# voidstrike/FPSG

Hardware: AMD Instinct MI355X
Metric: episodes/sec (+ Chamfer-kernel HBM GB/s in roofline.hbm), 2048-pt clouds, 224x224 images; episode = fwd + Chamfer + bwd, step = E episodes + all-reduce + Adam (higher is better)
Workload: dtype f32

## Files before the change

fpsg_amd/_hip.py:

```python
from __future__ import annotations

import ctypes
import os
import threading

import torch

_HERE = os.path.dirname(os.path.abspath(__file__))
LIB_PATH = os.environ.get("FPSG_HIP_LIB") or os.path.join(_HERE, "libfpsg_hip.so")

_c_f32p = ctypes.c_void_p
_c_i32p = ctypes.c_void_p
_c_int = ctypes.c_int
_c_stream = ctypes.c_void_p

SIGNATURES = {
    "fpsg_version": [],
    "fpsg_last_error": [],
    "fpsg_chamfer_fwd": [_c_f32p, _c_f32p, _c_int, _c_int, _c_int,
                         _c_f32p, _c_i32p, _c_f32p, _c_i32p, _c_stream],
    "fpsg_chamfer_bwd": [_c_f32p, _c_f32p, _c_i32p, _c_i32p, _c_f32p, _c_f32p,
                         _c_int, _c_int, _c_int, _c_f32p, _c_f32p, _c_stream],
    "fpsg_chamfer_losses": [_c_f32p, _c_f32p, _c_int, _c_int, _c_int, _c_int, ctypes.c_float, ctypes.c_float, _c_f32p,
                            _c_stream],
    "fpsg_chamfer_loss_grads": [_c_f32p, _c_f32p, _c_f32p, _c_int, _c_int, _c_int, _c_int, ctypes.c_float,
                                ctypes.c_float, _c_f32p, _c_f32p, _c_stream],
    "fpsg_chamfer_fwd_variant": [_c_f32p, _c_f32p, _c_int, _c_int, _c_int,
                                 _c_f32p, _c_i32p, _c_f32p, _c_i32p, _c_int, _c_stream],
    "fpsg_chamfer_workspace_bytes": [_c_int, _c_int, _c_int, _c_int],
    "fpsg_chamfer_fwd_tiled": [_c_f32p, _c_f32p, _c_int, _c_int, _c_int,
                               _c_f32p, _c_i32p, _c_f32p, _c_i32p, ctypes.c_void_p, ctypes.c_size_t, _c_int,
                               _c_stream],
    "fpsg_chamfer_fwd_tiled_losses": [_c_f32p, _c_f32p, _c_int, _c_int, _c_int,
                                      _c_f32p, _c_i32p, _c_f32p, _c_i32p, ctypes.c_void_p, ctypes.c_size_t, _c_int,
                                      _c_int, ctypes.c_float, ctypes.c_float, _c_f32p, _c_stream],
    "fpsg_chamfer_bwd_losses": [_c_f32p, _c_f32p, _c_i32p, _c_i32p, _c_f32p, _c_f32p, _c_f32p,
                                _c_int, _c_int, _c_int, _c_int, ctypes.c_float, ctypes.c_float, _c_f32p, _c_f32p,
                                _c_stream],
    "fpsg_chamfer_bwd_sorted": [_c_f32p, _c_f32p, _c_i32p, _c_i32p, _c_f32p, _c_f32p,
                                _c_int, _c_int, _c_int, _c_f32p, _c_f32p, _c_stream],
    "fpsg_chamfer_bwd_scan": [_c_f32p, _c_f32p, _c_i32p, _c_i32p, _c_f32p, _c_f32p,
                              _c_int, _c_int, _c_int, _c_f32p, _c_f32p, _c_stream],
    "fpsg_knn_workspace_floats": [_c_int, _c_int, _c_int],
    "fpsg_knn": [_c_f32p, _c_int, _c_int, _c_int, _c_int, _c_i32p, _c_f32p, _c_stream],
    "fpsg_knn_ex": [_c_f32p, _c_int, _c_int, _c_int, _c_int, _c_int, _c_i32p, _c_f32p, _c_int, _c_stream],
    "fpsg_edge_feature_fwd": [_c_f32p, _c_i32p, _c_int, _c_int, _c_int, _c_int, _c_f32p, _c_stream],
    "fpsg_edge_feature_bwd": [_c_f32p, _c_i32p, _c_int, _c_int, _c_int, _c_int, _c_f32p, _c_stream],
    "fpsg_edgeconv_blocks": [_c_int, _c_int, _c_int],
    "fpsg_edgeconv_reverse_graph_fits": [_c_int, _c_int],
    "fpsg_edgeconv_reverse_graph": [_c_i32p, _c_int, _c_int, _c_int, _c_i32p, _c_i32p, _c_stream],
    "fpsg_edgeconv_prep_blocks": [ctypes.c_long],
    "fpsg_edgeconv_stats_finalize": [_c_f32p, _c_int, _c_f32p, _c_f32p, _c_f32p, _c_f32p, ctypes.c_float, ctypes.c_float,
                                     ctypes.c_double, _c_int, _c_int, _c_f32p, _c_stream],
    "fpsg_edgeconv_stats_ws_floats": [_c_int, _c_int],
    "fpsg_edgeconv_stats_finalize_ws": [_c_f32p, _c_int, _c_f32p, _c_f32p, _c_f32p, _c_f32p, ctypes.c_float, ctypes.c_float,
                                        ctypes.c_double, _c_int, _c_int, _c_f32p, _c_f32p, _c_stream],
    "fpsg_edgeconv_bwd_finalize": [_c_f32p, _c_int, _c_f32p, ctypes.c_double, _c_int, _c_int, _c_f32p, _c_f32p, _c_f32p,
                                   _c_stream],
    "fpsg_edgeconv_act": [_c_f32p, _c_f32p, _c_f32p, ctypes.c_float, ctypes.c_long, _c_int, _c_f32p, _c_stream],
    "fpsg_edgeconv_bwd_prep": [_c_f32p, _c_f32p, _c_f32p, _c_f32p, ctypes.c_float, ctypes.c_long, _c_int, _c_f32p, _c_f32p,
                               _c_stream],
    "fpsg_edgeconv_fwd": [_c_f32p, _c_i32p, _c_f32p, _c_int, _c_int, _c_int, _c_int, _c_f32p, _c_f32p,
                          _c_f32p, _c_f32p, _c_stream],
    "fpsg_edgeconv_bwd": [_c_f32p, _c_f32p, _c_f32p, _c_f32p, _c_i32p, _c_i32p, _c_f32p, _c_int, _c_int,
                          _c_int, _c_int, _c_f32p, _c_stream],
    "fpsg_softmin": [_c_f32p, _c_f32p, _c_f32p, _c_int, _c_int, _c_int, ctypes.c_float, _c_f32p, _c_stream],
    "fpsg_sinkhorn_workspace_floats": [_c_int, _c_int, _c_int],
    "fpsg_sinkhorn_divergence": [_c_f32p, _c_f32p, _c_int, _c_int, _c_int, ctypes.c_void_p, _c_int, _c_f32p, _c_f32p,
                                 _c_stream],
    "fpsg_dec1_tiles": [_c_int],
    "fpsg_dec1_fwd": [_c_f32p, _c_f32p, _c_int, _c_int, _c_f32p, _c_f32p, _c_f32p, _c_f32p, _c_f32p, _c_int, _c_int,
                      _c_int, _c_int, _c_int, ctypes.c_float, _c_f32p, _c_f32p, _c_f32p, _c_f32p, _c_stream],
    "fpsg_dec1_bwd": [_c_f32p, _c_f32p, _c_f32p, _c_int, _c_int, _c_f32p, _c_f32p, _c_int, _c_int, _c_int, _c_int,
                      _c_int, _c_f32p, _c_f32p, _c_f32p, _c_f32p, _c_f32p, _c_stream],
    "fpsg_dec1_fwd_ld": [_c_f32p, _c_int, _c_f32p, _c_int, _c_int, _c_f32p, _c_int, _c_f32p, _c_f32p, _c_f32p, _c_f32p, _c_int,
                         _c_int, _c_int, _c_int, _c_int, ctypes.c_float, _c_f32p, _c_int, _c_f32p, _c_f32p, _c_f32p,
                         _c_stream],
    "fpsg_dec1_bwd_ld": [_c_f32p, _c_int, _c_f32p, _c_int, _c_f32p, _c_int, _c_int, _c_f32p, _c_int, _c_f32p, _c_int, _c_int,
                         _c_int, _c_int, _c_int, _c_int, _c_f32p, _c_f32p, _c_f32p, _c_f32p, _c_f32p, _c_stream],
    "fpsg_bn_act_rows_fwd": [_c_f32p, _c_int, ctypes.POINTER(ctypes.c_int), ctypes.POINTER(ctypes.c_int), _c_int,
                             _c_f32p, _c_f32p, _c_f32p, _c_int, ctypes.c_float, _c_int, ctypes.c_float, _c_f32p,
                             _c_f32p, _c_f32p, _c_stream],
    "fpsg_bn_act_rows_bwd": [_c_f32p, _c_int, ctypes.POINTER(ctypes.c_int), ctypes.POINTER(ctypes.c_int), _c_int,
                             _c_f32p, _c_f32p, _c_f32p, _c_int, _c_int, ctypes.c_float, _c_f32p, _c_f32p, _c_f32p,
                             _c_f32p, _c_stream],
    "fpsg_bn_workspace_floats": [_c_int, _c_int, _c_int],
    "fpsg_bn_act_fwd": [_c_f32p, _c_f32p, _c_f32p, _c_f32p, _c_f32p, _c_f32p, ctypes.c_float, _c_int, _c_int, _c_int, _c_int,
                        ctypes.c_float, _c_int, ctypes.c_float, _c_f32p, _c_f32p, _c_f32p, _c_f32p, _c_f32p,
                        _c_stream],
    "fpsg_bn_act_bwd": [_c_f32p, _c_f32p, _c_f32p, _c_f32p, _c_int, _c_int, _c_int, _c_int, _c_int,
                        ctypes.c_float, _c_f32p, _c_f32p, _c_f32p, _c_f32p, _c_f32p, _c_f32p, _c_stream],
    "fpsg_bn_act_bwd_coef": [_c_f32p, _c_f32p, _c_f32p, _c_f32p, _c_int, _c_int, _c_int, _c_int, _c_int, ctypes.c_float,
                             _c_f32p, _c_f32p, _c_f32p, _c_f32p, _c_stream],
    "fpsg_bn_act_bwd_parts": [_c_f32p, _c_f32p, _c_f32p, _c_f32p, _c_int, _c_int, _c_int, _c_int, _c_int,
                        ctypes.c_float, _c_f32p, _c_f32p, _c_f32p, _c_f32p, _c_f32p, _c_f32p, _c_f32p, _c_int, _c_stream],
    "fpsg_bn_pool_workspace_floats": [_c_int, _c_int, _c_int, _c_int],
    "fpsg_bn_act_pool_fwd": [_c_f32p, _c_f32p, _c_f32p, _c_f32p, _c_f32p, _c_f32p, ctypes.c_float, _c_int, _c_int, _c_int, _c_int,
                             _c_int, ctypes.c_float, _c_int, ctypes.c_float, _c_f32p, _c_f32p, _c_f32p, _c_f32p,
                             _c_f32p, _c_f32p, _c_int, _c_stream],
    "fpsg_bn_act_pool_bwd": [_c_f32p, _c_f32p, _c_f32p, _c_f32p, _c_int, _c_int, _c_int, _c_int, _c_int, _c_int,
                             ctypes.c_float, _c_f32p, _c_f32p, _c_f32p, _c_f32p, _c_f32p, _c_f32p, _c_stream],
    "fpsg_bn_max_workspace_floats": [_c_int, _c_int, _c_int],
    "fpsg_bn_max_dz_offset": [_c_int, _c_int, _c_int],
    "fpsg_bn_act_max_fwd": [_c_f32p, _c_f32p, _c_f32p, _c_f32p, _c_f32p, _c_f32p, ctypes.c_float, _c_int, _c_int, _c_int, _c_int,
                            ctypes.c_float, _c_int, ctypes.c_float, _c_f32p, _c_i32p, _c_f32p, _c_f32p, _c_f32p,
                            _c_f32p, _c_stream],
    "fpsg_bn_act_max_bwd": [_c_f32p, _c_f32p, _c_f32p, _c_i32p, _c_f32p, _c_int, _c_int, _c_int, _c_int, _c_int,
                            ctypes.c_float, _c_f32p, _c_f32p, _c_f32p, _c_f32p, _c_f32p, _c_f32p, _c_stream],
    "fpsg_max_bwd_prep": [_c_f32p, _c_f32p, _c_f32p, _c_f32p, _c_f32p, _c_f32p, _c_int, _c_int, _c_int, _c_int, _c_f32p, _c_f32p,
                          _c_f32p, _c_f32p, _c_stream],
    "fpsg_max_bwd_dw": [_c_f32p, _c_f32p, _c_f32p, _c_f32p, _c_f32p, _c_int, _c_int, _c_int, _c_f32p, _c_stream],
    "fpsg_max_bwd_gather": [_c_f32p, _c_f32p, _c_i32p, _c_int, _c_int, _c_int, _c_int, _c_f32p, _c_f32p, _c_stream],
    "fpsg_max_bwd_scatter": [_c_f32p, _c_f32p, _c_f32p, _c_f32p, _c_i32p, _c_f32p, _c_int, _c_int, _c_int, _c_int, _c_f32p,
                             _c_stream],
    "fpsg_max_bwd_scatter_workspace_floats": [_c_int, _c_int, _c_int],
    "fpsg_bn_act_max_bwd_coef": [_c_f32p, _c_f32p, _c_f32p, _c_i32p, _c_f32p, _c_int, _c_int, _c_int, _c_int, _c_int,
                                 ctypes.c_float, _c_f32p, _c_f32p, _c_f32p, _c_f32p, _c_stream],
    "fpsg_wino_input_transform": [_c_int, _c_f32p, _c_int, _c_int, _c_int, _c_int, _c_f32p, ctypes.c_long, _c_stream],
    "fpsg_wino_output_transform": [_c_int, _c_f32p, _c_int, _c_int, _c_int, _c_int, _c_f32p, ctypes.c_long, _c_stream],
    "fpsg_wino_stats_parts": [_c_int, _c_int, _c_int, _c_int],
    "fpsg_wino_output_transform_stats": [_c_int, _c_f32p, _c_int, _c_int, _c_int, _c_int, _c_f32p, _c_f32p, _c_f32p,
                                         ctypes.c_long, _c_stream],
    "fpsg_wino_grad_output_transform": [_c_int, _c_f32p, _c_int, _c_int, _c_int, _c_int, _c_f32p, ctypes.c_long, _c_stream],
    "fpsg_wino_grad_transforms": [_c_int, _c_f32p, _c_int, _c_int, _c_int, _c_int, _c_f32p, _c_f32p, ctypes.c_long, _c_stream],
    "fpsg_wino_filter_transform": [_c_int, _c_f32p, _c_int, _c_int, _c_int, _c_f32p, _c_stream],
    "fpsg_wino_output_transform_bwd_stats": [_c_int, _c_f32p, _c_int, _c_int, _c_int, _c_int, _c_f32p, _c_f32p, _c_f32p,
                                             _c_f32p, _c_f32p, ctypes.c_long, _c_stream],
    "fpsg_wino_filter_transform_batch": [ctypes.c_void_p, _c_int, ctypes.c_long, _c_stream],
    "fpsg_wino_filter_grad_transform": [_c_int, _c_f32p, _c_int, _c_int, _c_f32p, _c_stream],
    "fpsg_wino_conv_fused": [_c_f32p, _c_f32p, _c_int, _c_int, _c_int, _c_int, _c_int, _c_f32p, _c_stream],
    "fpsg_wino_input_transform_act": [_c_int, _c_f32p, _c_f32p, _c_f32p, _c_int, _c_int, _c_int, _c_int, _c_f32p, ctypes.c_long,
                                      _c_stream],
    "fpsg_wino_conv_fused_act": [_c_f32p, _c_f32p, _c_f32p, _c_f32p, _c_int, _c_int, _c_int, _c_int, _c_int, _c_f32p,
                                 _c_stream],
    "fpsg_wino_dw_fused_workspace_floats": [_c_int, _c_int, _c_int, _c_int],
    "fpsg_wino_dw_fused": [_c_f32p, _c_f32p, _c_f32p, _c_f32p, _c_int, _c_int, _c_int, _c_int, _c_int, _c_f32p, _c_f32p,
                           _c_stream],
    "fpsg_wino_conv_fused_parts": [_c_int, _c_int, _c_int, _c_int],
    "fpsg_wino_conv_fused_stats": [_c_f32p, _c_f32p, _c_f32p, _c_f32p, _c_int, _c_int, _c_int, _c_int, _c_int, _c_f32p,
                                   _c_f32p, _c_f32p, _c_stream],
    "fpsg_bn_stats": [_c_f32p, _c_f32p, _c_f32p, _c_f32p, _c_f32p, _c_f32p, ctypes.c_float, _c_int, _c_int, _c_int, _c_int,
                      ctypes.c_float, _c_f32p, _c_f32p, _c_f32p, _c_f32p, _c_f32p, _c_int, _c_stream],
    "fpsg_conv_first_dw_workspace_floats": [_c_int, _c_int, _c_int],
    "fpsg_conv_first_parts": [_c_int, _c_int, _c_int],
    "fpsg_conv_first_fwd": [_c_f32p, _c_f32p, _c_int, _c_int, _c_int, _c_int, _c_int, _c_f32p, _c_f32p, _c_f32p, _c_stream],
    "fpsg_conv_first_dw": [_c_f32p, _c_f32p, _c_int, _c_int, _c_int, _c_int, _c_int, _c_f32p, _c_f32p, _c_stream],
    "fpsg_conv_first_dw_fold": [_c_f32p, _c_f32p, _c_f32p, _c_f32p, _c_f32p, _c_f32p, _c_int, _c_int, _c_int, _c_int, _c_int,
                                _c_f32p, _c_f32p, _c_stream],
    "fpsg_adam_step": [_c_f32p, _c_f32p, _c_f32p, _c_f32p, ctypes.c_size_t, ctypes.c_float, ctypes.c_float,
                       ctypes.c_float, ctypes.c_float, _c_int, ctypes.c_float, _c_stream],
    "fpsg_flat_accumulate_segments": [_c_f32p, ctypes.c_void_p, ctypes.c_void_p, _c_int, ctypes.c_size_t, _c_int, _c_stream],
    "fpsg_flat_accumulate_tables": [_c_f32p, ctypes.c_void_p, ctypes.c_void_p, _c_int, _c_int, ctypes.c_size_t, _c_int,
                                    _c_stream],
    "fpsg_adam_step_segments": [_c_f32p, ctypes.c_void_p, ctypes.c_void_p, _c_int, _c_f32p, _c_f32p, ctypes.c_size_t,
                                ctypes.c_float, ctypes.c_float, ctypes.c_float, ctypes.c_float, _c_int, ctypes.c_float,
                                _c_stream],
    "fpsg_gemm_split_workspace_floats": [_c_int, _c_int, _c_int, _c_int, _c_int, _c_int],
    "fpsg_gemm_split": [_c_f32p, _c_f32p, _c_f32p, _c_int, _c_int, _c_int, _c_int, _c_int, _c_int, _c_int, ctypes.c_long,
                        ctypes.c_long, ctypes.c_long, _c_int, _c_int, _c_f32p, ctypes.c_size_t, _c_stream],
    "fpsg_gemm_split_packed_a_bytes": [_c_int, _c_int, _c_int, _c_int],
    "fpsg_gemm_split_pack_a": [_c_f32p, _c_int, _c_int, _c_int, _c_int, ctypes.c_long, _c_int, ctypes.c_void_p, _c_stream],
    "fpsg_gemm_split_nn_packed": [ctypes.c_void_p, _c_f32p, _c_f32p, _c_int, _c_int, _c_int, _c_int, _c_int, _c_int,
                                  ctypes.c_long, ctypes.c_long, _c_int, _c_stream],
    "fpsg_gemm_split_nn_persistent": [ctypes.c_void_p, _c_f32p, _c_f32p, _c_int, _c_int, _c_int, _c_int, _c_int, _c_int,
                                      ctypes.c_long, ctypes.c_long, _c_int, _c_stream],
    "fpsg_gemm_f32_nn": [_c_f32p, _c_f32p, _c_f32p, _c_int, _c_int, _c_int, _c_int, _c_int, _c_int, _c_int,
                         ctypes.c_long, ctypes.c_long, ctypes.c_long, _c_int, _c_stream],
    "fpsg_emd_workspace_floats": [_c_int, _c_int, _c_int],
    "fpsg_emd_approx": [_c_f32p, _c_f32p, _c_int, _c_int, _c_int, _c_f32p, _c_f32p, _c_f32p, _c_f32p,
                        _c_stream],
    "fpsg_emd_approx_variant": [_c_f32p, _c_f32p, _c_int, _c_int, _c_int, _c_f32p, _c_f32p, _c_f32p, _c_f32p, _c_int,
                                _c_stream],
    "fpsg_emd_exact_workspace_floats": [_c_int, _c_int],
    "fpsg_emd_exact": [_c_f32p, _c_f32p, _c_int, _c_int, ctypes.c_float, _c_int, _c_f32p, _c_f32p, _c_i32p, _c_i32p,
                       _c_f32p, _c_f32p, _c_f32p, _c_stream],
    "fpsg_chamfer_cross": [_c_f32p, _c_f32p, _c_int, _c_int, _c_int, _c_int, _c_f32p, _c_stream],
}
_RESTYPES = {"fpsg_last_error": ctypes.c_char_p, "fpsg_chamfer_workspace_bytes": ctypes.c_size_t,
             "fpsg_sinkhorn_workspace_floats": ctypes.c_size_t,
             "fpsg_knn_workspace_floats": ctypes.c_size_t,
             "fpsg_bn_workspace_floats": ctypes.c_size_t, "fpsg_bn_pool_workspace_floats": ctypes.c_size_t, "fpsg_bn_max_workspace_floats": ctypes.c_size_t, "fpsg_bn_max_dz_offset": ctypes.c_size_t, "fpsg_conv_first_dw_workspace_floats": ctypes.c_size_t, "fpsg_emd_workspace_floats": ctypes.c_size_t, "fpsg_emd_exact_workspace_floats": ctypes.c_size_t, "fpsg_max_bwd_scatter_workspace_floats": ctypes.c_size_t,
             "fpsg_wino_dw_fused_workspace_floats": ctypes.c_size_t, "fpsg_gemm_split_workspace_floats": ctypes.c_size_t, "fpsg_gemm_split_packed_a_bytes": ctypes.c_size_t, "fpsg_edgeconv_stats_ws_floats": ctypes.c_size_t}

_lib = None
_lock = threading.Lock()


class FpsgHipError(RuntimeError):
    pass


def load() -> ctypes.CDLL:
    global _lib
    if _lib is None:
        with _lock:
            if _lib is None:
                if not os.path.exists(LIB_PATH):
                    raise FpsgHipError(
                        f"{LIB_PATH} not found: build it with `make -C fpsg_amd/csrc` "
                        "(or `python -c 'import __graft_entry__ as g; g.build()'`). "
                        "fpsg_amd has no CPU or PyTorch fallback for its HIP ops.")
                lib = ctypes.CDLL(LIB_PATH)
                for name, argtypes in SIGNATURES.items():
                    fn = getattr(lib, name)
                    fn.argtypes = argtypes
                    fn.restype = _RESTYPES.get(name, ctypes.c_int)
                _lib = lib
    return _lib


def check(rc: int, what: str) -> None:
    if rc != 0:
        msg = load().fpsg_last_error()
        raise FpsgHipError(f"{what} failed (code {rc}): {msg.decode() if msg else ''}")


def dev_tensor(t: torch.Tensor, dtype: torch.dtype, name: str) -> torch.Tensor:
    if not isinstance(t, torch.Tensor):
        raise TypeError(f"{name}: expected a torch.Tensor, got {type(t)}")
    if t.device.type != "cuda":
        raise FpsgHipError(
            f"{name}: tensor is on '{t.device}'; fpsg_amd HIP ops run on a ROCm GPU only "
            "(no CPU fallback)")
    if t.dtype != dtype:
        raise TypeError(f"{name}: expected dtype {dtype}, got {t.dtype}")
    if not t.is_contiguous():
        raise ValueError(f"{name}: tensor must be contiguous")
    return t


def stream_of(t: torch.Tensor) -> int:
    return torch.cuda.current_stream(t.device).cuda_stream


def ptr(t: torch.Tensor) -> int:
    return t.data_ptr()
```

fpsg_amd/csrc/bnact.hip:

```cpp
#include <algorithm>
#include <atomic>
#include <cstdlib>

#include "fpsg_common.h"

namespace fpsg {
namespace {

constexpr int kBnThreads = 256;
constexpr int kBnSeg = 4096;
constexpr int kBnSlices = 64;
constexpr int kBnU = kBnSeg / 4 / kBnThreads;

enum BnAct { kActNone = 0, kActRelu = 1, kActLeaky = 2 };

template <int ACT>
__device__ __forceinline__ float act_fwd(float z, float slope) {
  if (ACT == kActRelu) return z > 0.0f ? z : 0.0f;
  if (ACT == kActLeaky) return z > 0.0f ? z : z * slope;
  return z;
}
template <int ACT>
__device__ __forceinline__ float act_grad(float z, float slope) {
  if (ACT == kActRelu) return z > 0.0f ? 1.0f : 0.0f;
  if (ACT == kActLeaky) return z > 0.0f ? 1.0f : slope;
  return 1.0f;
}

__device__ __forceinline__ void block_reduce2(float& a, float& b, float* red ) {
#pragma unroll
  for (int off = 32; off >= 1; off >>= 1) {
    a += __shfl_down(a, off, 64);
    b += __shfl_down(b, off, 64);
  }
  const int wave = threadIdx.x >> 6, lane = threadIdx.x & 63;
  if (lane == 0) { red[wave] = a; red[4 + wave] = b; }
  __syncthreads();
  if (threadIdx.x == 0) {
    a = (red[0] + red[1]) + (red[2] + red[3]);
    b = (red[4] + red[5]) + (red[6] + red[7]);
  }
}

constexpr int kBnFoldBanks = 16, kBnFoldChannels = 4096;
__device__ unsigned g_bn_fold_counters[kBnFoldBanks * kBnFoldChannels];
struct BnFoldArgs {
  const float* gamma; const float* beta;
  double count; float eps, momentum;
  float* chan; float* batch_mean; float* batch_var_unbiased; float* run_mean; float* run_var;
  unsigned* counters;
};
__device__ __forceinline__ void wave_sum2(double& a, double& b);
__device__ __forceinline__ void bn_fwd_finalize_channel(double s0, double s1, int c, int C, const float* gamma, const float* beta,
                                                        double count, float eps, float* chan, float* batch_mean,
                                                        float* batch_var_unbiased, float* run_mean, float* run_var, float momentum);

template <int MODE, int ACT, bool NT = false, bool FOLD = false>
__global__ __launch_bounds__(kBnThreads) void bn_reduce_kernel(
    const float* __restrict__ x, const float* __restrict__ dy, const float* __restrict__ chan ,
    const float* __restrict__ pb, int N, int C, int L, int S, float slope, float* __restrict__ part ,
    const BnFoldArgs f = BnFoldArgs{}) {
  __shared__ float red[8];
  const int c = blockIdx.y, s = blockIdx.x;
  const float b = pb ? pb[c] : 0.0f;
  const int segs = (L + kBnSeg - 1) / kBnSeg;
  const int items = N * segs;
  float sc = 0.0f, sh = 0.0f, mu = 0.0f, rs = 0.0f;
  if (MODE == 1) { sc = chan[c]; sh = chan[C + c]; mu = chan[2 * C + c]; rs = chan[3 * C + c]; }
  float a0 = 0.0f, a1 = 0.0f;
  const bool vec = (L & 3) == 0;
  for (int it = s; it < items; it += S) {
    const int n = it / segs, seg = it - n * segs;
    const size_t base = ((size_t)n * C + c) * L + (size_t)seg * kBnSeg;
    const int len = (L - seg * kBnSeg) < kBnSeg ? (L - seg * kBnSeg) : kBnSeg;
    if (vec) {
      const v4f* __restrict__ xp = reinterpret_cast<const v4f*>(x + base);
      const v4f* __restrict__ gp = reinterpret_cast<const v4f*>(MODE == 1 ? dy + base : x + base);
      const int nvec = len / 4;
      for (int e0 = threadIdx.x; e0 < nvec; e0 += kBnU * kBnThreads) {
        v4f xq[kBnU], gq[kBnU];
#pragma unroll
        for (int j = 0; j < kBnU; ++j) {
          const int e = e0 + j * kBnThreads;
          xq[j] = gq[j] = (v4f){0.0f, 0.0f, 0.0f, 0.0f};
          if (e < nvec) {
            xq[j] = ld_stream<NT>(xp + e);
            if (MODE == 1) gq[j] = ld_stream<NT>(gp + e);
          }
        }
#pragma unroll
        for (int j = 0; j < kBnU; ++j) {
          if (e0 + j * kBnThreads < nvec) {
            v4f xv = xq[j];
#pragma unroll
            for (int u = 0; u < 4; ++u) xv[u] += b;
            if (MODE == 0) {
#pragma unroll
              for (int u = 0; u < 4; ++u) { a0 += xv[u]; a1 = fma_rn(xv[u], xv[u], a1); }
            } else {
#pragma unroll
              for (int u = 0; u < 4; ++u) {
                const float dz = gq[j][u] * act_grad<ACT>(fma_rn(xv[u], sc, sh), slope);
                a0 += dz;
                a1 = fma_rn(dz, (xv[u] - mu) * rs, a1);
              }
            }
          }
        }
      }
    } else {
      for (int e = threadIdx.x; e < len; e += kBnThreads) {
        const float xv = x[base + e] + b;
        if (MODE == 0) {
          a0 += xv; a1 = fma_rn(xv, xv, a1);
        } else {
          const float dz = dy[base + e] * act_grad<ACT>(fma_rn(xv, sc, sh), slope);
          a0 += dz;
          a1 = fma_rn(dz, (xv - mu) * rs, a1);
        }
      }
    }
  }
  block_reduce2(a0, a1, red);
  if constexpr (FOLD) {
    __shared__ int last;
    if (threadIdx.x == 0) {
      __hip_atomic_store(&part[((size_t)c * S + s) * 2 + 0], a0, __ATOMIC_RELAXED, __HIP_MEMORY_SCOPE_AGENT);
      __hip_atomic_store(&part[((size_t)c * S + s) * 2 + 1], a1, __ATOMIC_RELAXED, __HIP_MEMORY_SCOPE_AGENT);
      asm volatile("s_waitcnt vmcnt(0)" ::: "memory");
      const unsigned t = __hip_atomic_fetch_add(&f.counters[c], 1u, __ATOMIC_RELAXED, __HIP_MEMORY_SCOPE_AGENT);
      last = t == (unsigned)S - 1u;
    }
    __syncthreads();
    if (!last || threadIdx.x >= 64) return;
    const int lane = threadIdx.x;
    double s0 = 0.0, s1 = 0.0;
    for (int sl = lane; sl < S; sl += 64) {
      s0 += __hip_atomic_load(&part[((size_t)c * S + sl) * 2], __ATOMIC_RELAXED, __HIP_MEMORY_SCOPE_AGENT);
      s1 += __hip_atomic_load(&part[((size_t)c * S + sl) * 2 + 1], __ATOMIC_RELAXED, __HIP_MEMORY_SCOPE_AGENT);
    }
    wave_sum2(s0, s1);
    if (lane != 0) return;
    bn_fwd_finalize_channel(s0, s1, c, C, f.gamma, f.beta, f.count, f.eps, f.chan, f.batch_mean, f.batch_var_unbiased,
                            f.run_mean, f.run_var, f.momentum);
    __hip_atomic_store(&f.counters[c], 0u, __ATOMIC_RELAXED, __HIP_MEMORY_SCOPE_AGENT);
    return;
  }
  if (threadIdx.x == 0) {
    part[((size_t)c * S + s) * 2 + 0] = a0;
    part[((size_t)c * S + s) * 2 + 1] = a1;
  }
}

__device__ __forceinline__ void wave_sum2(double& a, double& b) {
#pragma unroll
  for (int off = 32; off >= 1; off >>= 1) { a += __shfl_down(a, off, 64); b += __shfl_down(b, off, 64); }
}

__global__ __launch_bounds__(64) void bn_fwd_finalize_kernel(const float* __restrict__ part, const float* __restrict__ gamma,
                                       const float* __restrict__ beta, int C, int S, double count, float eps,
                                       float* __restrict__ chan, float* __restrict__ batch_mean,
                                       float* __restrict__ batch_var_unbiased, float* __restrict__ run_mean,
                                       float* __restrict__ run_var, float momentum) {
  const int c = blockIdx.x, lane = threadIdx.x;
  double s0 = 0.0, s1 = 0.0;
  for (int sl = lane; sl < S; sl += 64) { s0 += part[((size_t)c * S + sl) * 2]; s1 += part[((size_t)c * S + sl) * 2 + 1]; }
  wave_sum2(s0, s1);
  if (lane != 0) return;
  bn_fwd_finalize_channel(s0, s1, c, C, gamma, beta, count, eps, chan, batch_mean, batch_var_unbiased, run_mean, run_var, momentum);
}

__device__ __forceinline__ void bn_fwd_finalize_channel(double s0, double s1, int c, int C, const float* gamma, const float* beta,
                                                        double count, float eps, float* chan, float* batch_mean,
                                                        float* batch_var_unbiased, float* run_mean, float* run_var, float momentum) {
  const double mean = s0 / count;
  double var = s1 / count - mean * mean;
  var = var > 0.0 ? var : 0.0;
  const float rstd = (float)(1.0 / sqrt(var + (double)eps));
  const float g = gamma ? gamma[c] : 1.0f, b = beta ? beta[c] : 0.0f;
  const float scale = g * rstd;
  chan[c] = scale;
  chan[C + c] = b - (float)mean * scale;
  chan[2 * C + c] = (float)mean;
  chan[3 * C + c] = rstd;
  const float unbiased = (float)(count > 1.0 ? var * count / (count - 1.0) : var);
  if (batch_mean) batch_mean[c] = (float)mean;
  if (batch_var_unbiased) batch_var_unbiased[c] = unbiased;
  if (run_mean && momentum >= 0.0f) {
    run_mean[c] = fma_rn(momentum, (float)mean, (1.0f - momentum) * run_mean[c]);
    run_var[c] = fma_rn(momentum, unbiased, (1.0f - momentum) * run_var[c]);
  }
}

__global__ void bn_eval_chan_kernel(const float* __restrict__ rmean, const float* __restrict__ rvar,
                                    const float* __restrict__ gamma, const float* __restrict__ beta, int C,
                                    float eps, float* __restrict__ chan) {
  const int c = blockIdx.x * blockDim.x + threadIdx.x;
  if (c >= C) return;
  const float rstd = 1.0f / sqrtf(rvar[c] + eps);
  const float g = gamma ? gamma[c] : 1.0f, b = beta ? beta[c] : 0.0f;
  chan[c] = g * rstd;
  chan[C + c] = b - rmean[c] * g * rstd;
  chan[2 * C + c] = rmean[c];
  chan[3 * C + c] = rstd;
}

__global__ __launch_bounds__(64) void bn_bwd_finalize_kernel(const float* __restrict__ part, const float* __restrict__ chan, int C,
                                       int S, double count, int training, float* __restrict__ dgamma,
                                       float* __restrict__ dbeta, float* __restrict__ coef ) {
  const int c = blockIdx.x, lane = threadIdx.x;
  double s0 = 0.0, s1 = 0.0;
  for (int q = lane; q < S; q += 64) {
    s0 += part[((size_t)c * S + q) * 2];
    s1 += part[((size_t)c * S + q) * 2 + 1];
  }
  wave_sum2(s0, s1);
  if (lane != 0) return;
  dbeta[c] = (float)s0;
  dgamma[c] = (float)s1;
  const double scale = chan[c], mean = chan[2 * C + c], rstd = chan[3 * C + c];
  coef[c] = (float)scale;
  if (training) {
    const double k2 = -scale * s1 * rstd / count;
    coef[C + c] = (float)k2;
    coef[2 * C + c] = (float)(-scale * s0 / count - k2 * mean);
  } else {
    coef[C + c] = 0.0f;
    coef[2 * C + c] = 0.0f;
  }
}

template <int MODE, int ACT, bool NT = false>
__global__ __launch_bounds__(kBnThreads) void bn_apply_kernel(const float* __restrict__ x,
                                                              const float* __restrict__ dy,
                                                              const float* __restrict__ chan,
                                                              const float* __restrict__ coef,
                                                              const float* __restrict__ pb, int C, int L,
                                                              float slope, float* __restrict__ out,
                                                              float* __restrict__ dxpart ) {
  __shared__ float red[8];
  const int row = blockIdx.x;
  const int c = row % C;
  const int seg = blockIdx.y;
  const float b = pb ? pb[c] : 0.0f;
  float acc = 0.0f, unused = 0.0f;
  const size_t base = (size_t)row * L + (size_t)seg * kBnSeg;
  const int len = (L - seg * kBnSeg) < kBnSeg ? (L - seg * kBnSeg) : kBnSeg;
  const float sc = chan[c], sh = chan[C + c];
  float k1 = 0.0f, k2 = 0.0f, k3 = 0.0f;
  if (MODE == 1) { k1 = coef[c]; k2 = coef[C + c]; k3 = coef[2 * C + c]; }
  if ((L & 3) == 0) {
    const v4f* __restrict__ xp = reinterpret_cast<const v4f*>(x + base);
    const v4f* __restrict__ gp = reinterpret_cast<const v4f*>(MODE == 1 ? dy + base : x + base);
    v4f* __restrict__ op = reinterpret_cast<v4f*>(out + base);
    const int nvec = len / 4;
    for (int e0 = threadIdx.x; e0 < nvec; e0 += kBnU * kBnThreads) {
      v4f xq[kBnU], gq[kBnU];
#pragma unroll
      for (int j = 0; j < kBnU; ++j) {
        const int e = e0 + j * kBnThreads;
        xq[j] = gq[j] = (v4f){0.0f, 0.0f, 0.0f, 0.0f};
        if (e < nvec) {
          xq[j] = ld_stream<NT>(xp + e);
          if (MODE == 1) gq[j] = ld_stream<NT>(gp + e);
        }
      }
#pragma unroll
      for (int j = 0; j < kBnU; ++j) {
        const int e = e0 + j * kBnThreads;
        if (e < nvec) {
          v4f xv = xq[j];
#pragma unroll
          for (int u = 0; u < 4; ++u) xv[u] += b;
          v4f r;
          if (MODE == 0) {
#pragma unroll
            for (int u = 0; u < 4; ++u) r[u] = act_fwd<ACT>(fma_rn(xv[u], sc, sh), slope);
          } else {
#pragma unroll
            for (int u = 0; u < 4; ++u) {
              const float dz = gq[j][u] * act_grad<ACT>(fma_rn(xv[u], sc, sh), slope);
              r[u] = fma_rn(k1, dz, fma_rn(k2, xv[u], k3));
            }
            acc += (r[0] + r[1]) + (r[2] + r[3]);
          }
          st_stream<NT>(op + e, r);
        }
      }
    }
  } else {
    for (int e = threadIdx.x; e < len; e += kBnThreads) {
      const float xv = x[base + e] + b;
      if (MODE == 0) {
        out[base + e] = act_fwd<ACT>(fma_rn(xv, sc, sh), slope);
      } else {
        const float dz = dy[base + e] * act_grad<ACT>(fma_rn(xv, sc, sh), slope);
        const float r = fma_rn(k1, dz, fma_rn(k2, xv, k3));
        out[base + e] = r;
        acc += r;
      }
    }
  }
  if (MODE == 1 && dxpart) {
    block_reduce2(acc, unused, red);
    if (threadIdx.x == 0) dxpart[(size_t)row * gridDim.y + seg] = acc;
  }
}

__global__ __launch_bounds__(64) void bn_dxsum_kernel(const float* __restrict__ dxpart, int N, int C, int segs,
                                                      float* __restrict__ dpb) {
  const int c = blockIdx.x;
  const int items = N * segs;
  double a = 0.0;
  for (int it = threadIdx.x; it < items; it += 64) {
    const int n = it / segs, seg = it - n * segs;
    a += (double)dxpart[((size_t)n * C + c) * segs + seg];
  }
#pragma unroll
  for (int off = 32; off >= 1; off >>= 1) a += __shfl_down(a, off, 64);
  if (threadIdx.x == 0) dpb[c] = (float)a;
}

constexpr int kBnSmallMax = 16384;

constexpr int kBnMaxSegs = 4;
struct BnSegs {
  int ld;
  int off[kBnMaxSegs], len[kBnMaxSegs];
  int staged[kBnMaxSegs];
  int tpr_log2[kBnMaxSegs];
  int stat_stride;
};

template <int MODE, int ACT>
__global__ __launch_bounds__(kBnThreads) void bn_small_kernel(
    const float* __restrict__ x, const float* __restrict__ dy, const float* __restrict__ gamma,
    const float* __restrict__ beta, const float* __restrict__ pb, int N, int C, BnSegs segs, int training, float eps,
    float slope, float* __restrict__ out, float* __restrict__ chan, float* __restrict__ batch_mean,
    float* __restrict__ batch_var_unbiased, float* __restrict__ dgamma, float* __restrict__ dbeta,
    float* __restrict__ dpb, float* __restrict__ run_mean, float* __restrict__ run_var, float momentum) {
  const int sgi = blockIdx.y;
  const int L = segs.len[sgi], ld = segs.ld, staged = segs.staged[sgi], tpr_log2 = segs.tpr_log2[sgi];
  x += segs.off[sgi];
  out += segs.off[sgi];
  if (MODE == 1) dy += segs.off[sgi];
  chan += (size_t)sgi * 4 * C;
  if (batch_mean) batch_mean += (size_t)sgi * segs.stat_stride;
  if (batch_var_unbiased) batch_var_unbiased += (size_t)sgi * segs.stat_stride;
  if (MODE == 1) {
    dgamma += (size_t)sgi * C;
    dbeta += (size_t)sgi * C;
    if (dpb) dpb += (size_t)sgi * C;
  }
  extern __shared__ __attribute__((aligned(16))) float stage[];
  __shared__ float red[8];
  __shared__ float bc[4];
  const int c = blockIdx.x;
  const float b = pb ? pb[c] : 0.0f;
  const double count = (double)N * (double)L;
  const bool vec = (L & 3) == 0;
  const int L4 = L >> 2;
  v4f* __restrict__ sx = reinterpret_cast<v4f*>(stage);
  v4f* __restrict__ sd = reinterpret_cast<v4f*>(stage) + (size_t)N * L4;
  float sc = 0.0f, sh = 0.0f, mu = 0.0f, rs = 0.0f;
  if (MODE == 1 || !training) { sc = chan[c]; sh = chan[C + c]; mu = chan[2 * C + c]; rs = chan[3 * C + c]; }
  const bool two_sweeps = MODE == 1 || training;
  const bool keep = staged && vec && two_sweeps;
  const int tpr = 1 << tpr_log2, rpi = kBnThreads >> tpr_log2;
  const int e0 = threadIdx.x & (tpr - 1), n0 = threadIdx.x >> tpr_log2;
  if (two_sweeps) {
    float a0 = 0.0f, a1 = 0.0f;
    int n_first = n0;
    if (vec && L4 <= tpr) {
      const bool has = e0 < L4;
      for (; n_first + (kBnU - 1) * rpi < N; n_first += kBnU * rpi) {
        v4f xq[kBnU], gq[kBnU];
#pragma unroll
        for (int j = 0; j < kBnU; ++j) {
          xq[j] = gq[j] = (v4f){0.0f, 0.0f, 0.0f, 0.0f};
          if (has) {
            const size_t base = ((size_t)(n_first + j * rpi) * C + c) * ld;
            xq[j] = reinterpret_cast<const v4f*>(x + base)[e0];
            if (MODE == 1) gq[j] = reinterpret_cast<const v4f*>(dy + base)[e0];
          }
        }
        if (has) {
#pragma unroll
          for (int j = 0; j < kBnU; ++j) {
            const int n = n_first + j * rpi;
            v4f xv = xq[j];
#pragma unroll
            for (int u = 0; u < 4; ++u) xv[u] += b;
            if (MODE == 0) {
#pragma unroll
              for (int u = 0; u < 4; ++u) { a0 += xv[u]; a1 = fma_rn(xv[u], xv[u], a1); }
            } else {
              v4f dz;
#pragma unroll
              for (int u = 0; u < 4; ++u) {
                dz[u] = gq[j][u] * act_grad<ACT>(fma_rn(xv[u], sc, sh), slope);
                a0 += dz[u];
                a1 = fma_rn(dz[u], (xv[u] - mu) * rs, a1);
              }
              if (keep) sd[(size_t)n * L4 + e0] = dz;
            }
            if (keep) sx[(size_t)n * L4 + e0] = xv;
          }
        }
      }
    }
    for (int n = n_first; n < N; n += rpi) {
      const size_t base = ((size_t)n * C + c) * ld;
      if (vec) {
        const v4f* __restrict__ xp = reinterpret_cast<const v4f*>(x + base);
        const v4f* __restrict__ gp = reinterpret_cast<const v4f*>(MODE == 1 ? dy + base : x + base);
        for (int e = e0; e < L4; e += tpr) {
          v4f xv = xp[e];
#pragma unroll
          for (int u = 0; u < 4; ++u) xv[u] += b;
          if (MODE == 0) {
#pragma unroll
            for (int u = 0; u < 4; ++u) { a0 += xv[u]; a1 = fma_rn(xv[u], xv[u], a1); }
          } else {
            const v4f gv = gp[e];
            v4f dz;
#pragma unroll
            for (int u = 0; u < 4; ++u) {
              dz[u] = gv[u] * act_grad<ACT>(fma_rn(xv[u], sc, sh), slope);
              a0 += dz[u];
              a1 = fma_rn(dz[u], (xv[u] - mu) * rs, a1);
            }
            if (keep) sd[(size_t)n * L4 + e] = dz;
          }
          if (keep) sx[(size_t)n * L4 + e] = xv;
        }
      } else {
        for (int e = e0; e < L; e += tpr) {
          const float xv = x[base + e] + b;
          if (MODE == 0) {
            a0 += xv; a1 = fma_rn(xv, xv, a1);
          } else {
            const float dz = dy[base + e] * act_grad<ACT>(fma_rn(xv, sc, sh), slope);
            a0 += dz; a1 = fma_rn(dz, (xv - mu) * rs, a1);
          }
        }
      }
    }
    block_reduce2(a0, a1, red);
    if (threadIdx.x == 0) {
      if (MODE == 0) {
        const double mean = a0 / count;
        double var = a1 / count - mean * mean;
        var = var > 0.0 ? var : 0.0;
        const float rstd = (float)(1.0 / sqrt(var + (double)eps));
        const float g = gamma ? gamma[c] : 1.0f, bb = beta ? beta[c] : 0.0f;
        bc[0] = g * rstd; bc[1] = bb - (float)mean * g * rstd; bc[2] = (float)mean; bc[3] = rstd;
        chan[c] = bc[0]; chan[C + c] = bc[1]; chan[2 * C + c] = bc[2]; chan[3 * C + c] = bc[3];
        const float unbiased = (float)(count > 1.0 ? var * count / (count - 1.0) : var);
        if (batch_mean) batch_mean[c] = (float)mean;
        if (batch_var_unbiased) batch_var_unbiased[c] = unbiased;
        if (run_mean && momentum >= 0.0f) {
          run_mean[c] = fma_rn(momentum, (float)mean, (1.0f - momentum) * run_mean[c]);
          run_var[c] = fma_rn(momentum, unbiased, (1.0f - momentum) * run_var[c]);
        }
      } else {
        dbeta[c] = a0; dgamma[c] = a1;
        const double k2 = training ? -(double)sc * a1 * rs / count : 0.0;
        bc[0] = sc; bc[1] = (float)k2;
        bc[2] = training ? (float)(-(double)sc * a0 / count - k2 * mu) : 0.0f;
      }
    }
    __syncthreads();
    if (MODE == 0) { sc = bc[0]; sh = bc[1]; }
  } else {
    if (threadIdx.x == 0) { bc[0] = sc; bc[1] = 0.0f; bc[2] = 0.0f; }
    __syncthreads();
  }
  const float k1 = bc[0], k2 = bc[1], k3 = bc[2];
  float acc = 0.0f, unused = 0.0f;
  for (int n = n0; n < N; n += rpi) {
    const size_t base = ((size_t)n * C + c) * ld;
    if (vec) {
      const v4f* __restrict__ xp = reinterpret_cast<const v4f*>(x + base);
      const v4f* __restrict__ gp = reinterpret_cast<const v4f*>(MODE == 1 ? dy + base : x + base);
      v4f* __restrict__ op = reinterpret_cast<v4f*>(out + base);
      for (int e = e0; e < L4; e += tpr) {
        v4f xv;
        if (keep) {
          xv = sx[(size_t)n * L4 + e];
        } else {
          xv = xp[e];
#pragma unroll
          for (int u = 0; u < 4; ++u) xv[u] += b;
        }
        v4f r;
        if (MODE == 0) {
#pragma unroll
          for (int u = 0; u < 4; ++u) r[u] = act_fwd<ACT>(fma_rn(xv[u], sc, sh), slope);
        } else {
          v4f dz;
          if (keep) {
            dz = sd[(size_t)n * L4 + e];
          } else {
            const v4f gv = gp[e];
#pragma unroll
            for (int u = 0; u < 4; ++u) dz[u] = gv[u] * act_grad<ACT>(fma_rn(xv[u], sc, sh), slope);
          }
#pragma unroll
          for (int u = 0; u < 4; ++u) r[u] = fma_rn(k1, dz[u], fma_rn(k2, xv[u], k3));
          acc += (r[0] + r[1]) + (r[2] + r[3]);
        }
        op[e] = r;
      }
    } else {
      for (int e = e0; e < L; e += tpr) {
        const float xv = x[base + e] + b;
        if (MODE == 0) {
          out[base + e] = act_fwd<ACT>(fma_rn(xv, sc, sh), slope);
        } else {
          const float dz = dy[base + e] * act_grad<ACT>(fma_rn(xv, sc, sh), slope);
          const float r = fma_rn(k1, dz, fma_rn(k2, xv, k3));
          out[base + e] = r;
          acc += r;
        }
      }
    }
  }
  if (MODE == 1 && dpb) {
    __syncthreads();
    block_reduce2(acc, unused, red);
    if (threadIdx.x == 0) dpb[c] = acc;
  }
}

inline void small_segment(BnSegs& g, int i, int N, int off, int L, int training, bool backward) {
  g.off[i] = off;
  g.len[i] = L;
  const size_t need = (size_t)N * L * sizeof(float) * (backward ? 2 : 1);
  g.staged[i] = ((L & 3) == 0 && need <= 64 * 1024 && (backward || training)) ? 1 : 0;
  const int row_items = (L & 3) == 0 ? L / 4 : L;
  int t = 0;
  while ((1 << t) < row_items && (1 << t) < kBnThreads) ++t;
  g.tpr_log2[i] = t;
}

template <int MODE>
void launch_small_segs(int act, const float* x, const float* dy, const float* gamma, const float* beta, const float* pb,
                       int N, int C, const BnSegs& g, int nseg, int training, float eps, float slope, float* out,
                       float* chan, float* bm, float* bv, float* dgamma, float* dbeta, float* dpb, float* rmean,
                       float* rvar, float momentum, hipStream_t s) {
  dim3 grid(C, nseg);
  size_t lds = 0;
  for (int i = 0; i < nseg; ++i)
    if (g.staged[i]) lds = std::max(lds, (size_t)N * g.len[i] * sizeof(float) * (MODE == 1 ? 2 : 1));
#define FPSG_SMALL(A) hipLaunchKernelGGL((bn_small_kernel<MODE, A>), grid, dim3(kBnThreads), lds, s, x, dy, gamma, beta, \
                                         pb, N, C, g, training, eps, slope, out, chan, bm, bv, dgamma, dbeta, dpb, rmean, \
                                         rvar, momentum)
  if (act == kActRelu) FPSG_SMALL(kActRelu);
  else if (act == kActLeaky) FPSG_SMALL(kActLeaky);
  else FPSG_SMALL(kActNone);
#undef FPSG_SMALL
}

template <int MODE>
void launch_small(int act, const float* x, const float* dy, const float* gamma, const float* beta, const float* pb,
                  int N, int C, int L, int training, float eps, float slope, float* out, float* chan, float* bm,
                  float* bv, float* dgamma, float* dbeta, float* dpb, float* rmean, float* rvar, float momentum,
                  hipStream_t s) {
  BnSegs g{};
  g.ld = L;
  small_segment(g, 0, N, 0, L, training, MODE == 1);
  launch_small_segs<MODE>(act, x, dy, gamma, beta, pb, N, C, g, 1, training, eps, slope, out, chan, bm, bv, dgamma,
                          dbeta, dpb, rmean, rvar, momentum, s);
}

int slices_for(int N, int L) {
  const int items = N * ((L + kBnSeg - 1) / kBnSeg);
  return items < kBnSlices ? items : kBnSlices;
}

template <int MODE>
void launch_reduce(int act, const float* x, const float* dy, const float* chan, const float* pb, int N, int C, int L,
                   int S, float slope, float* part, hipStream_t s) {
  dim3 grid(S, C);
#define FPSG_RED(A, T) hipLaunchKernelGGL((bn_reduce_kernel<MODE, A, T>), grid, dim3(kBnThreads), 0, s, x, dy, chan, pb, N, C, L, S, slope, part)
  if (beyond_cache((size_t)N * C * L * sizeof(float))) {
    if (act == kActRelu) FPSG_RED(kActRelu, true); else if (act == kActLeaky) FPSG_RED(kActLeaky, true); else FPSG_RED(kActNone, true);
  } else {
    if (act == kActRelu) FPSG_RED(kActRelu, false); else if (act == kActLeaky) FPSG_RED(kActLeaky, false); else FPSG_RED(kActNone, false);
  }
#undef FPSG_RED
}

template <int MODE>
void launch_apply(int act, const float* x, const float* dy, const float* chan, const float* coef, const float* pb,
                  int N, int C, int L, float slope, float* out, float* dxpart, hipStream_t s) {
  dim3 grid((unsigned)((size_t)N * C), (L + kBnSeg - 1) / kBnSeg);
#define FPSG_APP(A, T) hipLaunchKernelGGL((bn_apply_kernel<MODE, A, T>), grid, dim3(kBnThreads), 0, s, x, dy, chan, coef, pb, C, L, slope, out, dxpart)
  if (beyond_cache((size_t)N * C * L * sizeof(float))) {
    if (act == kActRelu) FPSG_APP(kActRelu, true); else if (act == kActLeaky) FPSG_APP(kActLeaky, true); else FPSG_APP(kActNone, true);
  } else {
    if (act == kActRelu) FPSG_APP(kActRelu, false); else if (act == kActLeaky) FPSG_APP(kActLeaky, false); else FPSG_APP(kActNone, false);
  }
#undef FPSG_APP
}

template <int VW> struct PoolVec;
template <> struct PoolVec<2> { typedef v4f in_t; typedef v2f out_t; };
template <> struct PoolVec<1> { typedef v2f in_t; typedef float out_t; };

template <int ACT>
__device__ __forceinline__ int window_argmax(const float (&z)[4], float slope, float& ymax) {
  float m = -INFINITY;
  int sel = 0;
#pragma unroll
  for (int k = 0; k < 4; ++k) {
    const float y = act_fwd<ACT>(z[k], slope);
    if (y > m || y != y) { m = y; sel = k; }
  }
  ymax = m;
  return sel;
}

template <int MODE, int ACT, int VW, bool NT>
__device__ __forceinline__ void pool_item(const float* __restrict__ xpl, const float* __restrict__ gpl,
// ... 308 lines not shown
      coef[2 * C + c] = 0.0f;
    }
  }
}

template <bool NT>
__global__ __launch_bounds__(kBnThreads) void bn_max_apply_kernel(const float* __restrict__ x,
                                                                  const float* __restrict__ pb,
                                                                  const float* __restrict__ dz,
                                                                  const int* __restrict__ idx,
                                                                  const float* __restrict__ coef, int C, int L,
                                                                  float* __restrict__ dx, float* __restrict__ dxpart) {
  __shared__ float red[8];
  const int row = blockIdx.x, c = row % C, seg = blockIdx.y;
  const size_t base = (size_t)row * L + (size_t)seg * kBnSeg;
  const int len = (L - seg * kBnSeg) < kBnSeg ? (L - seg * kBnSeg) : kBnSeg;
  const float b = pb ? pb[c] : 0.0f;
  const float k1 = coef[c], k2 = coef[C + c], k3 = coef[2 * C + c];
  const float d = dz[row];
  const int sel = idx[row] - seg * kBnSeg;
  float acc = 0.0f, unused = 0.0f;
  if ((L & 3) == 0) {
    const v4f* __restrict__ xp = reinterpret_cast<const v4f*>(x + base);
    v4f* __restrict__ op = reinterpret_cast<v4f*>(dx + base);
    const int nvec = len / 4;
    for (int e0 = threadIdx.x; e0 < nvec; e0 += kBnU * kBnThreads) {
      v4f xq[kBnU];
#pragma unroll
      for (int j = 0; j < kBnU; ++j) {
        const int e = e0 + j * kBnThreads;
        xq[j] = e < nvec ? ld_stream<NT>(xp + e) : (v4f){0.0f, 0.0f, 0.0f, 0.0f};
      }
#pragma unroll
      for (int j = 0; j < kBnU; ++j) {
        const int e = e0 + j * kBnThreads;
        if (e < nvec) {
          v4f r;
#pragma unroll
          for (int u = 0; u < 4; ++u) r[u] = fma_rn(k1, (4 * e + u == sel) ? d : 0.0f, fma_rn(k2, xq[j][u] + b, k3));
          acc += (r[0] + r[1]) + (r[2] + r[3]);
          st_stream<NT>(op + e, r);
        }
      }
    }
  } else {
    for (int e = threadIdx.x; e < len; e += kBnThreads) {
      const float r = fma_rn(k1, (e == sel) ? d : 0.0f, fma_rn(k2, x[base + e] + b, k3));
      acc += r;
      dx[base + e] = r;
    }
  }
  if (dxpart) {
    block_reduce2(acc, unused, red);
    if (threadIdx.x == 0) dxpart[(size_t)row * gridDim.y + seg] = acc;
  }
}

int check_dims(const char* fn, int N, int C, int L, int act) {
  FPSG_REQUIRE(N > 0 && C > 0 && L > 0, FPSG_E_SHAPE, "%s: N,C,L must be positive (got %d,%d,%d)", fn, N, C, L);
  FPSG_REQUIRE(act >= 0 && act <= 2, FPSG_E_SHAPE, "%s: act must be 0 (none), 1 (relu) or 2 (leaky)", fn);
  FPSG_REQUIRE(C <= 65535 && (L + kBnSeg - 1) / kBnSeg <= 65535 && (long)N * C < (1L << 31), FPSG_E_LIMIT,
               "%s: C=%d, L=%d or N*C=%ld beyond the grid limits", fn, C, L, (long)N * C);
  return 0;
}

}
}

extern "C" size_t fpsg_bn_workspace_floats(int N, int C, int L) {
  if (N <= 0 || C <= 0 || L <= 0) return 0;
  const size_t segs = ((size_t)L + fpsg::kBnSeg - 1) / fpsg::kBnSeg;
  return (size_t)C * fpsg::kBnSlices * 2 + (size_t)N * C * segs;
}

extern "C" int fpsg_bn_act_fwd(const float* x, const float* pre_bias, const float* gamma, const float* beta,
                               float* running_mean, float* running_var, float momentum, int N, int C, int L,
                               int training, float eps, int act, float slope, float* y, float* chan,
                               float* batch_mean, float* batch_var_unbiased, float* ws, fpsg_stream_t stream) {
  using namespace fpsg;
  int rc = check_dims("fpsg_bn_act_fwd", N, C, L, act);
  if (rc) return rc;
  FPSG_REQUIRE_PTR(x); FPSG_REQUIRE_PTR(y); FPSG_REQUIRE_PTR(chan);
  FPSG_REQUIRE(((reinterpret_cast<uintptr_t>(x) | reinterpret_cast<uintptr_t>(y)) & 15) == 0, FPSG_E_ALIGN,
               "fpsg_bn_act_fwd: x and y must be 16-byte aligned");
  hipStream_t s = static_cast<hipStream_t>(stream);
  const bool chan_given = training == 2;
  if (chan_given) training = 0;
  if (!training && !chan_given) { FPSG_REQUIRE_PTR(running_mean); FPSG_REQUIRE_PTR(running_var); }
  if ((long)N * L <= kBnSmallMax) {
    if (!training && !chan_given) {
      hipLaunchKernelGGL(bn_eval_chan_kernel, dim3((C + 255) / 256), dim3(256), 0, s, running_mean, running_var,
                         gamma, beta, C, eps, chan);
      if ((rc = launch_status("fpsg_bn_act_fwd(eval)"))) return rc;
    }
    launch_small<0>(act, x, nullptr, gamma, beta, pre_bias, N, C, L, training, eps, slope, y, chan, batch_mean,
                    batch_var_unbiased, nullptr, nullptr, nullptr, running_mean, running_var, momentum, s);
    return launch_status("fpsg_bn_act_fwd(small)");
  }
  if (training) {
    FPSG_REQUIRE_PTR(ws);
    const int S = slices_for(N, L);
    const char* fold = getenv("FPSG_BN_FINALIZE_FOLD");
    if (fold && fold[0] == '1' && C <= kBnFoldChannels) {
      static std::atomic<unsigned> next_bank{0};
      unsigned* counters = nullptr;
      FPSG_REQUIRE(hipGetSymbolAddress(reinterpret_cast<void**>(&counters), HIP_SYMBOL(g_bn_fold_counters)) == hipSuccess &&
                       counters, FPSG_E_LIMIT, "fpsg_bn_act_fwd: the fold counters are not addressable");
      BnFoldArgs f{gamma, beta, (double)N * (double)L, eps, momentum, chan, batch_mean, batch_var_unbiased, running_mean,
                   running_var, counters + (size_t)(next_bank.fetch_add(1) % kBnFoldBanks) * kBnFoldChannels};
      const dim3 grid(S, C);
      if (beyond_cache((size_t)N * C * L * sizeof(float)))
        hipLaunchKernelGGL((bn_reduce_kernel<0, kActNone, true, true>), grid, dim3(kBnThreads), 0, s, x, nullptr, nullptr, pre_bias, N, C, L, S, 0.0f, ws, f);
      else
        hipLaunchKernelGGL((bn_reduce_kernel<0, kActNone, false, true>), grid, dim3(kBnThreads), 0, s, x, nullptr, nullptr, pre_bias, N, C, L, S, 0.0f, ws, f);
      if ((rc = launch_status("fpsg_bn_act_fwd(stats + finalize)"))) return rc;
    } else {
      launch_reduce<0>(kActNone, x, nullptr, nullptr, pre_bias, N, C, L, S, 0.0f, ws, s);
      if ((rc = launch_status("fpsg_bn_act_fwd(stats)"))) return rc;
      hipLaunchKernelGGL(bn_fwd_finalize_kernel, dim3(C), dim3(64), 0, s, ws, gamma, beta, C, S,
                         (double)N * (double)L, eps, chan, batch_mean, batch_var_unbiased, running_mean, running_var,
                         momentum);
      if ((rc = launch_status("fpsg_bn_act_fwd(finalize)"))) return rc;
    }
  } else if (!chan_given) {
    hipLaunchKernelGGL(bn_eval_chan_kernel, dim3((C + 255) / 256), dim3(256), 0, s, running_mean, running_var,
                       gamma, beta, C, eps, chan);
    if ((rc = launch_status("fpsg_bn_act_fwd(eval)"))) return rc;
  }
  launch_apply<0>(act, x, nullptr, chan, nullptr, pre_bias, N, C, L, slope, y, nullptr, s);
  return launch_status("fpsg_bn_act_fwd(apply)");
}

namespace fpsg {
namespace {
int rows_segments(const char* fn, int ld, const int* seg_off, const int* seg_len, int nseg, int C, int act, bool backward,
                  BnSegs& g) {
  FPSG_REQUIRE(C > 0 && C <= 65535 * 64 && ld > 0, FPSG_E_SHAPE, "%s: C, ld must be positive (got %d, %d)", fn, C, ld);
  FPSG_REQUIRE(act >= kActNone && act <= kActLeaky, FPSG_E_SHAPE, "%s: unknown activation %d", fn, act);
  FPSG_REQUIRE(nseg >= 1 && nseg <= kBnMaxSegs, FPSG_E_LIMIT, "%s: %d segments (1..%d)", fn, nseg, kBnMaxSegs);
  FPSG_REQUIRE_PTR(seg_off); FPSG_REQUIRE_PTR(seg_len);
  FPSG_REQUIRE((ld & 3) == 0, FPSG_E_ALIGN, "%s: ld = %d must be a multiple of 4", fn, ld);
  g = BnSegs{};
  g.ld = ld;
  for (int i = 0; i < nseg; ++i) {
    FPSG_REQUIRE(seg_len[i] > 0 && seg_len[i] <= kBnSmallMax && seg_off[i] >= 0 && seg_off[i] + seg_len[i] <= ld,
                 FPSG_E_SHAPE, "%s: segment %d = [%d, +%d) does not fit a row of %d (a segment holds at most %d)", fn, i,
                 seg_off[i], seg_len[i], ld, kBnSmallMax);
    FPSG_REQUIRE((seg_off[i] & 3) == 0, FPSG_E_ALIGN, "%s: segment offset %d must be a multiple of 4", fn, seg_off[i]);
    for (int j = 0; j < i; ++j)
      FPSG_REQUIRE(seg_off[i] >= seg_off[j] + seg_len[j] || seg_off[j] >= seg_off[i] + seg_len[i], FPSG_E_SHAPE,
                   "%s: segments %d and %d overlap", fn, j, i);
    small_segment(g, i, 1, seg_off[i], seg_len[i], 1, backward);
  }
  return 0;
}
}
}

extern "C" int fpsg_bn_act_rows_fwd(const float* x, int ld, const int* seg_off, const int* seg_len, int nseg,
                                    const float* pre_bias, const float* gamma, const float* beta, int C, float eps,
                                    int act, float slope, float* y, float* chan, float* stats,
                                    fpsg_stream_t stream) {
  using namespace fpsg;
  BnSegs g;
  int rc = rows_segments("fpsg_bn_act_rows_fwd", ld, seg_off, seg_len, nseg, C, act, false, g);
  if (rc) return rc;
  FPSG_REQUIRE_PTR(x); FPSG_REQUIRE_PTR(y); FPSG_REQUIRE_PTR(chan);
  FPSG_REQUIRE(((reinterpret_cast<uintptr_t>(x) | reinterpret_cast<uintptr_t>(y)) & 15) == 0, FPSG_E_ALIGN,
               "fpsg_bn_act_rows_fwd: x and y must be 16-byte aligned");
  g.stat_stride = 2 * C;
  launch_small_segs<0>(act, x, nullptr, gamma, beta, pre_bias, 1, C, g, nseg, 1, eps, slope, y, chan, stats,
                       stats ? stats + C : nullptr, nullptr, nullptr, nullptr, nullptr, nullptr, -1.0f,
                       static_cast<hipStream_t>(stream));
  return launch_status("fpsg_bn_act_rows_fwd");
}

extern "C" int fpsg_bn_act_rows_bwd(const float* x, int ld, const int* seg_off, const int* seg_len, int nseg,
                                    const float* pre_bias, const float* dy, const float* chan, int C, int act,
                                    float slope, float* dx, float* dgamma, float* dbeta, float* dpre_bias,
                                    fpsg_stream_t stream) {
  using namespace fpsg;
  BnSegs g;
  int rc = rows_segments("fpsg_bn_act_rows_bwd", ld, seg_off, seg_len, nseg, C, act, true, g);
  if (rc) return rc;
  FPSG_REQUIRE_PTR(x); FPSG_REQUIRE_PTR(dy); FPSG_REQUIRE_PTR(chan); FPSG_REQUIRE_PTR(dx);
  FPSG_REQUIRE_PTR(dgamma); FPSG_REQUIRE_PTR(dbeta);
  FPSG_REQUIRE(((reinterpret_cast<uintptr_t>(x) | reinterpret_cast<uintptr_t>(dy) | reinterpret_cast<uintptr_t>(dx)) & 15) == 0,
               FPSG_E_ALIGN, "fpsg_bn_act_rows_bwd: x, dy and dx must be 16-byte aligned");
  launch_small_segs<1>(act, x, dy, nullptr, nullptr, pre_bias, 1, C, g, nseg, 1, 0.0f, slope, dx,
                       const_cast<float*>(chan), nullptr, nullptr, dgamma, dbeta, dpre_bias, nullptr, nullptr, -1.0f,
                       static_cast<hipStream_t>(stream));
  return launch_status("fpsg_bn_act_rows_bwd");
}

extern "C" int fpsg_bn_stats(const float* x, const float* pre_bias, const float* gamma, const float* beta,
                             float* running_mean, float* running_var, float momentum, int N, int C, int L,
                             int training, float eps, float* chan, float* batch_mean, float* batch_var_unbiased,
                             float* ws, const float* parts, int n_parts, fpsg_stream_t stream) {
  using namespace fpsg;
  int rc = check_dims("fpsg_bn_stats", N, C, L, kActNone);
  if (rc) return rc;
  FPSG_REQUIRE_PTR(x); FPSG_REQUIRE_PTR(chan);
  FPSG_REQUIRE((reinterpret_cast<uintptr_t>(x) & 15) == 0, FPSG_E_ALIGN, "fpsg_bn_stats: x must be 16-byte aligned");
  hipStream_t s = static_cast<hipStream_t>(stream);
  if (training) {
    int S = n_parts;
    if (parts) {
      FPSG_REQUIRE(n_parts > 0, FPSG_E_SHAPE, "fpsg_bn_stats: n_parts must be positive with parts (got %d)", n_parts);
    } else {
      FPSG_REQUIRE_PTR(ws);
      S = slices_for(N, L);
      launch_reduce<0>(kActNone, x, nullptr, nullptr, pre_bias, N, C, L, S, 0.0f, ws, s);
      if ((rc = launch_status("fpsg_bn_stats(stats)"))) return rc;
    }
    hipLaunchKernelGGL(bn_fwd_finalize_kernel, dim3(C), dim3(64), 0, s, parts ? parts : ws, gamma, beta, C, S,
                       (double)N * (double)L, eps, chan, batch_mean, batch_var_unbiased, running_mean, running_var,
                       momentum);
    return launch_status("fpsg_bn_stats(finalize)");
  }
  FPSG_REQUIRE_PTR(running_mean); FPSG_REQUIRE_PTR(running_var);
  hipLaunchKernelGGL(bn_eval_chan_kernel, dim3((C + 255) / 256), dim3(256), 0, s, running_mean, running_var,
                     gamma, beta, C, eps, chan);
  return launch_status("fpsg_bn_stats(eval)");
}

extern "C" int fpsg_bn_act_bwd(const float* x, const float* pre_bias, const float* dy, const float* chan, int N,
                               int C, int L, int training, int act, float slope, float* dx, float* dgamma,
                               float* dbeta, float* dpre_bias, float* coef, float* ws, fpsg_stream_t stream) {
  using namespace fpsg;
  int rc = check_dims("fpsg_bn_act_bwd", N, C, L, act);
  if (rc) return rc;
  FPSG_REQUIRE_PTR(x); FPSG_REQUIRE_PTR(dy); FPSG_REQUIRE_PTR(chan); FPSG_REQUIRE_PTR(dx);
  FPSG_REQUIRE_PTR(dgamma); FPSG_REQUIRE_PTR(dbeta); FPSG_REQUIRE_PTR(coef); FPSG_REQUIRE_PTR(ws);
  FPSG_REQUIRE(((reinterpret_cast<uintptr_t>(x) | reinterpret_cast<uintptr_t>(dy) | reinterpret_cast<uintptr_t>(dx)) & 15) == 0,
               FPSG_E_ALIGN, "fpsg_bn_act_bwd: x, dy and dx must be 16-byte aligned");
  hipStream_t s = static_cast<hipStream_t>(stream);
  if ((long)N * L <= kBnSmallMax) {
    launch_small<1>(act, x, dy, nullptr, nullptr, pre_bias, N, C, L, training, 0.0f, slope, dx,
                    const_cast<float*>(chan), nullptr, nullptr, dgamma, dbeta, dpre_bias, nullptr, nullptr, -1.0f, s);
    return launch_status("fpsg_bn_act_bwd(small)");
  }
  const int S = slices_for(N, L);
  launch_reduce<1>(act, x, dy, chan, pre_bias, N, C, L, S, slope, ws, s);
  if ((rc = launch_status("fpsg_bn_act_bwd(reduce)"))) return rc;
  hipLaunchKernelGGL(bn_bwd_finalize_kernel, dim3(C), dim3(64), 0, s, ws, chan, C, S,
                     (double)N * (double)L, training, dgamma, dbeta, coef);
  if ((rc = launch_status("fpsg_bn_act_bwd(finalize)"))) return rc;
  float* dxpart = dpre_bias ? ws + (size_t)C * kBnSlices * 2 : nullptr;
  launch_apply<1>(act, x, dy, chan, coef, pre_bias, N, C, L, slope, dx, dxpart, s);
  if ((rc = launch_status("fpsg_bn_act_bwd(apply)"))) return rc;
  if (dpre_bias) {
    hipLaunchKernelGGL(bn_dxsum_kernel, dim3(C), dim3(64), 0, s, dxpart, N, C, (L + kBnSeg - 1) / kBnSeg, dpre_bias);
    return launch_status("fpsg_bn_act_bwd(dpre_bias)");
  }
  return 0;
}

extern "C" int fpsg_bn_act_bwd_coef(const float* x, const float* pre_bias, const float* dy, const float* chan, int N,
                                    int C, int L, int training, int act, float slope, float* dgamma, float* dbeta,
                                    float* coef, float* ws, fpsg_stream_t stream) {
  using namespace fpsg;
  int rc = check_dims("fpsg_bn_act_bwd_coef", N, C, L, act);
  if (rc) return rc;
  FPSG_REQUIRE_PTR(x); FPSG_REQUIRE_PTR(dy); FPSG_REQUIRE_PTR(chan);
  FPSG_REQUIRE_PTR(dgamma); FPSG_REQUIRE_PTR(dbeta); FPSG_REQUIRE_PTR(coef); FPSG_REQUIRE_PTR(ws);
  FPSG_REQUIRE(((reinterpret_cast<uintptr_t>(x) | reinterpret_cast<uintptr_t>(dy)) & 15) == 0, FPSG_E_ALIGN,
               "fpsg_bn_act_bwd_coef: x and dy must be 16-byte aligned");
  FPSG_REQUIRE((long)N * L > kBnSmallMax, FPSG_E_LIMIT, "fpsg_bn_act_bwd_coef: N*L = %ld is a small tensor (<= %d): use fpsg_bn_act_bwd",
               (long)N * L, kBnSmallMax);
  hipStream_t s = static_cast<hipStream_t>(stream);
  const int S = slices_for(N, L);
  launch_reduce<1>(act, x, dy, chan, pre_bias, N, C, L, S, slope, ws, s);
  if ((rc = launch_status("fpsg_bn_act_bwd_coef(reduce)"))) return rc;
  hipLaunchKernelGGL(bn_bwd_finalize_kernel, dim3(C), dim3(64), 0, s, ws, chan, C, S,
                     (double)N * (double)L, training, dgamma, dbeta, coef);
  return launch_status("fpsg_bn_act_bwd_coef(finalize)");
}

extern "C" int fpsg_bn_act_bwd_parts(const float* x, const float* pre_bias, const float* dy, const float* chan, int N,
                                     int C, int L, int training, int act, float slope, float* dx, float* dgamma,
                                     float* dbeta, float* dpre_bias, float* coef, float* ws, const float* parts,
                                     int n_parts, fpsg_stream_t stream) {
  using namespace fpsg;
  int rc = check_dims("fpsg_bn_act_bwd_parts", N, C, L, act);
  if (rc) return rc;
  FPSG_REQUIRE_PTR(x); FPSG_REQUIRE_PTR(dy); FPSG_REQUIRE_PTR(chan); FPSG_REQUIRE_PTR(dx); FPSG_REQUIRE_PTR(parts);
  FPSG_REQUIRE_PTR(dgamma); FPSG_REQUIRE_PTR(dbeta); FPSG_REQUIRE_PTR(coef);
  FPSG_REQUIRE(n_parts > 0, FPSG_E_SHAPE, "fpsg_bn_act_bwd_parts: n_parts must be positive (got %d)", n_parts);
  FPSG_REQUIRE(dpre_bias == nullptr || ws != nullptr, FPSG_E_NULL, "fpsg_bn_act_bwd_parts: dpre_bias needs the workspace");
  FPSG_REQUIRE(((reinterpret_cast<uintptr_t>(x) | reinterpret_cast<uintptr_t>(dy) | reinterpret_cast<uintptr_t>(dx)) & 15) == 0,
               FPSG_E_ALIGN, "fpsg_bn_act_bwd_parts: x, dy and dx must be 16-byte aligned");
  hipStream_t s = static_cast<hipStream_t>(stream);
  hipLaunchKernelGGL(bn_bwd_finalize_kernel, dim3(C), dim3(64), 0, s, parts, chan, C, n_parts,
                     (double)N * (double)L, training, dgamma, dbeta, coef);
  if ((rc = launch_status("fpsg_bn_act_bwd_parts(finalize)"))) return rc;
  float* dxpart = dpre_bias ? ws + (size_t)C * kBnSlices * 2 : nullptr;
  launch_apply<1>(act, x, dy, chan, coef, pre_bias, N, C, L, slope, dx, dxpart, s);
  if ((rc = launch_status("fpsg_bn_act_bwd_parts(apply)"))) return rc;
  if (dpre_bias) {
    hipLaunchKernelGGL(bn_dxsum_kernel, dim3(C), dim3(64), 0, s, dxpart, N, C, (L + kBnSeg - 1) / kBnSeg, dpre_bias);
    return launch_status("fpsg_bn_act_bwd_parts(dpre_bias)");
  }
  return 0;
}

extern "C" size_t fpsg_bn_pool_workspace_floats(int N, int C, int H, int W) {
  if (N <= 0 || C <= 0 || H <= 1 || W <= 1) return 0;
  const int RP = fpsg::pool_rows_per_item(W);
  const size_t items = (size_t)(H / 2 + RP - 1) / RP;
  return (size_t)C * fpsg::kBnSlices * 2 + (size_t)N * C * items;
}

extern "C" int fpsg_bn_act_pool_fwd(const float* x, const float* pre_bias, const float* gamma, const float* beta,
                                    float* running_mean, float* running_var, float momentum, int N, int C, int H, int W,
                                    int training, float eps, int act, float slope, float* y_pooled, float* chan,
                                    float* batch_mean, float* batch_var_unbiased, float* ws, const float* parts,
                                    int n_parts, fpsg_stream_t stream) {
  using namespace fpsg;
  int rc = check_pool_dims("fpsg_bn_act_pool_fwd", N, C, H, W, act);
  if (rc) return rc;
  FPSG_REQUIRE_PTR(x); FPSG_REQUIRE_PTR(y_pooled); FPSG_REQUIRE_PTR(chan);
  FPSG_REQUIRE(((reinterpret_cast<uintptr_t>(x) | reinterpret_cast<uintptr_t>(y_pooled)) & 15) == 0, FPSG_E_ALIGN,
               "fpsg_bn_act_pool_fwd: x and y_pooled must be 16-byte aligned");
  hipStream_t s = static_cast<hipStream_t>(stream);
  const int L = H * W;
  const bool chan_given = training == 2;
  if (chan_given) training = 0;
  if (training) {
    int S = n_parts;
    if (parts) {
      FPSG_REQUIRE(n_parts > 0, FPSG_E_SHAPE, "fpsg_bn_act_pool_fwd: n_parts must be positive with parts (got %d)", n_parts);
    } else {
      FPSG_REQUIRE_PTR(ws);
      S = slices_for(N, L);
      launch_reduce<0>(kActNone, x, nullptr, nullptr, pre_bias, N, C, L, S, 0.0f, ws, s);
      if ((rc = launch_status("fpsg_bn_act_pool_fwd(stats)"))) return rc;
    }
    hipLaunchKernelGGL(bn_fwd_finalize_kernel, dim3(C), dim3(64), 0, s, parts ? parts : ws, gamma, beta, C, S,
                       (double)N * (double)L, eps, chan, batch_mean, batch_var_unbiased, running_mean, running_var,
                       momentum);
    if ((rc = launch_status("fpsg_bn_act_pool_fwd(finalize)"))) return rc;
  } else if (!chan_given) {
    FPSG_REQUIRE_PTR(running_mean); FPSG_REQUIRE_PTR(running_var);
    hipLaunchKernelGGL(bn_eval_chan_kernel, dim3((C + 255) / 256), dim3(256), 0, s, running_mean, running_var,
                       gamma, beta, C, eps, chan);
    if ((rc = launch_status("fpsg_bn_act_pool_fwd(eval)"))) return rc;
  }
  launch_pool_apply<0>(act, x, nullptr, chan, nullptr, pre_bias, N, C, H, W, slope, y_pooled, nullptr, s);
  return launch_status("fpsg_bn_act_pool_fwd(apply)");
}

extern "C" int fpsg_bn_act_pool_bwd(const float* x, const float* pre_bias, const float* dy_pooled, const float* chan,
                                    int N, int C, int H, int W, int training, int act, float slope, float* dx,
                                    float* dgamma, float* dbeta, float* dpre_bias, float* coef, float* ws,
                                    fpsg_stream_t stream) {
  using namespace fpsg;
  int rc = check_pool_dims("fpsg_bn_act_pool_bwd", N, C, H, W, act);
  if (rc) return rc;
  FPSG_REQUIRE_PTR(x); FPSG_REQUIRE_PTR(dy_pooled); FPSG_REQUIRE_PTR(chan); FPSG_REQUIRE_PTR(dx);
  FPSG_REQUIRE_PTR(dgamma); FPSG_REQUIRE_PTR(dbeta); FPSG_REQUIRE_PTR(coef); FPSG_REQUIRE_PTR(ws);
  FPSG_REQUIRE(((reinterpret_cast<uintptr_t>(x) | reinterpret_cast<uintptr_t>(dy_pooled) | reinterpret_cast<uintptr_t>(dx)) & 15) == 0,
               FPSG_E_ALIGN, "fpsg_bn_act_pool_bwd: x, dy_pooled and dx must be 16-byte aligned");
  hipStream_t s = static_cast<hipStream_t>(stream);
  const int RP = pool_rows_per_item(W);
  const int per_plane = (H / 2 + RP - 1) / RP;
  const long items = (long)N * per_plane;
  const int S = items < kBnSlices ? (int)items : kBnSlices;
  launch_pool_reduce(act, x, dy_pooled, chan, pre_bias, N, C, H, W, S, slope, ws, s);
  if ((rc = launch_status("fpsg_bn_act_pool_bwd(reduce)"))) return rc;
  hipLaunchKernelGGL(bn_bwd_finalize_kernel, dim3(C), dim3(64), 0, s, ws, chan, C, S,
                     (double)N * (double)H * (double)W, training, dgamma, dbeta, coef);
  if ((rc = launch_status("fpsg_bn_act_pool_bwd(finalize)"))) return rc;
  float* dxpart = dpre_bias ? ws + (size_t)C * kBnSlices * 2 : nullptr;
  launch_pool_apply<2>(act, x, dy_pooled, chan, coef, pre_bias, N, C, H, W, slope, dx, dxpart, s);
  if ((rc = launch_status("fpsg_bn_act_pool_bwd(apply)"))) return rc;
  if (dpre_bias) {
    hipLaunchKernelGGL(bn_dxsum_kernel, dim3(C), dim3(64), 0, s, dxpart, N, C, per_plane, dpre_bias);
    return launch_status("fpsg_bn_act_pool_bwd(dpre_bias)");
  }
  return 0;
}

extern "C" size_t fpsg_bn_max_workspace_floats(int N, int C, int L) {
  if (N <= 0 || C <= 0 || L <= 0) return 0;
  const size_t segs = ((size_t)L + fpsg::kBnSeg - 1) / fpsg::kBnSeg;
  return (size_t)C * fpsg::kBnSlices * 2 + (size_t)N * C * segs * 4 + (size_t)N * C;
}

extern "C" size_t fpsg_bn_max_dz_offset(int N, int C, int L) {
  if (N <= 0 || C <= 0 || L <= 0) return 0;
  const size_t segs = ((size_t)L + fpsg::kBnSeg - 1) / fpsg::kBnSeg;
  return (size_t)C * fpsg::kBnSlices * 2 + (size_t)N * C * segs * 4;
}

extern "C" int fpsg_bn_act_max_fwd(const float* x, const float* pre_bias, const float* gamma, const float* beta,
                                   float* running_mean, float* running_var, float momentum, int N, int C, int L,
                                   int training, float eps, int act, float slope, float* out, int32_t* idx,
                                   float* chan, float* batch_mean, float* batch_var_unbiased, float* ws,
                                   fpsg_stream_t stream) {
  using namespace fpsg;
  int rc = check_dims("fpsg_bn_act_max_fwd", N, C, L, act);
  if (rc) return rc;
  FPSG_REQUIRE_PTR(x); FPSG_REQUIRE_PTR(out); FPSG_REQUIRE_PTR(idx); FPSG_REQUIRE_PTR(chan); FPSG_REQUIRE_PTR(ws);
  hipStream_t s = static_cast<hipStream_t>(stream);
  const int segs = (L + kBnSeg - 1) / kBnSeg;
  const int items_max = N * segs;
  const int S = items_max >= 4 * kBnSlices ? kBnSlices : (items_max + 3) / 4;
  RowExt* ext = reinterpret_cast<RowExt*>(ws + (size_t)C * kBnSlices * 2);
  dim3 grid(C, S);
  const bool chan_given = training == 2;
  if (chan_given) training = 0;
  if (training) {
    if (beyond_cache((size_t)N * C * L * sizeof(float))) hipLaunchKernelGGL((bn_reduce_ext_kernel<1, true>), grid, dim3(kBnThreads), 0, s, x, pre_bias, N, C, L, S, ws, ext);
    else hipLaunchKernelGGL(bn_reduce_ext_kernel<1>, grid, dim3(kBnThreads), 0, s, x, pre_bias, N, C, L, S, ws, ext);
    if ((rc = launch_status("fpsg_bn_act_max_fwd(stats)"))) return rc;
    hipLaunchKernelGGL(bn_fwd_finalize_kernel, dim3(C), dim3(64), 0, s, ws, gamma, beta, C, S,
                       (double)N * (double)L, eps, chan, batch_mean, batch_var_unbiased, running_mean, running_var,
                       momentum);
    if ((rc = launch_status("fpsg_bn_act_max_fwd(finalize)"))) return rc;
  } else {
    if (!chan_given) { FPSG_REQUIRE_PTR(running_mean); FPSG_REQUIRE_PTR(running_var); }
    hipLaunchKernelGGL(bn_reduce_ext_kernel<0>, grid, dim3(kBnThreads), 0, s, x, pre_bias, N, C, L, S, ws, ext);
    if ((rc = launch_status("fpsg_bn_act_max_fwd(extremes)"))) return rc;
    if (!chan_given) {
      hipLaunchKernelGGL(bn_eval_chan_kernel, dim3((C + 255) / 256), dim3(256), 0, s, running_mean, running_var,
                         gamma, beta, C, eps, chan);
      if ((rc = launch_status("fpsg_bn_act_max_fwd(eval)"))) return rc;
    }
  }
  const int rows = N * C;
  dim3 og((rows + 255) / 256);
  if (act == kActRelu) hipLaunchKernelGGL(bn_max_out_kernel<kActRelu>, og, dim3(256), 0, s, ext, chan, rows, C, segs, slope, out, idx);
  else if (act == kActLeaky) hipLaunchKernelGGL(bn_max_out_kernel<kActLeaky>, og, dim3(256), 0, s, ext, chan, rows, C, segs, slope, out, idx);
  else hipLaunchKernelGGL(bn_max_out_kernel<kActNone>, og, dim3(256), 0, s, ext, chan, rows, C, segs, slope, out, idx);
  return launch_status("fpsg_bn_act_max_fwd(out)");
}

extern "C" int fpsg_bn_act_max_bwd_coef(const float* x, const float* pre_bias, const float* gout, const int32_t* idx,
                                        const float* chan, int N, int C, int L, int training, int act, float slope,
                                        float* dgamma, float* dbeta, float* coef, float* ws, fpsg_stream_t stream) {
  using namespace fpsg;
  int rc = check_dims("fpsg_bn_act_max_bwd_coef", N, C, L, act);
  if (rc) return rc;
  FPSG_REQUIRE_PTR(x); FPSG_REQUIRE_PTR(gout); FPSG_REQUIRE_PTR(idx); FPSG_REQUIRE_PTR(chan);
  FPSG_REQUIRE_PTR(dgamma); FPSG_REQUIRE_PTR(dbeta); FPSG_REQUIRE_PTR(coef); FPSG_REQUIRE_PTR(ws);
  hipStream_t s = static_cast<hipStream_t>(stream);
  const int segs = (L + kBnSeg - 1) / kBnSeg;
  float* dz = ws + (size_t)C * kBnSlices * 2 + (size_t)N * C * segs * 4;
#define FPSG_MAXB(A) hipLaunchKernelGGL(bn_max_bwd_coef_kernel<A>, dim3(C), dim3(64), 0, s, x, pre_bias, gout, idx, chan, \
                                        N, C, L, training, slope, dz, dgamma, dbeta, coef)
  if (act == kActRelu) FPSG_MAXB(kActRelu); else if (act == kActLeaky) FPSG_MAXB(kActLeaky); else FPSG_MAXB(kActNone);
#undef FPSG_MAXB
  return launch_status("fpsg_bn_act_max_bwd_coef");
}

extern "C" int fpsg_bn_act_max_bwd(const float* x, const float* pre_bias, const float* gout, const int32_t* idx,
                                   const float* chan, int N, int C, int L, int training, int act, float slope,
                                   float* dx, float* dgamma, float* dbeta, float* dpre_bias, float* coef, float* ws,
                                   fpsg_stream_t stream) {
  using namespace fpsg;
  int rc = check_dims("fpsg_bn_act_max_bwd", N, C, L, act);
  if (rc) return rc;
  FPSG_REQUIRE_PTR(x); FPSG_REQUIRE_PTR(gout); FPSG_REQUIRE_PTR(idx); FPSG_REQUIRE_PTR(chan); FPSG_REQUIRE_PTR(dx);
  FPSG_REQUIRE_PTR(dgamma); FPSG_REQUIRE_PTR(dbeta); FPSG_REQUIRE_PTR(coef); FPSG_REQUIRE_PTR(ws);
  FPSG_REQUIRE(((reinterpret_cast<uintptr_t>(x) | reinterpret_cast<uintptr_t>(dx)) & 15) == 0, FPSG_E_ALIGN,
               "fpsg_bn_act_max_bwd: x and dx must be 16-byte aligned");
  hipStream_t s = static_cast<hipStream_t>(stream);
  const int segs = (L + kBnSeg - 1) / kBnSeg;
  float* dxpart = ws + (size_t)C * kBnSlices * 2;
  float* dz = dxpart + (size_t)N * C * segs * 4;
#define FPSG_MAXB(A) hipLaunchKernelGGL(bn_max_bwd_coef_kernel<A>, dim3(C), dim3(64), 0, s, x, pre_bias, gout, idx, chan, \
                                        N, C, L, training, slope, dz, dgamma, dbeta, coef)
  if (act == kActRelu) FPSG_MAXB(kActRelu); else if (act == kActLeaky) FPSG_MAXB(kActLeaky); else FPSG_MAXB(kActNone);
#undef FPSG_MAXB
  if ((rc = launch_status("fpsg_bn_act_max_bwd(coef)"))) return rc;
  dim3 grid((unsigned)((size_t)N * C), segs);
  hipLaunchKernelGGL(beyond_cache((size_t)N * C * L * sizeof(float)) ? bn_max_apply_kernel<true> : bn_max_apply_kernel<false>, grid, dim3(kBnThreads), 0, s, x, pre_bias, dz, idx, coef, C, L, dx,
                     dpre_bias ? dxpart : nullptr);
  if ((rc = launch_status("fpsg_bn_act_max_bwd(apply)"))) return rc;
  if (dpre_bias) {
    hipLaunchKernelGGL(bn_dxsum_kernel, dim3(C), dim3(64), 0, s, dxpart, N, C, segs, dpre_bias);
    return launch_status("fpsg_bn_act_max_bwd(dpre_bias)");
  }
  return 0;
}
```

fpsg_amd/csrc/winograd.hip:

```cpp
#include "fpsg_common.h"

namespace fpsg {
namespace {

constexpr size_t kStreamBytes = (size_t)300 << 20;
template <bool NT>
__device__ __forceinline__ void stream_store(float* p, float v) {
  if constexpr (NT) __builtin_nontemporal_store(v, p);
  else *p = v;
}
template <bool NT>
__device__ __forceinline__ float stream_load(const float* p) {
  if constexpr (NT) return __builtin_nontemporal_load(p);
  else return *p;
}

constexpr int kWinoThreads = 256;

template <int M> struct Wino;

template <> struct Wino<2> {
  static constexpr int A = 4;
  static __device__ __forceinline__ void in(const float (&d)[4], float (&t)[4]) {
    t[0] = d[0] - d[2]; t[1] = d[1] + d[2]; t[2] = d[2] - d[1]; t[3] = d[1] - d[3];
  }
  static __device__ __forceinline__ void out(const float (&m)[4], float (&s)[2]) {
    s[0] = (m[0] + m[1]) + m[2]; s[1] = (m[1] - m[2]) - m[3];
  }
  static __device__ __forceinline__ void flt(const float (&g)[3], float (&u)[4]) {
    u[0] = g[0]; u[1] = 0.5f * ((g[0] + g[1]) + g[2]); u[2] = 0.5f * ((g[0] - g[1]) + g[2]); u[3] = g[2];
  }
  static __device__ __forceinline__ void gout(const float (&y)[2], float (&r)[4]) {
    r[0] = y[0]; r[1] = y[0] + y[1]; r[2] = y[0] - y[1]; r[3] = -y[1];
  }
  static __device__ __forceinline__ void fgrad(const float (&u)[4], float (&a)[3]) {
    a[0] = u[0] + 0.5f * (u[1] + u[2]); a[1] = 0.5f * (u[1] - u[2]); a[2] = 0.5f * (u[1] + u[2]) + u[3];
  }
};

template <> struct Wino<4> {
  static constexpr int A = 6;
  static __device__ __forceinline__ void in(const float (&d)[6], float (&t)[6]) {
    const float p = fma_rn(-4.0f, d[2], d[4]), q = fma_rn(-4.0f, d[1], d[3]);
    const float r = d[4] - d[2], s = d[3] - d[1];
    t[0] = fma_rn(4.0f, d[0], fma_rn(-5.0f, d[2], d[4]));
    t[1] = p + q;
    t[2] = p - q;
    t[3] = fma_rn(2.0f, s, r);
    t[4] = fma_rn(-2.0f, s, r);
    t[5] = fma_rn(4.0f, d[1], fma_rn(-5.0f, d[3], d[5]));
  }
  static __device__ __forceinline__ void out(const float (&m)[6], float (&s)[4]) {
    const float p12 = m[1] + m[2], m12 = m[1] - m[2], p34 = m[3] + m[4], m34 = m[3] - m[4];
    s[0] = (m[0] + p12) + p34;
    s[1] = fma_rn(2.0f, m34, m12);
    s[2] = fma_rn(4.0f, p34, p12);
    s[3] = fma_rn(8.0f, m34, m12) + m[5];
  }
  static __device__ __forceinline__ void flt(const float (&g)[3], float (&u)[6]) {
    const float e = g[0] + g[2];
    u[0] = 0.25f * g[0];
    u[1] = (-1.0f / 6.0f) * (e + g[1]);
    u[2] = (-1.0f / 6.0f) * (e - g[1]);
    const float f = fma_rn(1.0f / 24.0f, g[0], (1.0f / 6.0f) * g[2]);
    u[3] = fma_rn(1.0f / 12.0f, g[1], f);
    u[4] = fma_rn(-1.0f / 12.0f, g[1], f);
    u[5] = g[2];
  }
  static __device__ __forceinline__ void gout(const float (&y)[4], float (&r)[6]) {
    const float e = y[0] + y[2], o = y[1] + y[3];
    r[0] = y[0];
    r[1] = e + o;
    r[2] = e - o;
    const float e4 = fma_rn(4.0f, y[2], y[0]), o4 = fma_rn(8.0f, y[3], 2.0f * y[1]);
    r[3] = e4 + o4;
    r[4] = e4 - o4;
    r[5] = y[3];
  }
  static __device__ __forceinline__ void fgrad(const float (&u)[6], float (&a)[3]) {
    const float p12 = u[1] + u[2], m12 = u[1] - u[2], p34 = u[3] + u[4], m34 = u[3] - u[4];
    a[0] = fma_rn(0.25f, u[0], fma_rn(-1.0f / 6.0f, p12, (1.0f / 24.0f) * p34));
    a[1] = fma_rn(-1.0f / 6.0f, m12, (1.0f / 12.0f) * m34);
    a[2] = fma_rn(-1.0f / 6.0f, p12, fma_rn(1.0f / 6.0f, p34, u[5]));
  }
};

struct TileIndex { long n; int th, tw; };
__device__ __forceinline__ TileIndex tile_of(long p, int Th, int Tw) {
  TileIndex t;
  t.tw = (int)(p % Tw);
  const long q = p / Tw;
  t.th = (int)(q % Th);
  t.n = q / Th;
  return t;
}

template <int M, bool ACT, bool NT = false, bool RAG = false, bool GO = false>
__global__ __launch_bounds__(kWinoThreads) void wino_input_kernel(const float* __restrict__ x, int C, int H, int W,
                                                                   int Th, int Tw, long P, long Ps, float* __restrict__ V,
                                                                   const float* __restrict__ chan,
                                                                   const float* __restrict__ pre_bias,
                                                                   float* __restrict__ dM = nullptr) {
  constexpr int A = Wino<M>::A;
  typedef float vin __attribute__((ext_vector_type(M)));
  const long p_raw = (long)blockIdx.x * kWinoThreads + threadIdx.x;
  const bool live = p_raw < P;
  const long p = live ? p_raw : P - 1;
  const int c = blockIdx.y;
  const TileIndex ti = tile_of(p, Th, Tw);
  const float* xp = x + ((size_t)ti.n * C + c) * H * W;
  const int r0 = M * ti.th - 1, c0 = M * ti.tw;
  const int lane = threadIdx.x & (kWave - 1);
  const bool has_left = ti.tw > 0, has_right = ti.tw < Tw - 1;
  const bool left_lane = has_left && lane > 0;
  const bool right_lane = has_right && lane < kWave - 1;
  float sc = 1.0f, sh = 0.0f, pb = 0.0f;
  if (ACT) { sc = chan[c]; sh = chan[C + c]; pb = pre_bias ? pre_bias[c] : 0.0f; }
  auto act = [&](float v) { return ACT ? __builtin_fmaxf(fma_rn(v + pb, sc, sh), 0.0f) : v; };
  vin mid[A];
  bool rin[A];
  const float* rp[A];
  const bool hi_in = !RAG || c0 + 2 < W;
#pragma unroll
  for (int i = 0; i < A; ++i) {
    const int r = r0 + i;
    rin[i] = r >= 0 && r < H;
    rp[i] = xp + (size_t)(rin[i] ? r : (r < 0 ? 0 : H - 1)) * W + c0;
    if constexpr (RAG) {
      typedef float v2 __attribute__((ext_vector_type(2)));
      const v2 lo = *reinterpret_cast<const v2*>(rp[i]);
      v2 hi = {0.0f, 0.0f};
      if (hi_in) hi = *reinterpret_cast<const v2*>(rp[i] + 2);
      mid[i][0] = lo[0]; mid[i][1] = lo[1]; mid[i][M - 2] = hi[0]; mid[i][M - 1] = hi[1];
    } else {
      mid[i] = *reinterpret_cast<const vin*>(rp[i]);
    }
  }
  float el[A], er[A];
#pragma unroll
  for (int i = 0; i < A; ++i) el[i] = er[i] = 0.0f;
  if (has_left && !left_lane) {
#pragma unroll
    for (int i = 0; i < A; ++i) el[i] = rp[i][-1];
  }
  if (has_right && !right_lane) {
#pragma unroll
    for (int i = 0; i < A; ++i) er[i] = rp[i][M];
  }
  float d[A][A];
#pragma unroll
  for (int i = 0; i < A; ++i) {
#pragma unroll
    for (int j = 0; j < M; ++j) mid[i][j] = (rin[i] && (!RAG || j < 2 || hi_in)) ? act(mid[i][j]) : 0.0f;
    float lft = __shfl_up(mid[i][M - 1], 1, kWave);
    float rgt = __shfl_down(mid[i][0], 1, kWave);
    if (!left_lane) lft = (has_left && rin[i]) ? act(el[i]) : 0.0f;
    if (!right_lane) rgt = (has_right && rin[i]) ? act(er[i]) : 0.0f;
    d[i][0] = lft;
#pragma unroll
    for (int j = 0; j < M; ++j) d[i][1 + j] = mid[i][j];
    d[i][A - 1] = rgt;
  }
  float t[A][A];
#pragma unroll
  for (int j = 0; j < A; ++j) {
    float col[A];
#pragma unroll
    for (int i = 0; i < A; ++i) col[i] = d[i][j];
    Wino<M>::in(col, t[j]);
  }
  const size_t plane = (size_t)C * Ps;
  if (!live) {
    if (p_raw < Ps) {
#pragma unroll
      for (int q = 0; q < A * A; ++q) {
        stream_store<NT>(V + (size_t)c * Ps + p_raw + (size_t)q * plane, 0.0f);
        if constexpr (GO) stream_store<NT>(dM + (size_t)c * Ps + p_raw + (size_t)q * plane, 0.0f);
      }
    }
    return;
  }
  float* vp = V + (size_t)c * Ps + p;
#pragma unroll
  for (int i = 0; i < A; ++i) {
    float row[A], v[A];
#pragma unroll
    for (int j = 0; j < A; ++j) row[j] = t[j][i];
    Wino<M>::in(row, v);
#pragma unroll
    for (int j = 0; j < A; ++j) stream_store<NT>(vp + (size_t)(A * i + j) * plane, v[j]);
  }
  if constexpr (GO) {
    static_assert(!ACT, "an output gradient is not activated");
    float r[M][A];
#pragma unroll
    for (int j = 0; j < M; ++j) {
      float col[M];
#pragma unroll
      for (int i = 0; i < M; ++i) col[i] = mid[1 + i][j];
      Wino<M>::gout(col, r[j]);
    }
    float* mp = dM + (size_t)c * Ps + p;
#pragma unroll
    for (int i = 0; i < A; ++i) {
      float row[M], o[A];
#pragma unroll
      for (int j = 0; j < M; ++j) row[j] = r[j][i];
      Wino<M>::gout(row, o);
#pragma unroll
      for (int j = 0; j < A; ++j) stream_store<NT>(mp + (size_t)(A * i + j) * plane, o[j]);
    }
  }
}

template <int M, bool STATS, bool BWD = false, bool NT = false, bool RAG = false>
__global__ __launch_bounds__(kWinoThreads) void wino_output_kernel(const float* __restrict__ Mt, int K, int H, int W,
                                                                    int Th, int Tw, long P, long Ps, float* __restrict__ y,
                                                                    const float* __restrict__ bias,
                                                                    float* __restrict__ parts,
                                                                    const float* __restrict__ xpre = nullptr,
                                                                    const float* __restrict__ chan = nullptr) {
  constexpr int A = Wino<M>::A;
  typedef float vout __attribute__((ext_vector_type(M)));
  __shared__ float red[2 * (kWinoThreads / kWave)];
  const long p_raw = (long)blockIdx.x * kWinoThreads + threadIdx.x;
  const bool live = p_raw < P;
  if (!STATS && !live) return;
  const long p = live ? p_raw : P - 1;
  const int k = blockIdx.y;
  const TileIndex ti = tile_of(p, Th, Tw);
  const size_t plane = (size_t)K * Ps;
  const float* mp = Mt + (size_t)k * Ps + p;
  float s[A][M];
#pragma unroll
  for (int j = 0; j < A; ++j) {
    float m[A];
#pragma unroll
    for (int i = 0; i < A; ++i) m[i] = stream_load<NT>(mp + (size_t)(A * i + j) * plane);
    Wino<M>::out(m, s[j]);
  }
  const size_t yoff = (((size_t)ti.n * K + k) * H + M * ti.th) * W + M * ti.tw;
  float* yp = y + yoff;
  const float b = (STATS && bias) ? bias[k] : 0.0f;
  float sc = 0.0f, sh = 0.0f, mu = 0.0f, rs = 0.0f;
  vout xrow[M];
  const bool hi_in = !RAG || M * ti.tw + 2 < W;
  bool row_in[M];
#pragma unroll
  for (int i = 0; i < M; ++i) row_in[i] = !RAG || M * ti.th + i < H;
  if constexpr (BWD) {
    sc = chan[k]; sh = chan[K + k]; mu = chan[2 * K + k]; rs = chan[3 * K + k];
#pragma unroll
    for (int i = 0; i < M; ++i) {
      if constexpr (RAG) {
        typedef float v2 __attribute__((ext_vector_type(2)));
        v2 lo = {0.0f, 0.0f}, hi = {0.0f, 0.0f};
        if (row_in[i]) {
          lo = *reinterpret_cast<const v2*>(xpre + yoff + (size_t)i * W);
          if (hi_in) hi = *reinterpret_cast<const v2*>(xpre + yoff + (size_t)i * W + 2);
        }
        xrow[i][0] = lo[0]; xrow[i][1] = lo[1]; xrow[i][M - 2] = hi[0]; xrow[i][M - 1] = hi[1];
      } else {
        xrow[i] = *reinterpret_cast<const vout*>(xpre + yoff + (size_t)i * W);
      }
    }
  }
  float a0 = 0.0f, a1 = 0.0f;
#pragma unroll
  for (int i = 0; i < M; ++i) {
    float row[A], o[M];
#pragma unroll
    for (int j = 0; j < A; ++j) row[j] = s[j][i];
    Wino<M>::out(row, o);
    vout ov;
#pragma unroll
    for (int j = 0; j < M; ++j) ov[j] = o[j];
    if constexpr (RAG) {
      typedef float v2 __attribute__((ext_vector_type(2)));
      if (live && row_in[i]) {
        *reinterpret_cast<v2*>(yp + (size_t)i * W) = (v2){o[0], o[1]};
        if (hi_in) *reinterpret_cast<v2*>(yp + (size_t)i * W + 2) = (v2){o[M - 2], o[M - 1]};
      }
    } else {
      if (live) *reinterpret_cast<vout*>(yp + (size_t)i * W) = ov;
    }
    if constexpr (BWD) {
#pragma unroll
      for (int j = 0; j < M; ++j) {
        const bool in = live && row_in[i] && (j < 2 || hi_in);
        const float xv = xrow[i][j] + b;
        const float dz = (in && fma_rn(xv, sc, sh) > 0.0f) ? o[j] : 0.0f;
        a0 += dz;
        a1 = fma_rn(dz, (xv - mu) * rs, a1);
      }
    } else if (STATS) {
#pragma unroll
      for (int j = 0; j < M; ++j) {
        const bool in = live && row_in[i] && (j < 2 || hi_in);
        const float v = in ? o[j] + b : 0.0f;
        a0 += v;
        a1 = fma_rn(v, v, a1);
      }
    }
  }
  if (STATS) {
    a0 = wave_sum(a0);
    a1 = wave_sum(a1);
    const int wave = threadIdx.x / kWave;
    if ((threadIdx.x & (kWave - 1)) == 0) { red[2 * wave] = a0; red[2 * wave + 1] = a1; }
    __syncthreads();
    if (threadIdx.x == 0) {
      float t0 = red[0], t1 = red[1];
#pragma unroll
      for (int w = 1; w < kWinoThreads / kWave; ++w) { t0 += red[2 * w]; t1 += red[2 * w + 1]; }
      float* out = parts + ((size_t)k * gridDim.x + blockIdx.x) * 2;
      out[0] = t0;
      out[1] = t1;
    }
  }
}

template <int M, bool NT = false, bool RAG = false>
__global__ __launch_bounds__(kWinoThreads) void wino_grad_output_kernel(const float* __restrict__ dy, int K, int H,
                                                                         int W, int Th, int Tw, long P, long Ps,
                                                                         float* __restrict__ dM) {
  constexpr int A = Wino<M>::A;
  typedef float vin __attribute__((ext_vector_type(M)));
  const long p = (long)blockIdx.x * kWinoThreads + threadIdx.x;
  const int k = blockIdx.y;
  if (p >= P) {
    if (p < Ps) {
#pragma unroll
      for (int q = 0; q < A * A; ++q) stream_store<NT>(dM + (size_t)k * Ps + p + (size_t)q * (size_t)K * Ps, 0.0f);
    }
    return;
  }
  const TileIndex ti = tile_of(p, Th, Tw);
  const float* yp = dy + (((size_t)ti.n * K + k) * H + M * ti.th) * W + M * ti.tw;
  float yv[M][M];
#pragma unroll
  for (int i = 0; i < M; ++i) {
    if constexpr (RAG) {
      typedef float v2 __attribute__((ext_vector_type(2)));
      v2 lo = {0.0f, 0.0f}, hi = {0.0f, 0.0f};
      if (M * ti.th + i < H) {
        lo = *reinterpret_cast<const v2*>(yp + (size_t)i * W);
        if (M * ti.tw + 2 < W) hi = *reinterpret_cast<const v2*>(yp + (size_t)i * W + 2);
      }
      yv[i][0] = lo[0]; yv[i][1] = lo[1]; yv[i][M - 2] = hi[0]; yv[i][M - 1] = hi[1];
    } else {
      const vin v = *reinterpret_cast<const vin*>(yp + (size_t)i * W);
#pragma unroll
      for (int j = 0; j < M; ++j) yv[i][j] = v[j];
    }
  }
  float r[M][A];
#pragma unroll
  for (int j = 0; j < M; ++j) {
    float col[M];
#pragma unroll
    for (int i = 0; i < M; ++i) col[i] = yv[i][j];
    Wino<M>::gout(col, r[j]);
  }
  const size_t plane = (size_t)K * Ps;
  float* mp = dM + (size_t)k * Ps + p;
#pragma unroll
  for (int i = 0; i < A; ++i) {
    float row[M], o[A];
#pragma unroll
    for (int j = 0; j < M; ++j) row[j] = r[j][i];
    Wino<M>::gout(row, o);
#pragma unroll
    for (int j = 0; j < A; ++j) stream_store<NT>(mp + (size_t)(A * i + j) * plane, o[j]);
  }
}

template <int M>
__device__ __forceinline__ void wino_filter_one(const float* __restrict__ w, int K, int C, int flip, float* __restrict__ U,
                                                long e) {
  constexpr int A = Wino<M>::A;
  const int k = flip ? (int)(e % K) : (int)(e / C), c = flip ? (int)(e / K) : (int)(e % C);
  const float* g = w + ((size_t)k * C + c) * 9;
  float t[3][A];
#pragma unroll
  for (int j = 0; j < 3; ++j) {
    float col[3];
#pragma unroll
    for (int i = 0; i < 3; ++i) col[i] = flip ? g[(2 - i) * 3 + (2 - j)] : g[i * 3 + j];
    Wino<M>::flt(col, t[j]);
  }
  const size_t plane = (size_t)K * C;
  float* up = U + (flip ? (size_t)c * K + k : (size_t)k * C + c);
#pragma unroll
  for (int i = 0; i < A; ++i) {
    float row[3], o[A];
#pragma unroll
    for (int j = 0; j < 3; ++j) row[j] = t[j][i];
    Wino<M>::flt(row, o);
#pragma unroll
    for (int j = 0; j < A; ++j) up[(size_t)(A * i + j) * plane] = o[j];
  }
}

template <int M>
__global__ void wino_filter_kernel(const float* __restrict__ w, int K, int C, int flip, float* __restrict__ U) {
  const long e = (long)blockIdx.x * blockDim.x + threadIdx.x;
  if (e >= (long)K * C) return;
  wino_filter_one<M>(w, K, C, flip, U, e);
}

constexpr int kFilterJobFields = 6;
__global__ __launch_bounds__(256) void wino_filter_batch_kernel(const long long* __restrict__ jobs, int n_jobs) {
  int j = 0;
  while (j + 1 < n_jobs && (long long)blockIdx.x >= jobs[(j + 1) * kFilterJobFields + 5]) ++j;
  const long long* job = jobs + (size_t)j * kFilterJobFields;
  const float* w = reinterpret_cast<const float*>(job[0]);
  float* U = reinterpret_cast<float*>(job[1]);
  const int K = (int)job[2], C = (int)job[3], mf = (int)job[4];
  const long e = ((long)blockIdx.x - (long)job[5]) * 256 + threadIdx.x;
  if (e >= (long)K * C) return;
  if ((mf >> 1) == 2) wino_filter_one<2>(w, K, C, mf & 1, U, e);
  else wino_filter_one<4>(w, K, C, mf & 1, U, e);
}

template <int M>
__global__ void wino_filter_grad_kernel(const float* __restrict__ dU, int K, int C, float* __restrict__ dw) {
  constexpr int A = Wino<M>::A;
  const long e = (long)blockIdx.x * blockDim.x + threadIdx.x;
  if (e >= (long)K * C) return;
  const size_t plane = (size_t)K * C;
  float a[A][3];
#pragma unroll
  for (int j = 0; j < A; ++j) {
    float col[A];
#pragma unroll
    for (int i = 0; i < A; ++i) col[i] = dU[(size_t)(A * i + j) * plane + e];
    Wino<M>::fgrad(col, a[j]);
  }
  float* g = dw + (size_t)e * 9;
#pragma unroll
  for (int i = 0; i < 3; ++i) {
    float row[A], o[3];
#pragma unroll
    for (int j = 0; j < A; ++j) row[j] = a[j][i];
    Wino<M>::fgrad(row, o);
#pragma unroll
    for (int j = 0; j < 3; ++j) g[i * 3 + j] = o[j];
  }
}

inline int tiles_of(int H, int m) { return (H + m - 1) / m; }
inline bool ragged(int m, int H, int W) { return m == 4 && ((H | W) & 3) != 0; }

int check_image(const char* fn, int m, int N, int C, int H, int W) {
  FPSG_REQUIRE(m == 2 || m == 4, FPSG_E_SHAPE, "%s: m must be 2 or 4 (got %d)", fn, m);
  FPSG_REQUIRE(N > 0 && C > 0 && H > 0 && W > 0 && H % 2 == 0 && W % 2 == 0, FPSG_E_SHAPE,
               "%s: N,C positive and H,W positive and even (got %d,%d,%d,%d)", fn, N, C, H, W);
  const long P = (long)N * ((H + m - 1) / m) * ((W + m - 1) / m);
  FPSG_REQUIRE(C <= 65535 && (P + kWinoThreads - 1) / kWinoThreads < (1L << 31), FPSG_E_LIMIT,
               "%s: C=%d or tile count %ld beyond the grid limits", fn, C, P);
  return 0;
}

}
}

#define FPSG_WINO_IMAGE_LAUNCH(KERNEL, CH, ...)                                                              \
  const long P = (long)N * tiles_of(H, m) * tiles_of(W, m);                                                                \
  dim3 grid((unsigned)((P + kWinoThreads - 1) / kWinoThreads), CH);                                          \
  if (m == 2) hipLaunchKernelGGL((KERNEL<2>), grid, dim3(kWinoThreads), 0, static_cast<hipStream_t>(stream), __VA_ARGS__); \
  else hipLaunchKernelGGL((KERNEL<4>), grid, dim3(kWinoThreads), 0, static_cast<hipStream_t>(stream), __VA_ARGS__)

extern "C" int fpsg_wino_input_transform(int m, const float* x, int N, int C, int H, int W, float* V, long ldp,
    fpsg_stream_t stream) {
  using namespace fpsg;
  int rc = check_image("fpsg_wino_input_transform", m, N, C, H, W);
  if (rc) return rc;
  FPSG_REQUIRE_PTR(x); FPSG_REQUIRE_PTR(V);
  FPSG_REQUIRE((reinterpret_cast<uintptr_t>(x) & 15) == 0, FPSG_E_ALIGN, "fpsg_wino_input_transform: x must be 16-byte aligned");
  const long P = (long)N * tiles_of(H, m) * tiles_of(W, m);
  const long Ps = ldp ? ldp : P;
  FPSG_REQUIRE(Ps >= P, FPSG_E_SHAPE, "fpsg_wino_input_transform: row stride %ld must be 0 or at least the %ld tiles", ldp, P);
  dim3 grid((unsigned)((Ps + kWinoThreads - 1) / kWinoThreads), C);
  if (m == 2) hipLaunchKernelGGL((wino_input_kernel<2, false>), grid, dim3(kWinoThreads), 0, static_cast<hipStream_t>(stream), x, C, H, W, tiles_of(H, m), tiles_of(W, m), P, Ps, V, nullptr, nullptr);
  else if (ragged(m, H, W)) hipLaunchKernelGGL((wino_input_kernel<4, false, false, true>), grid, dim3(kWinoThreads), 0, static_cast<hipStream_t>(stream), x, C, H, W, tiles_of(H, m), tiles_of(W, m), P, Ps, V, nullptr, nullptr);
  else if ((size_t)36 * C * Ps * sizeof(float) > kStreamBytes) hipLaunchKernelGGL((wino_input_kernel<4, false, true>), grid, dim3(kWinoThreads), 0, static_cast<hipStream_t>(stream), x, C, H, W, tiles_of(H, m), tiles_of(W, m), P, Ps, V, nullptr, nullptr);
  else hipLaunchKernelGGL((wino_input_kernel<4, false>), grid, dim3(kWinoThreads), 0, static_cast<hipStream_t>(stream), x, C, H, W, tiles_of(H, m), tiles_of(W, m), P, Ps, V, nullptr, nullptr);
  return launch_status("fpsg_wino_input_transform");
}

extern "C" int fpsg_wino_input_transform_act(int m, const float* x, const float* chan, const float* pre_bias, int N,
                                             int C, int H, int W, float* V, long ldp,
    fpsg_stream_t stream) {
  using namespace fpsg;
  int rc = check_image("fpsg_wino_input_transform_act", m, N, C, H, W);
  if (rc) return rc;
  FPSG_REQUIRE_PTR(x); FPSG_REQUIRE_PTR(V); FPSG_REQUIRE_PTR(chan);
  FPSG_REQUIRE(!misaligned4(pre_bias), FPSG_E_ALIGN, "fpsg_wino_input_transform_act: pre_bias not 4-byte aligned");
  FPSG_REQUIRE((reinterpret_cast<uintptr_t>(x) & 15) == 0, FPSG_E_ALIGN, "fpsg_wino_input_transform_act: x must be 16-byte aligned");
  const long P = (long)N * tiles_of(H, m) * tiles_of(W, m);
  const long Ps = ldp ? ldp : P;
  FPSG_REQUIRE(Ps >= P, FPSG_E_SHAPE, "fpsg_wino_input_transform_act: row stride %ld must be 0 or at least the %ld tiles", ldp, P);
  dim3 grid((unsigned)((Ps + kWinoThreads - 1) / kWinoThreads), C);
  if (m == 2) hipLaunchKernelGGL((wino_input_kernel<2, true>), grid, dim3(kWinoThreads), 0, static_cast<hipStream_t>(stream), x, C, H, W, tiles_of(H, m), tiles_of(W, m), P, Ps, V, chan, pre_bias);
  else if (ragged(m, H, W)) hipLaunchKernelGGL((wino_input_kernel<4, true, false, true>), grid, dim3(kWinoThreads), 0, static_cast<hipStream_t>(stream), x, C, H, W, tiles_of(H, m), tiles_of(W, m), P, Ps, V, chan, pre_bias);
  else if ((size_t)36 * C * Ps * sizeof(float) > kStreamBytes) hipLaunchKernelGGL((wino_input_kernel<4, true, true>), grid, dim3(kWinoThreads), 0, static_cast<hipStream_t>(stream), x, C, H, W, tiles_of(H, m), tiles_of(W, m), P, Ps, V, chan, pre_bias);
  else hipLaunchKernelGGL((wino_input_kernel<4, true>), grid, dim3(kWinoThreads), 0, static_cast<hipStream_t>(stream), x, C, H, W, tiles_of(H, m), tiles_of(W, m), P, Ps, V, chan, pre_bias);
  return launch_status("fpsg_wino_input_transform_act");
}

extern "C" int fpsg_wino_output_transform(int m, const float* M, int N, int K, int H, int W, float* y, long ldp,
    fpsg_stream_t stream) {
  using namespace fpsg;
  int rc = check_image("fpsg_wino_output_transform", m, N, K, H, W);
  if (rc) return rc;
  FPSG_REQUIRE_PTR(M); FPSG_REQUIRE_PTR(y);
  FPSG_REQUIRE((reinterpret_cast<uintptr_t>(y) & 15) == 0, FPSG_E_ALIGN, "fpsg_wino_output_transform: y must be 16-byte aligned");
  const long P = (long)N * tiles_of(H, m) * tiles_of(W, m);
  const long Ps = ldp ? ldp : P;
  FPSG_REQUIRE(Ps >= P, FPSG_E_SHAPE, "fpsg_wino_output_transform: row stride %ld must be 0 or at least the %ld tiles", ldp, P);
  dim3 grid((unsigned)((P + kWinoThreads - 1) / kWinoThreads), K);
  hipStream_t hs = static_cast<hipStream_t>(stream);
  if (m == 2) hipLaunchKernelGGL((wino_output_kernel<2, false>), grid, dim3(kWinoThreads), 0, hs, M, K, H, W, tiles_of(H, m), tiles_of(W, m), P, Ps, y, nullptr, nullptr);
  else if (ragged(m, H, W)) hipLaunchKernelGGL((wino_output_kernel<4, false, false, false, true>), grid, dim3(kWinoThreads), 0, hs, M, K, H, W, tiles_of(H, m), tiles_of(W, m), P, Ps, y, nullptr, nullptr);
  else if ((size_t)36 * K * Ps * sizeof(float) > kStreamBytes) hipLaunchKernelGGL((wino_output_kernel<4, false, false, true>), grid, dim3(kWinoThreads), 0, hs, M, K, H, W, tiles_of(H, m), tiles_of(W, m), P, Ps, y, nullptr, nullptr);
  else hipLaunchKernelGGL((wino_output_kernel<4, false>), grid, dim3(kWinoThreads), 0, hs, M, K, H, W, tiles_of(H, m), tiles_of(W, m), P, Ps, y, nullptr, nullptr);
  return launch_status("fpsg_wino_output_transform");
}

extern "C" int fpsg_wino_stats_parts(int m, int N, int H, int W) {
  if ((m != 2 && m != 4) || N <= 0 || H <= 0 || W <= 0 || H % 2 || W % 2) return 0;
  const long P = (long)N * fpsg::tiles_of(H, m) * fpsg::tiles_of(W, m);
  return (int)((P + fpsg::kWinoThreads - 1) / fpsg::kWinoThreads);
}

extern "C" int fpsg_wino_output_transform_stats(int m, const float* M, int N, int K, int H, int W, float* y,
                                                const float* bias, float* parts, long ldp,
    fpsg_stream_t stream) {
  using namespace fpsg;
  int rc = check_image("fpsg_wino_output_transform_stats", m, N, K, H, W);
  if (rc) return rc;
  FPSG_REQUIRE_PTR(M); FPSG_REQUIRE_PTR(y); FPSG_REQUIRE_PTR(parts);
  FPSG_REQUIRE((reinterpret_cast<uintptr_t>(y) & 15) == 0, FPSG_E_ALIGN, "fpsg_wino_output_transform_stats: y must be 16-byte aligned");
  FPSG_REQUIRE(!misaligned4(bias) && !misaligned4(parts), FPSG_E_ALIGN, "fpsg_wino_output_transform_stats: bias / parts not 4-byte aligned");
  const long P = (long)N * tiles_of(H, m) * tiles_of(W, m);
  const long Ps = ldp ? ldp : P;
  FPSG_REQUIRE(Ps >= P, FPSG_E_SHAPE, "fpsg_wino_output_transform_stats: row stride %ld must be 0 or at least the %ld tiles", ldp, P);
  dim3 grid((unsigned)((P + kWinoThreads - 1) / kWinoThreads), K);
  hipStream_t hs = static_cast<hipStream_t>(stream);
  if (m == 2) hipLaunchKernelGGL((wino_output_kernel<2, true>), grid, dim3(kWinoThreads), 0, hs, M, K, H, W, tiles_of(H, m), tiles_of(W, m), P, Ps, y, bias, parts);
  else if (ragged(m, H, W)) hipLaunchKernelGGL((wino_output_kernel<4, true, false, false, true>), grid, dim3(kWinoThreads), 0, hs, M, K, H, W, tiles_of(H, m), tiles_of(W, m), P, Ps, y, bias, parts);
  else if ((size_t)36 * K * Ps * sizeof(float) > kStreamBytes) hipLaunchKernelGGL((wino_output_kernel<4, true, false, true>), grid, dim3(kWinoThreads), 0, hs, M, K, H, W, tiles_of(H, m), tiles_of(W, m), P, Ps, y, bias, parts);
  else hipLaunchKernelGGL((wino_output_kernel<4, true>), grid, dim3(kWinoThreads), 0, hs, M, K, H, W, tiles_of(H, m), tiles_of(W, m), P, Ps, y, bias, parts);
  return launch_status("fpsg_wino_output_transform_stats");
}

extern "C" int fpsg_wino_output_transform_bwd_stats(int m, const float* M, int N, int K, int H, int W, float* y,
                                                    const float* xpre, const float* pre_bias, const float* chan,
                                                    float* parts, long ldp,
    fpsg_stream_t stream) {
  using namespace fpsg;
  int rc = check_image("fpsg_wino_output_transform_bwd_stats", m, N, K, H, W);
  if (rc) return rc;
  FPSG_REQUIRE_PTR(M); FPSG_REQUIRE_PTR(y); FPSG_REQUIRE_PTR(parts); FPSG_REQUIRE_PTR(xpre); FPSG_REQUIRE_PTR(chan);
  FPSG_REQUIRE(((reinterpret_cast<uintptr_t>(y) | reinterpret_cast<uintptr_t>(xpre)) & 15) == 0, FPSG_E_ALIGN,
               "fpsg_wino_output_transform_bwd_stats: y and xpre must be 16-byte aligned");
  FPSG_REQUIRE(!misaligned4(pre_bias) && !misaligned4(parts) && !misaligned4(chan), FPSG_E_ALIGN,
               "fpsg_wino_output_transform_bwd_stats: pre_bias / chan / parts not 4-byte aligned");
  const long P = (long)N * tiles_of(H, m) * tiles_of(W, m);
  const long Ps = ldp ? ldp : P;
  FPSG_REQUIRE(Ps >= P, FPSG_E_SHAPE, "fpsg_wino_output_transform_bwd_stats: row stride %ld must be 0 or at least the %ld tiles", ldp, P);
  dim3 grid((unsigned)((P + kWinoThreads - 1) / kWinoThreads), K);
  hipStream_t hs = static_cast<hipStream_t>(stream);
  if (m == 2) hipLaunchKernelGGL((wino_output_kernel<2, true, true>), grid, dim3(kWinoThreads), 0, hs, M, K, H, W, tiles_of(H, m), tiles_of(W, m), P, Ps, y, pre_bias, parts, xpre, chan);
  else if (ragged(m, H, W)) hipLaunchKernelGGL((wino_output_kernel<4, true, true, false, true>), grid, dim3(kWinoThreads), 0, hs, M, K, H, W, tiles_of(H, m), tiles_of(W, m), P, Ps, y, pre_bias, parts, xpre, chan);
  else if ((size_t)36 * K * Ps * sizeof(float) > kStreamBytes) hipLaunchKernelGGL((wino_output_kernel<4, true, true, true>), grid, dim3(kWinoThreads), 0, hs, M, K, H, W, tiles_of(H, m), tiles_of(W, m), P, Ps, y, pre_bias, parts, xpre, chan);
  else hipLaunchKernelGGL((wino_output_kernel<4, true, true>), grid, dim3(kWinoThreads), 0, hs, M, K, H, W, tiles_of(H, m), tiles_of(W, m), P, Ps, y, pre_bias, parts, xpre, chan);
  return launch_status("fpsg_wino_output_transform_bwd_stats");
}

extern "C" int fpsg_wino_grad_output_transform(int m, const float* dy, int N, int K, int H, int W, float* dM, long ldp,
    fpsg_stream_t stream) {
  using namespace fpsg;
  int rc = check_image("fpsg_wino_grad_output_transform", m, N, K, H, W);
  if (rc) return rc;
  FPSG_REQUIRE_PTR(dy); FPSG_REQUIRE_PTR(dM);
  FPSG_REQUIRE((reinterpret_cast<uintptr_t>(dy) & 15) == 0, FPSG_E_ALIGN, "fpsg_wino_grad_output_transform: dy must be 16-byte aligned");
  const long P = (long)N * tiles_of(H, m) * tiles_of(W, m);
  const long Ps = ldp ? ldp : P;
  FPSG_REQUIRE(Ps >= P, FPSG_E_SHAPE, "fpsg_wino_grad_output_transform: row stride %ld must be 0 or at least the %ld tiles", ldp, P);
  dim3 grid((unsigned)((Ps + kWinoThreads - 1) / kWinoThreads), K);
  hipStream_t hs = static_cast<hipStream_t>(stream);
  if (m == 2) hipLaunchKernelGGL((wino_grad_output_kernel<2>), grid, dim3(kWinoThreads), 0, hs, dy, K, H, W, tiles_of(H, m), tiles_of(W, m), P, Ps, dM);
  else if (ragged(m, H, W)) hipLaunchKernelGGL((wino_grad_output_kernel<4, false, true>), grid, dim3(kWinoThreads), 0, hs, dy, K, H, W, tiles_of(H, m), tiles_of(W, m), P, Ps, dM);
  else if ((size_t)36 * K * Ps * sizeof(float) > kStreamBytes) hipLaunchKernelGGL((wino_grad_output_kernel<4, true>), grid, dim3(kWinoThreads), 0, hs, dy, K, H, W, tiles_of(H, m), tiles_of(W, m), P, Ps, dM);
  else hipLaunchKernelGGL((wino_grad_output_kernel<4>), grid, dim3(kWinoThreads), 0, hs, dy, K, H, W, tiles_of(H, m), tiles_of(W, m), P, Ps, dM);
  return launch_status("fpsg_wino_grad_output_transform");
}

extern "C" int fpsg_wino_grad_transforms(int m, const float* dy, int N, int K, int H, int W, float* V, float* dM, long ldp,
    fpsg_stream_t stream) {
  using namespace fpsg;
  int rc = check_image("fpsg_wino_grad_transforms", m, N, K, H, W);
  if (rc) return rc;
  FPSG_REQUIRE_PTR(dy); FPSG_REQUIRE_PTR(V); FPSG_REQUIRE_PTR(dM);
  FPSG_REQUIRE((reinterpret_cast<uintptr_t>(dy) & 15) == 0, FPSG_E_ALIGN, "fpsg_wino_grad_transforms: dy must be 16-byte aligned");
  const long P = (long)N * tiles_of(H, m) * tiles_of(W, m);
  const long Ps = ldp ? ldp : P;
  FPSG_REQUIRE(Ps >= P, FPSG_E_SHAPE, "fpsg_wino_grad_transforms: row stride %ld must be 0 or at least the %ld tiles", ldp, P);
  dim3 grid((unsigned)((Ps + kWinoThreads - 1) / kWinoThreads), K);
  hipStream_t hs = static_cast<hipStream_t>(stream);
  if (m == 2) hipLaunchKernelGGL((wino_input_kernel<2, false, false, false, true>), grid, dim3(kWinoThreads), 0, hs, dy, K, H, W, tiles_of(H, m), tiles_of(W, m), P, Ps, V, nullptr, nullptr, dM);
  else if (ragged(m, H, W)) hipLaunchKernelGGL((wino_input_kernel<4, false, false, true, true>), grid, dim3(kWinoThreads), 0, hs, dy, K, H, W, tiles_of(H, m), tiles_of(W, m), P, Ps, V, nullptr, nullptr, dM);
  else if ((size_t)36 * K * Ps * sizeof(float) > kStreamBytes) hipLaunchKernelGGL((wino_input_kernel<4, false, true, false, true>), grid, dim3(kWinoThreads), 0, hs, dy, K, H, W, tiles_of(H, m), tiles_of(W, m), P, Ps, V, nullptr, nullptr, dM);
  else hipLaunchKernelGGL((wino_input_kernel<4, false, false, false, true>), grid, dim3(kWinoThreads), 0, hs, dy, K, H, W, tiles_of(H, m), tiles_of(W, m), P, Ps, V, nullptr, nullptr, dM);
  return launch_status("fpsg_wino_grad_transforms");
}

extern "C" int fpsg_wino_filter_transform(int m, const float* w, int K, int C, int flip_transpose, float* U,
                                          fpsg_stream_t stream) {
  using namespace fpsg;
  FPSG_REQUIRE(m == 2 || m == 4, FPSG_E_SHAPE, "fpsg_wino_filter_transform: m must be 2 or 4 (got %d)", m);
  FPSG_REQUIRE(K > 0 && C > 0, FPSG_E_SHAPE, "fpsg_wino_filter_transform: K,C must be positive (got %d,%d)", K, C);
  FPSG_REQUIRE_PTR(w); FPSG_REQUIRE_PTR(U);
  const long n = (long)K * C;
  dim3 grid((unsigned)((n + 255) / 256));
  if (m == 2) hipLaunchKernelGGL(wino_filter_kernel<2>, grid, dim3(256), 0, static_cast<hipStream_t>(stream), w, K, C, flip_transpose, U);
  else hipLaunchKernelGGL(wino_filter_kernel<4>, grid, dim3(256), 0, static_cast<hipStream_t>(stream), w, K, C, flip_transpose, U);
  return launch_status("fpsg_wino_filter_transform");
}

extern "C" int fpsg_wino_filter_transform_batch(const int64_t* jobs, int n_jobs, long total_blocks, fpsg_stream_t stream) {
  using namespace fpsg;
  FPSG_REQUIRE(n_jobs > 0 && total_blocks > 0 && total_blocks < (1L << 31), FPSG_E_SHAPE,
               "fpsg_wino_filter_transform_batch: n_jobs and total_blocks must be positive (got %d, %ld)", n_jobs, total_blocks);
  FPSG_REQUIRE_PTR(jobs);
  hipLaunchKernelGGL(wino_filter_batch_kernel, dim3((unsigned)total_blocks), dim3(256), 0, static_cast<hipStream_t>(stream),
                     reinterpret_cast<const long long*>(jobs), n_jobs);
  return launch_status("fpsg_wino_filter_transform_batch");
}

extern "C" int fpsg_wino_filter_grad_transform(int m, const float* dU, int K, int C, float* dw, fpsg_stream_t stream) {
  using namespace fpsg;
  FPSG_REQUIRE(m == 2 || m == 4, FPSG_E_SHAPE, "fpsg_wino_filter_grad_transform: m must be 2 or 4 (got %d)", m);
  FPSG_REQUIRE(K > 0 && C > 0, FPSG_E_SHAPE, "fpsg_wino_filter_grad_transform: K,C must be positive (got %d,%d)", K, C);
  FPSG_REQUIRE_PTR(dU); FPSG_REQUIRE_PTR(dw);
  const long n = (long)K * C;
  dim3 grid((unsigned)((n + 255) / 256));
  if (m == 2) hipLaunchKernelGGL(wino_filter_grad_kernel<2>, grid, dim3(256), 0, static_cast<hipStream_t>(stream), dU, K, C, dw);
  else hipLaunchKernelGGL(wino_filter_grad_kernel<4>, grid, dim3(256), 0, static_cast<hipStream_t>(stream), dU, K, C, dw);
  return launch_status("fpsg_wino_filter_grad_transform");
}
```

fpsg_amd/image_net.py:

```python
from __future__ import annotations

import os

import torch
import torch.nn as nn

from . import winograd
from .fused_bn import (_conv_without_bias, bn_act, bn_act_of, bn_act_pool_of, conv_bn_act, conv_bn_act_pool,
                       foldable_into, fusable_conv, wants_conv_stats)

_VGG16_PLAN = (64, 64, "P", 128, 128, "P", 256, 256, 256, "P", 512, 512, 512, "P", 512, 512,
               512, "P")


def vgg16_bn_trunk() -> nn.Sequential:
    layers = []
    c_in = 3
    for item in _VGG16_PLAN:
        if item == "P":
            layers.append(nn.MaxPool2d(kernel_size=2, stride=2))
            continue
        conv = nn.Conv2d(c_in, item, kernel_size=3, padding=1)
        nn.init.kaiming_normal_(conv.weight, mode="fan_out", nonlinearity="relu")
        nn.init.zeros_(conv.bias)
        layers += [conv, nn.BatchNorm2d(item), nn.ReLU(inplace=True)]
        c_in = item
    return nn.Sequential(*layers)


class ImageEncoderWarpper(nn.Module):

    def __init__(self, core: str = "vgg_16", finetune_layer: int = 0, weights: str | None = None):
        super().__init__()
        if core != "vgg_16":
            raise NotImplementedError(f"Unsupported Image Encoder Core Compoenent: {core}")
        self.finetune_layer = finetune_layer
        self.img_feature_extractor = vgg16_bn_trunk()
        self.img_feature_pool = nn.AdaptiveAvgPool2d(output_size=(1, 1))
        if weights:
            self.load_trunk(weights)

    def load_trunk(self, path: str) -> None:
        if not os.path.exists(path):
            raise FileNotFoundError(path)
        sd = torch.load(path, map_location="cpu", weights_only=True)
        if any(k.startswith("features.") for k in sd):
            sd = {k[len("features."):]: v for k, v in sd.items() if k.startswith("features.")}
        elif any(k.startswith("img_feature_extractor.") for k in sd):
            sd = {k[len("img_feature_extractor."):]: v for k, v in sd.items()
                  if k.startswith("img_feature_extractor.")}
        self.img_feature_extractor.load_state_dict(sd)

    def forward(self, x: torch.Tensor) -> torch.Tensor:
        layers = list(self.img_feature_extractor)
        i = 0
        pending = None
        while i < len(layers):
            layer = layers[i]
            triple = (isinstance(layer, nn.Conv2d) and i + 2 < len(layers) and isinstance(layers[i + 1], nn.BatchNorm2d)
                      and isinstance(layers[i + 2], nn.ReLU))
            if triple and (pending is not None or fusable_conv(layer, layers[i + 1], x)):
                bn = layers[i + 1]
                want = wants_conv_stats(layer, bn, x)
                parts = None
                nxt3 = layers[i + 3] if i + 5 < len(layers) else None
                if (pending is None and i == 0 and isinstance(nxt3, nn.Conv2d) and isinstance(layers[i + 4], nn.BatchNorm2d)
                        and isinstance(layers[i + 5], nn.ReLU) and fusable_conv(nxt3, layers[i + 4], x)
                        and winograd.stem_applies(x, layer, bn, nxt3)):
                    i += 3
                    layer, bn = nxt3, layers[i + 1]
                    want = bn.training and winograd.stats_enabled()
                    y = winograd.stem_conv_bn_relu_conv(x, layers[0], layers[1], layer, want_parts=want)
                elif pending is not None:
                    py, pconv, pbn, pparts = pending
                    y = winograd.bn_relu_conv3x3(py, pconv.bias, pbn, layer.weight, parts=pparts,
                                                 stats_bias=layer.bias, want_parts=want)
                    pending = None
                else:
                    y = _conv_without_bias(layer, x, want)
                if want:
                    y, parts = y
                nxt = layers[i + 3] if i + 3 < len(layers) else None
                next_is_triple = (isinstance(nxt, nn.Conv2d) and i + 5 < len(layers)
                                  and isinstance(layers[i + 4], nn.BatchNorm2d) and isinstance(layers[i + 5], nn.ReLU))
                if isinstance(nxt, nn.MaxPool2d):
                    x = bn_act_pool_of(y, layer, bn, nxt, "relu", parts)
                    i += 4
                elif next_is_triple and fusable_conv(nxt, layers[i + 4], y) and foldable_into(y, bn, nxt):
                    pending = (y, layer, bn, parts)
                    x = y
                    i += 3
                else:
                    x = bn_act_of(y, layer, bn, "relu")
                    i += 3
            elif triple:
                if i + 3 < len(layers) and isinstance(layers[i + 3], nn.MaxPool2d):
                    x = conv_bn_act_pool(layer, layers[i + 1], layers[i + 3], x, "relu")
                    i += 4
                else:
                    x = conv_bn_act(layer, layers[i + 1], x, "relu")
                    i += 3
            elif isinstance(layer, nn.BatchNorm2d) and i + 1 < len(layers) and isinstance(layers[i + 1], nn.ReLU):
                x = bn_act(layer, x, "relu")
                i += 2
            else:
                x = layer(x)
                i += 1
        return self.img_feature_pool(x).flatten(1)

    def _set_finetune(self, new_layer: int | None = None) -> None:
        if new_layer is not None:
            self.finetune_layer = new_layer
        budget = self.finetune_layer
        for layer in reversed(self.img_feature_extractor):
            if isinstance(layer, nn.Conv2d):
                layer.requires_grad_(budget > 0)
                budget -= 1 if budget > 0 else 0
```

fpsg_amd/winograd.py:

```python
from __future__ import annotations

import os

import torch

from . import _hip, gemm_split
from .bn_counters import count_batch

MIN_CHANNELS_M4 = 64
MIN_CHANNELS_M2 = 128
MIN_WIDE_CHANNELS_M2 = 256


def enabled() -> bool:
    return os.environ.get("FPSG_WINOGRAD", "1") != "0"


def _eligible_layer(conv: torch.nn.Conv2d, H: int, W: int) -> bool:
    def is_(v, want):
        return v == want or v == (want, want)
    return (enabled() and is_(conv.kernel_size, 3) and is_(conv.stride, 1) and is_(conv.padding, 1) and is_(conv.dilation, 1)
            and conv.groups == 1 and conv.padding_mode == "zeros" and H % 2 == 0 and W % 2 == 0
            and _wide_enough(conv.in_channels, conv.out_channels, tile_size(H, W)))

# ... 38 lines not shown
            and c_out % 16 == 0 and H % 4 == 0 and W % 16 == 0 and N * max(c_in, c_out) * H * W * 4 < (1 << 31)
            and N * (H // 4) * (W // 4) >= MIN_DW_TILES)


def _fused_dw(x, chan, pre_bias, gy):
    N, C, H, W = x.shape
    K = gy.shape[1]
    lib = _hip.load()
    dU = torch.empty((36, K, C), dtype=torch.float32, device=x.device)
    ws = torch.empty((lib.fpsg_wino_dw_fused_workspace_floats(N, K, H, W),), dtype=torch.float32, device=x.device)
    opt = lambda t: _hip.ptr(t) if t is not None else None
    _call("fpsg_wino_dw_fused", _hip.ptr(x), opt(chan), opt(pre_bias), _hip.ptr(gy), N, C, K, H, W, _hip.ptr(dU),
          _hip.ptr(ws), _hip.stream_of(x))
    return dU


def _wide_enough(c_in: int, c_out: int, m: int) -> bool:
    lo, hi = min(c_in, c_out), max(c_in, c_out)
    return lo >= MIN_CHANNELS_M4 if m == 4 else (lo >= MIN_CHANNELS_M2 and hi >= MIN_WIDE_CHANNELS_M2)


def _call(name, *args):
    _hip.check(getattr(_hip.load(), name)(*args), name)


def _bmm(A, B):
    if gemm_split.enabled() and min(A.shape[1], A.shape[2]) >= 128 and A.is_cuda:
        return gemm_split.bmm_split(A.contiguous(), B.contiguous(), False)
    return torch.bmm(A, B)


def _bmm_nt(A, B):
    if gemm_split.enabled() and min(A.shape[1], B.shape[1]) >= 128 and A.is_cuda:
        return gemm_split.bmm_split(A.contiguous(), B.contiguous(), True)
    return torch.bmm(A, B.transpose(1, 2))


_frozen_cache = None


class _FilterBank:

    MAX_ENTRIES = 96

    def __init__(self):
        self.entries = {}
        self.table = None
        self.valid = False

    def register(self, key, w, U):
        if len(self.entries) < self.MAX_ENTRIES:
            self.entries[key] = [w, U, w.shape[0], w.shape[1], True, False]
            self.table = None

    def lookup(self, key, w, capturing):
        ent = self.entries.get(key) if self.valid else None
        if ent is None or ent[2] != w.shape[0] or ent[3] != w.shape[1] or ent[1].device != w.device:
            return None
        ent[4] = True
        ent[5] = ent[5] or capturing
        return ent[1]

    def has_pinned(self) -> bool:
        return any(e[5] for e in self.entries.values())

    def refresh(self):
        self.valid = False
        stale = [k for k, e in self.entries.items() if not (e[4] or e[5])]
        for k in stale:
            del self.entries[k]
        if stale:
            self.table = None
        if not self.entries:
            return
        if self.table is None:
            per_dev = {}
            for (ptr, m, flip), (w, U, K, C, _, _) in self.entries.items():
                rows, first = per_dev.setdefault(U.device, [[], 0])
                rows.append([ptr, U.data_ptr(), K, C, 2 * m + (1 if flip else 0), first])
                per_dev[U.device][1] = first + (K * C + 255) // 256
            self.table = [(dev, torch.tensor(rows, dtype=torch.int64).to(dev), blocks)
                          for dev, (rows, blocks) in per_dev.items()]
        for e in self.entries.values():
            e[4] = False
        for dev, table, blocks in self.table:
            with torch.cuda.device(dev):
                _call("fpsg_wino_filter_transform_batch", _hip.ptr(table), table.shape[0], blocks,
                      torch.cuda.current_stream(dev).cuda_stream)
        self.valid = True


_bank = _FilterBank()


def check_bank_before_replay() -> None:
    if _bank.has_pinned() and not _bank.valid:
        raise RuntimeError("hipGraph replay outside a refreshed winograd.weights_frozen() block: the captured "
                           "episode reads transformed filters that were not recomputed for the current weights")


def filter_bank_enabled() -> bool:
    return os.environ.get("FPSG_FILTER_BANK", "1") != "0"


class _ReadOnlyView:

    def __init__(self, d):
        self._d = d

    def __contains__(self, k):
        return k in self._d

    def __getitem__(self, k):
        return self._d[k]

    def get(self, k, default=None):
        return self._d.get(k, default)

    def __setitem__(self, k, v):
        pass

    def __iter__(self):
        return iter(self._d)


_frozen_constant = False


class weights_frozen:

    def __init__(self, constant: bool = False):
        self._constant = bool(constant)

    def __enter__(self):
        global _frozen_cache, _frozen_constant
        self._outer = _frozen_cache
        self._outer_constant = _frozen_constant
        _frozen_constant = self._constant or (_frozen_constant and _frozen_cache is not None)
        _frozen_cache = {} if _frozen_cache is None else _frozen_cache
        if self._outer is None and (filter_bank_enabled() or _bank.has_pinned()) and torch.cuda.is_available() \
                and not torch.cuda.is_current_stream_capturing():
            _bank.refresh()
        return self

    def __exit__(self, *exc):
        global _frozen_cache, _frozen_constant
        _frozen_cache = self._outer
        _frozen_constant = self._outer_constant
        if self._outer is None:
            _bank.valid = False
        return False


def frozen_cache():
    if _frozen_cache is None:
        return None
    if torch.cuda.is_available() and torch.cuda.is_current_stream_capturing():
        return _ReadOnlyView(_frozen_cache) if _frozen_constant else None
    return _frozen_cache


def frozen_cache_ro():
    return _frozen_cache


def eval_chan(gamma, beta, running_mean, running_var, eps, C, dev):
    cache = _frozen_cache
    if cache is None or running_mean is None or running_var is None or os.environ.get("FPSG_EVAL_CHAN_CACHE", "1") == "0":
        return torch.empty((4, C), dtype=torch.float32, device=dev), 0
    key = ("bn_chan", running_mean.data_ptr(), running_var.data_ptr(), gamma.data_ptr() if gamma is not None else 0,
           beta.data_ptr() if beta is not None else 0, float(eps))
    chan = cache.get(key)
    if chan is not None:
        return chan, 2
    chan = torch.empty((4, C), dtype=torch.float32, device=dev)
    if dev.type != "cuda" or torch.cuda.is_current_stream_capturing():
        return chan, 0
    opt = lambda t: _hip.ptr(t) if t is not None else None
    with torch.cuda.device(dev):
        _call("fpsg_bn_stats", _hip.ptr(chan), None, opt(gamma), opt(beta), _hip.ptr(running_mean), _hip.ptr(running_var),
              0.0, 1, C, 1, 0, float(eps), _hip.ptr(chan), None, None, None, None, 0,
              torch.cuda.current_stream(dev).cuda_stream)
    cache[key] = chan
    return chan, 2


def _filter(m, w, flip):
    key = (w.data_ptr(), m, bool(flip))
    capturing = w.is_cuda and torch.cuda.is_current_stream_capturing()
    banked = _bank.lookup(key, w, capturing)
    if banked is not None:
        return banked
    cache = _frozen_cache
    if cache is not None and capturing:
        cache = _ReadOnlyView(cache) if _frozen_constant else None
    if cache is not None and key in cache:
        return cache[key]
    K, C = w.shape[0], w.shape[1]
    a2 = (m + 2) ** 2
    U = torch.empty((a2, C, K) if flip else (a2, K, C), dtype=torch.float32, device=w.device)
    _call("fpsg_wino_filter_transform", m, _hip.ptr(w), K, C, 1 if flip else 0, _hip.ptr(U), _hip.stream_of(w))
    if cache is not None and not capturing:
        cache[key] = U
        if filter_bank_enabled():
            _bank.register(key, w.detach(), U)
    return U


def row_stride(P: int) -> int:
    a = int(os.environ.get("FPSG_WINO_ROW_ALIGN", "32"))
    if a < 1 or a > 1024:
        raise ValueError(f"FPSG_WINO_ROW_ALIGN must be in 1 .. 1024 (got {a})")
    return (P + a - 1) // a * a


def _ldp(T, N, H, W, m):
    if not T.is_contiguous() or T.shape[2] < N * _tiles(H, W, m):
        raise ValueError(f"transform-domain tensor {tuple(T.shape)} must be contiguous with at least "
                         f"{N * _tiles(H, W, m)} columns")
    return T.shape[2]


def _input(m, x):
    N, C, H, W = x.shape
    Ps = row_stride(N * _tiles(H, W, m))
    V = torch.empty(((m + 2) ** 2, C, Ps), dtype=torch.float32, device=x.device)
    _call("fpsg_wino_input_transform", m, _hip.ptr(x), N, C, H, W, _hip.ptr(V), Ps, _hip.stream_of(x))
    return V


def stats_enabled() -> bool:
    return os.environ.get("FPSG_CONV_STATS", "1") != "0"


_BN_SMALL_MAX = 16384


def bwd_stats_enabled() -> bool:
    return os.environ.get("FPSG_CONV_BWD_STATS", "1") != "0"


def _output_bwd_stats(m, M, N, H, W, xpre, pre_bias, chan):
    K = M.shape[1]
    y = torch.empty((N, K, H, W), dtype=torch.float32, device=M.device)
    S = _hip.load().fpsg_wino_stats_parts(m, N, H, W)
    parts = torch.empty((K, S, 2), dtype=torch.float32, device=M.device)
    _call("fpsg_wino_output_transform_bwd_stats", m, _hip.ptr(M), N, K, H, W, _hip.ptr(y), _hip.ptr(xpre),
          _hip.ptr(pre_bias) if pre_bias is not None else None, _hip.ptr(chan), _hip.ptr(parts), _ldp(M, N, H, W, m),
          _hip.stream_of(M))
    return y, parts


def _output(m, M, N, H, W, stats_bias=None, want_parts=False):
    K = M.shape[1]
    y = torch.empty((N, K, H, W), dtype=torch.float32, device=M.device)
    if not want_parts:
        _call("fpsg_wino_output_transform", m, _hip.ptr(M), N, K, H, W, _hip.ptr(y), _ldp(M, N, H, W, m), _hip.stream_of(M))
        return y
    S = _hip.load().fpsg_wino_stats_parts(m, N, H, W)
    parts = torch.empty((K, S, 2), dtype=torch.float32, device=M.device)
    _call("fpsg_wino_output_transform_stats", m, _hip.ptr(M), N, K, H, W, _hip.ptr(y),
          _hip.ptr(stats_bias) if stats_bias is not None else None, _hip.ptr(parts), _ldp(M, N, H, W, m), _hip.stream_of(M))
    return y, parts


def _fused_stats(x, chan, pre_bias, U, stats_bias):
    N, C, H, W = x.shape
    K = U.shape[1]
    y = torch.empty((N, K, H, W), dtype=torch.float32, device=x.device)
    S = _hip.load().fpsg_wino_conv_fused_parts(N, K, H, W)
    parts = torch.empty((K, S, 2), dtype=torch.float32, device=x.device)
    opt = lambda t: _hip.ptr(t) if t is not None else None
    _call("fpsg_wino_conv_fused_stats", _hip.ptr(x), opt(chan), opt(pre_bias), _hip.ptr(U), N, C, K, H, W, _hip.ptr(y),
          opt(stats_bias), _hip.ptr(parts), _hip.stream_of(x))
    return y, parts


def _fused(x, U):
    N, C, H, W = x.shape
    K = U.shape[1]
    y = torch.empty((N, K, H, W), dtype=torch.float32, device=x.device)
    _call("fpsg_wino_conv_fused", _hip.ptr(x), _hip.ptr(U), N, C, K, H, W, _hip.ptr(y), _hip.stream_of(x))
    return y


def _grad_output(m, gy):
    N, K, H, W = gy.shape
    Ps = row_stride(N * _tiles(H, W, m))
    dM = torch.empty(((m + 2) ** 2, K, Ps), dtype=torch.float32, device=gy.device)
    _call("fpsg_wino_grad_output_transform", m, _hip.ptr(gy), N, K, H, W, _hip.ptr(dM), Ps, _hip.stream_of(gy))
    return dM


def grad_transforms_enabled() -> bool:
    return os.environ.get("FPSG_GRAD_TRANSFORMS", "1") != "0"


def _grad_transforms(m, gy):
    N, K, H, W = gy.shape
    Ps = row_stride(N * _tiles(H, W, m))
    V = torch.empty(((m + 2) ** 2, K, Ps), dtype=torch.float32, device=gy.device)
    dM = torch.empty_like(V)
    _call("fpsg_wino_grad_transforms", m, _hip.ptr(gy), N, K, H, W, _hip.ptr(V), _hip.ptr(dM), Ps, _hip.stream_of(gy))
    return V, dM


def _filter_grad(m, dU, like):
    gw = torch.empty_like(like)
    _call("fpsg_wino_filter_grad_transform", m, _hip.ptr(dU), like.shape[0], like.shape[1], _hip.ptr(gw),
          _hip.stream_of(dU))
    return gw


class _Conv3x3(torch.autograd.Function):

    @staticmethod
    def forward(ctx, x, w, m, stats_bias=None, want_parts=False):
        ctx.set_materialize_grads(False)
        x, w = x.contiguous(), w.contiguous()
        N, C, H, W = x.shape
        K = w.shape[0]
        parts = None
        with torch.cuda.device(x.device):
            if _can_fuse(m, C, K, N * H * W, H, W):
                if want_parts:
                    y, parts = _fused_stats(x, None, None, _filter(m, w, False), stats_bias)
                else:
                    y = _fused(x, _filter(m, w, False))
                keep, kept_is_v = x, False
            else:
                V = _input(m, x)
                Mt = _bmm(_filter(m, w, False), V)
                if want_parts:
                    y, parts = _output(m, Mt, N, H, W, stats_bias, True)
                else:
                    y = _output(m, Mt, N, H, W)
                keep, kept_is_v = V, True
        ctx.save_for_backward(keep if ctx.needs_input_grad[1] else None, w)
        ctx.dims = (N, C, H, W, m, kept_is_v)
        if not want_parts:
            return y
        if parts is not None:
            ctx.mark_non_differentiable(parts)
        return y, parts

    @staticmethod
    def backward(ctx, gy, _gparts=None):
        if gy is None:
            return None, None, None, None, None
        kept, w = ctx.saved_tensors
        N, C, H, W, m, kept_is_v = ctx.dims
        K = w.shape[0]
        gy = gy.contiguous()
        gx = gw = None
        with torch.cuda.device(gy.device):
            fuse_dx = _can_fuse(m, K, C, N * H * W, H, W)
            fuse_dw = not kept_is_v and _can_fuse_dw(m, C, K, N, H, W)
            Vg = dM = None
            if (ctx.needs_input_grad[0] and ctx.needs_input_grad[1] and not fuse_dx and not fuse_dw
                    and grad_transforms_enabled()):
                Vg, dM = _grad_transforms(m, gy)
            if ctx.needs_input_grad[0]:
                if fuse_dx:
                    gx = _fused(gy, _filter(m, w, True))
                else:
                    gx = _output(m, _bmm(_filter(m, w, True), Vg if Vg is not None else _input(m, gy)), N, H, W)
                    Vg = None
            if ctx.needs_input_grad[1]:
                if fuse_dw:
                    gw = _filter_grad(m, _fused_dw(kept, None, None, gy), w)
                else:
                    V = kept if kept_is_v else _input(m, kept)
                    gw = _filter_grad(m, _bmm_nt(dM if dM is not None else _grad_output(m, gy), V), w)
        return gx, gw, None, None, None


def _input_act(m, x, chan, pre_bias):
    N, C, H, W = x.shape
    Ps = row_stride(N * _tiles(H, W, m))
    V = torch.empty(((m + 2) ** 2, C, Ps), dtype=torch.float32, device=x.device)
    _call("fpsg_wino_input_transform_act", m, _hip.ptr(x), _hip.ptr(chan), _hip.ptr(pre_bias) if pre_bias is not None else None,
          N, C, H, W, _hip.ptr(V), Ps, _hip.stream_of(x))
    return V


def _fused_act(x, chan, pre_bias, U):
    N, C, H, W = x.shape
    K = U.shape[1]
    y = torch.empty((N, K, H, W), dtype=torch.float32, device=x.device)
    _call("fpsg_wino_conv_fused_act", _hip.ptr(x), _hip.ptr(chan), _hip.ptr(pre_bias) if pre_bias is not None else None,
          _hip.ptr(U), N, C, K, H, W, _hip.ptr(y), _hip.stream_of(x))
    return y


def fold_enabled() -> bool:
    return os.environ.get("FPSG_BN_FOLD", "1") != "0"


class _BNReluConv3x3(torch.autograd.Function):

    @staticmethod
    def forward(ctx, y, pre_bias, gamma, beta, running_mean, running_var, training, momentum, eps, w, m, parts=None,
                stats_bias=None, want_parts=False):
        ctx.set_materialize_grads(False)
        y, w = y.contiguous(), w.contiguous()
        N, C, H, W = y.shape
        K = w.shape[0]
        lib = _hip.load()
        dev = y.device
        chan, mode = (torch.empty((4, C), dtype=torch.float32, device=dev), 1) if training else \
            eval_chan(gamma, beta, running_mean, running_var, eps, C, dev)
        use_parts = parts is not None and training
        ws = None if (use_parts or mode == 2) else torch.empty((lib.fpsg_bn_workspace_floats(N, C, H * W),), dtype=torch.float32, device=dev)
        opt = lambda t: _hip.ptr(t) if t is not None else None
        out_parts = None
        with torch.cuda.device(dev):
            if mode != 2:
                _call("fpsg_bn_stats", _hip.ptr(y), opt(pre_bias), opt(gamma), opt(beta), opt(running_mean), opt(running_var),
                      float(momentum), N, C, H * W, 1 if training else 0, float(eps), _hip.ptr(chan), None, None,
                      opt(ws), _hip.ptr(parts) if use_parts else None, parts.shape[1] if use_parts else 0,
                      _hip.stream_of(y))
            if _can_fuse(m, C, K, N * H * W, H, W):
                if want_parts:
                    out, out_parts = _fused_stats(y, chan, pre_bias, _filter(m, w, False), stats_bias)
                else:
                    out = _fused_act(y, chan, pre_bias, _filter(m, w, False))
                V = None
            else:
                V = _input_act(m, y, chan, pre_bias)
                Mt = _bmm(_filter(m, w, False), V)
                if want_parts:
                    out, out_parts = _output(m, Mt, N, H, W, stats_bias, True)
                else:
                    out = _output(m, Mt, N, H, W)
        ctx.save_for_backward(y, chan, pre_bias, w, V if ctx.needs_input_grad[9] else None)
        ctx.cfg = (N, C, H, W, m, bool(training), gamma is not None, beta is not None)
        if not want_parts:
            return out
        if out_parts is not None:
            ctx.mark_non_differentiable(out_parts)
        return out, out_parts

    @staticmethod
    def backward(ctx, gout, _gparts=None):
        if gout is None:
            return (None,) * 14
        y, chan, pre_bias, w, V = ctx.saved_tensors
        N, C, H, W, m, training, has_g, has_b = ctx.cfg
        K = w.shape[0]
        lib = _hip.load()
        dev = y.device
        gout = gout.contiguous()
        gw = None
        with torch.cuda.device(dev):
            bwd_parts = None
            fuse_dx = _can_fuse(m, K, C, N * H * W, H, W)
            fuse_dw = V is None and _can_fuse_dw(m, C, K, N, H, W)
            Vg = dM = None
            if ctx.needs_input_grad[9] and not fuse_dx and not fuse_dw and grad_transforms_enabled():
                Vg, dM = _grad_transforms(m, gout)
            if fuse_dx:
                ga = _fused(gout, _filter(m, w, True))
            elif bwd_stats_enabled() and N * H * W > _BN_SMALL_MAX:
                ga, bwd_parts = _output_bwd_stats(m, _bmm(_filter(m, w, True), Vg if Vg is not None else _input(m, gout)),
                                                  N, H, W, y, pre_bias, chan)
            else:
                ga = _output(m, _bmm(_filter(m, w, True), Vg if Vg is not None else _input(m, gout)), N, H, W)
            Vg = None
            if ctx.needs_input_grad[9]:
                if fuse_dw:
                    gw = _filter_grad(m, _fused_dw(y, chan, pre_bias, gout), w)
                else:
                    if V is None:
                        V = _input_act(m, y, chan, pre_bias)
                    gw = _filter_grad(m, _bmm_nt(dM if dM is not None else _grad_output(m, gout), V), w)
            want_dpb = pre_bias is not None and ctx.needs_input_grad[1]
            dy = torch.empty_like(y)
            dgamma = torch.empty((C,), dtype=torch.float32, device=dev)
            dbeta = torch.empty((C,), dtype=torch.float32, device=dev)
            dpb = torch.empty((C,), dtype=torch.float32, device=dev) if want_dpb else None
            coef = torch.empty((3, C), dtype=torch.float32, device=dev)
            ws = torch.empty((lib.fpsg_bn_workspace_floats(N, C, H * W),), dtype=torch.float32, device=dev)
            if bwd_parts is not None:
                _call("fpsg_bn_act_bwd_parts", _hip.ptr(y), _hip.ptr(pre_bias) if pre_bias is not None else None,
                      _hip.ptr(ga), _hip.ptr(chan), N, C, H * W, 1 if training else 0, 1, 0.0, _hip.ptr(dy),
                      _hip.ptr(dgamma), _hip.ptr(dbeta), _hip.ptr(dpb) if want_dpb else None, _hip.ptr(coef),
                      _hip.ptr(ws), _hip.ptr(bwd_parts), bwd_parts.shape[1], _hip.stream_of(y))
            else:
                _call("fpsg_bn_act_bwd", _hip.ptr(y), _hip.ptr(pre_bias) if pre_bias is not None else None, _hip.ptr(ga),
                      _hip.ptr(chan), N, C, H * W, 1 if training else 0, 1, 0.0, _hip.ptr(dy), _hip.ptr(dgamma),
                      _hip.ptr(dbeta), _hip.ptr(dpb) if want_dpb else None, _hip.ptr(coef), _hip.ptr(ws), _hip.stream_of(y))
        return (dy, dpb, dgamma if has_g else None, dbeta if has_b else None, None, None, None, None, None, gw, None,
                None, None, None)


def stem_fold_enabled() -> bool:
    return os.environ.get("FPSG_STEM_FOLD", "1") != "0"


class _StemConvBNReluConv(torch.autograd.Function):

    @staticmethod
    def forward(ctx, x, w1, b1, gamma, beta, running_mean, running_var, momentum, eps, w2, m, stats_bias=None,
                want_parts=False):
        from . import conv_first
        ctx.set_materialize_grads(False)
        y1, parts1 = conv_first._forward(x, w1, b1, True)
        N, C, H, W = y1.shape
        K = w2.shape[0]
        lib = _hip.load()
        dev = y1.device
        chan = torch.empty((4, C), dtype=torch.float32, device=dev)
        opt = lambda t: _hip.ptr(t) if t is not None else None
        out_parts = None
        w2c = w2.contiguous()
        with torch.cuda.device(dev):
            _call("fpsg_bn_stats", _hip.ptr(y1), opt(b1), opt(gamma), opt(beta), opt(running_mean), opt(running_var),
                  float(momentum), N, C, H * W, 1, float(eps), _hip.ptr(chan), None, None, None, _hip.ptr(parts1),
                  parts1.shape[1], _hip.stream_of(y1))
            if _can_fuse(m, C, K, N * H * W, H, W):
                if want_parts:
                    out, out_parts = _fused_stats(y1, chan, b1, _filter(m, w2c, False), stats_bias)
                else:
                    out = _fused_act(y1, chan, b1, _filter(m, w2c, False))
                V = None
            else:
                V = _input_act(m, y1, chan, b1)
                Mt = _bmm(_filter(m, w2c, False), V)
                if want_parts:
                    out, out_parts = _output(m, Mt, N, H, W, stats_bias, True)
                else:
                    out = _output(m, Mt, N, H, W)
        ctx.save_for_backward(x, w1, y1, chan, b1, w2c, V if ctx.needs_input_grad[9] else None)
        ctx.cfg = (N, C, H, W, m, gamma is not None, beta is not None)
        if not want_parts:
            return out
        if out_parts is not None:
            ctx.mark_non_differentiable(out_parts)
        return out, out_parts

    @staticmethod
    def backward(ctx, gout, _gparts=None):
        if gout is None:
            return (None,) * 13
        x, w1, y1, chan, b1, w2, V = ctx.saved_tensors
        N, C, H, W, m, has_g, has_b = ctx.cfg
        K = w2.shape[0]
        lib = _hip.load()
        dev = y1.device
        gout = gout.contiguous()
        gw1 = gw2 = db1 = None
        with torch.cuda.device(dev):
            if _can_fuse(m, K, C, N * H * W, H, W):
                ga = _fused(gout, _filter(m, w2, True))
            else:
                ga = _output(m, _bmm(_filter(m, w2, True), _input(m, gout)), N, H, W)
            if ctx.needs_input_grad[9]:
                if V is None and _can_fuse_dw(m, C, K, N, H, W):
                    gw2 = _filter_grad(m, _fused_dw(y1, chan, b1, gout), w2)
                else:
                    if V is None:
                        V = _input_act(m, y1, chan, b1)
                    gw2 = _filter_grad(m, _bmm_nt(_grad_output(m, gout), V), w2)
            dgamma = torch.empty((C,), dtype=torch.float32, device=dev)
            dbeta = torch.empty((C,), dtype=torch.float32, device=dev)
            coef = torch.empty((3, C), dtype=torch.float32, device=dev)
            ws = torch.empty((lib.fpsg_bn_workspace_floats(N, C, H * W),), dtype=torch.float32, device=dev)
            _call("fpsg_bn_act_bwd_coef", _hip.ptr(y1), _hip.ptr(b1), _hip.ptr(ga), _hip.ptr(chan), N, C, H * W, 1, 1, 0.0,
                  _hip.ptr(dgamma), _hip.ptr(dbeta), _hip.ptr(coef), _hip.ptr(ws), _hip.stream_of(y1))
            if ctx.needs_input_grad[1]:
                gw1 = torch.empty_like(w1, memory_format=torch.contiguous_format)
                ws1 = torch.empty((lib.fpsg_conv_first_dw_workspace_floats(N, H, W),), dtype=torch.float32, device=dev)
                xc = x.contiguous()
                _call("fpsg_conv_first_dw_fold", _hip.ptr(xc), _hip.ptr(y1), _hip.ptr(ga), _hip.ptr(chan), _hip.ptr(coef),
                      _hip.ptr(b1), N, 3, 64, H, W, _hip.ptr(gw1), _hip.ptr(ws1), _hip.stream_of(y1))
            if ctx.needs_input_grad[2]:
                db1 = torch.zeros((C,), dtype=torch.float32, device=dev)
        return (None, gw1, db1, dgamma if has_g else None, dbeta if has_b else None, None, None, None, None, gw2, None,
                None, None)


def stem_applies(x, conv1, bn1, conv2) -> bool:
    from . import conv_first
    if not (stem_fold_enabled() and fold_enabled() and bn1.training and bn1.track_running_stats and stats_enabled()):
        return False
    if x.requires_grad or not conv_first.eligible(x, conv1) or os.environ.get("FPSG_CONV_FIRST_FWD", "1") == "0":
        return False
    if conv1.bias is None or conv2.bias is None or x.shape[0] * x.shape[2] * x.shape[3] <= _BN_SMALL_MAX:
        return False
    return (isinstance(conv2, torch.nn.Conv2d) and conv2.in_channels == 64
            and _eligible_layer(conv2, x.shape[2], x.shape[3]))


def stem_conv_bn_relu_conv(x, conv1, bn1, conv2, want_parts=False):
    count_batch(bn1)
    mom = 0.1 if bn1.momentum is None else float(bn1.momentum)
    m = tile_size(x.shape[2], x.shape[3])
    return _StemConvBNReluConv.apply(x.contiguous(), conv1.weight, conv1.bias, bn1.weight, bn1.bias, bn1.running_mean,
                                     bn1.running_var, mom, bn1.eps, conv2.weight, m, conv2.bias, bool(want_parts))


def bn_relu_conv3x3(y, pre_bias, bn, weight, m=None, parts=None, stats_bias=None, want_parts=False):
    if m is None:
        m = tile_size(y.shape[2], y.shape[3])
    training = bn.training
    if training:
        count_batch(bn)
    mom = (0.1 if bn.momentum is None else float(bn.momentum)) if training else -1.0
    return _BNReluConv3x3.apply(y, pre_bias, bn.weight, bn.bias, bn.running_mean, bn.running_var, bool(training), mom,
                                bn.eps, weight, m, parts, stats_bias, bool(want_parts))


def conv3x3(x: torch.Tensor, weight: torch.Tensor, m: int | None = None, stats_bias=None, want_parts: bool = False):
    if x.dim() != 4 or weight.dim() != 4 or tuple(weight.shape[2:]) != (3, 3) or weight.shape[1] != x.shape[1]:
        raise ValueError(f"conv3x3: x {tuple(x.shape)} / weight {tuple(weight.shape)}")
    if m is None:
        m = tile_size(x.shape[2], x.shape[3])
    if m not in (2, 4) or x.shape[2] % 2 or x.shape[3] % 2:
        raise ValueError(f"conv3x3: m={m} must be 2 or 4 and H, W even (got {tuple(x.shape[2:])})")
    if want_parts:
        return _Conv3x3.apply(x, weight, m, stats_bias, True)
    return _Conv3x3.apply(x, weight, m)
```

include/fpsg_hip.h:

```cpp
#ifndef FPSG_HIP_H
#define FPSG_HIP_H

#include <stddef.h>
#include <stdint.h>

#ifdef __cplusplus
extern "C" {
#endif

typedef void* fpsg_stream_t;

#define FPSG_ABI_VERSION 1

#define FPSG_E_NULL   (-1)
#define FPSG_E_SHAPE  (-2)
#define FPSG_E_ALIGN  (-3)
#define FPSG_E_LIMIT  (-4)

int         fpsg_version(void);
const char* fpsg_last_error(void);

int fpsg_chamfer_fwd(const float* xyz1, const float* xyz2, int B, int N, int M,
                     float* dist1, int32_t* idx1, float* dist2, int32_t* idx2,
                     fpsg_stream_t stream);

int fpsg_chamfer_fwd_variant(const float* xyz1, const float* xyz2, int B, int N, int M,
                             float* dist1, int32_t* idx1, float* dist2, int32_t* idx2,
                             int cfg, fpsg_stream_t stream);

size_t fpsg_chamfer_workspace_bytes(int B, int N, int M, int variant);
int fpsg_chamfer_fwd_tiled(const float* xyz1, const float* xyz2, int B, int N, int M,
                           float* dist1, int32_t* idx1, float* dist2, int32_t* idx2,
                           void* ws, size_t ws_bytes, int variant, fpsg_stream_t stream);
int fpsg_chamfer_fwd_tiled_losses(const float* xyz1, const float* xyz2, int B, int N, int M,
                                  float* dist1, int32_t* idx1, float* dist2, int32_t* idx2,
                                  void* ws, size_t ws_bytes, int variant, int n_first, float w_first,
                                  float w_rest, float* out3, fpsg_stream_t stream);

int fpsg_chamfer_bwd(const float* xyz1, const float* xyz2,
                     const int32_t* idx1, const int32_t* idx2,
                     const float* g1, const float* g2,
                     int B, int N, int M,
                     float* gxyz1, float* gxyz2, fpsg_stream_t stream);
int fpsg_chamfer_bwd_sorted(const float* xyz1, const float* xyz2,
                            const int32_t* idx1, const int32_t* idx2,
                            const float* g1, const float* g2,
                            int B, int N, int M,
                            float* gxyz1, float* gxyz2, fpsg_stream_t stream);
int fpsg_chamfer_bwd_scan(const float* xyz1, const float* xyz2,
                          const int32_t* idx1, const int32_t* idx2,
                          const float* g1, const float* g2,
                          int B, int N, int M,
                          float* gxyz1, float* gxyz2, fpsg_stream_t stream);

int fpsg_chamfer_losses(const float* dist1, const float* dist2, int B, int N, int M, int n_first,
                        float w_first, float w_rest, float* out3, fpsg_stream_t stream);
int fpsg_chamfer_loss_grads(const float* g_first, const float* g_rest, const float* g_total, int B, int N, int M,
                            int n_first, float w_first, float w_rest, float* g1, float* g2, fpsg_stream_t stream);
int fpsg_chamfer_bwd_losses(const float* xyz1, const float* xyz2, const int32_t* idx1, const int32_t* idx2,
                            const float* g_first, const float* g_rest, const float* g_total,
                            int B, int N, int M, int n_first, float w_first, float w_rest,
                            float* gxyz1, float* gxyz2, fpsg_stream_t stream);

#define FPSG_KNN_CHANNEL_MAJOR 0
#define FPSG_KNN_POINT_MAJOR   1
#define FPSG_KNN_FORCE_TILE    1
#define FPSG_KNN_FORCE_SLOW    2
size_t fpsg_knn_workspace_floats(int B, int C, int N);
int fpsg_knn(const float* x, int B, int C, int N, int k, int32_t* idx, float* ws,
             fpsg_stream_t stream);
int fpsg_knn_ex(const float* x, int layout, int B, int C, int N, int k, int32_t* idx, float* ws,
                int flags, fpsg_stream_t stream);

int fpsg_edge_feature_fwd(const float* x, const int32_t* idx, int B, int C, int N, int k,
                          float* out, fpsg_stream_t stream);

int fpsg_edge_feature_bwd(const float* gout, const int32_t* idx, int B, int C, int N, int k,
                          float* gx, fpsg_stream_t stream);

size_t fpsg_emd_workspace_floats(int B, int N, int M);
int fpsg_emd_approx(const float* xyz1, const float* xyz2, int B, int N, int M, float* cost,
                    float* gxyz1, float* gxyz2, float* ws, fpsg_stream_t stream);
int fpsg_emd_approx_variant(const float* xyz1, const float* xyz2, int B, int N, int M, float* cost,
                            float* gxyz1, float* gxyz2, float* ws, int variant, fpsg_stream_t stream);

#define FPSG_EMD_EXACT_MAX_N 2048
size_t fpsg_emd_exact_workspace_floats(int B, int N);
int fpsg_emd_exact(const float* xyz1, const float* xyz2, int B, int N, float eps_final, int max_rounds,
                   float* cost, float* gap, int* assign, int* status,
                   float* gxyz1, float* gxyz2, float* ws, fpsg_stream_t stream);

#define FPSG_CHAMFER_CROSS_MAX_N 4096
int fpsg_chamfer_cross(const float* xyz1, const float* xyz2, int Na, int Nb, int N, int M, float* out,
                       fpsg_stream_t stream);

int fpsg_edgeconv_blocks(int B, int N, int Co);
int fpsg_edgeconv_fwd(const float* PQ, const int32_t* idx, const float* sgn, int B, int N, int k,
                      int Co, float* ysel, uint8_t* jsel, float* s1, float* part,
                      fpsg_stream_t stream);
int fpsg_edgeconv_bwd(const float* dzs, const uint8_t* jsel, const float* PQ, const float* s1,
                      const int32_t* rev, const int32_t* off, const float* coef, int B, int N, int k,
                      int Co, float* dPQ, fpsg_stream_t stream);

int fpsg_edgeconv_reverse_graph_fits(int N, int k);
int fpsg_edgeconv_reverse_graph(const int32_t* idx, int B, int N, int k, int32_t* rev, int32_t* off,
                                fpsg_stream_t stream);
int fpsg_edgeconv_prep_blocks(long rows);
int fpsg_edgeconv_stats_finalize(const float* part, int blocks, const float* gamma, const float* beta,
                                 float* running_mean, float* running_var, float momentum, float eps, double count, int Co,
                                 int training, float* chan, fpsg_stream_t stream);
size_t fpsg_edgeconv_stats_ws_floats(int blocks, int Co);
int fpsg_edgeconv_stats_finalize_ws(const float* part, int blocks, const float* gamma, const float* beta,
                                    float* running_mean, float* running_var, float momentum, float eps, double count,
                                    int Co, int training, float* chan, float* ws, fpsg_stream_t stream);
int fpsg_edgeconv_bwd_finalize(const float* part, int blocks, const float* chan, double count, int Co, int training,
                               float* dgamma, float* dbeta, float* coef, fpsg_stream_t stream);
int fpsg_edgeconv_act(const float* ysel, const float* scale, const float* shift, float slope, long rows, int Co,
                      float* out, fpsg_stream_t stream);
int fpsg_edgeconv_bwd_prep(const float* g, const float* ysel, const float* scale, const float* shift, float slope,
                           long rows, int Co, float* dzs, float* part, fpsg_stream_t stream);

int fpsg_softmin(const float* x, const float* y, const float* h, int B, int N, int M, float eps,
                 float* out, fpsg_stream_t stream);

size_t fpsg_sinkhorn_workspace_floats(int B, int N, int M);
int fpsg_sinkhorn_divergence(const float* x, const float* y, int B, int N, int M,
                             const float* eps_host, int n_eps, float* out, float* ws,
                             fpsg_stream_t stream);

int fpsg_dec1_tiles(int D);
int fpsg_dec1_fwd(const float* hlat, const float* w, int ldw, int wofs, const float* pts,
                  const float* gamma, const float* beta, const float* running_mean, const float* running_var,
                  int G, int D, int B, int P, int training, float eps, float* out, float* chan,
                  float* batch_mean, float* batch_var_unbiased, fpsg_stream_t stream);
int fpsg_dec1_bwd(const float* dout, const float* hlat, const float* w, int ldw, int wofs, const float* pts,
                  const float* chan, int G, int D, int B, int P, int training, float* dhlat, float* dw,
                  float* dpts_part, float* dgamma, float* dbeta, fpsg_stream_t stream);

int fpsg_dec1_fwd_ld(const float* hlat, int ld_hlat, const float* w, int ldw, int wofs, const float* pts, int ld_pts,
                     const float* gamma, const float* beta, const float* running_mean, const float* running_var,
                     int G, int D, int B, int P, int training, float eps, float* out, int ld_out, float* chan,
                     float* batch_mean, float* batch_var_unbiased, fpsg_stream_t stream);
int fpsg_dec1_bwd_ld(const float* dout, int ld_dout, const float* hlat, int ld_hlat, const float* w, int ldw, int wofs,
                     const float* pts, int ld_pts, const float* chan, int G, int D, int B, int P, int training,
                     int accumulate, float* dhlat, float* dw, float* dpts_part, float* dgamma, float* dbeta,
                     fpsg_stream_t stream);

size_t fpsg_bn_workspace_floats(int N, int C, int L);
int fpsg_bn_act_fwd(const float* x, const float* pre_bias, const float* gamma, const float* beta,
                    float* running_mean, float* running_var, float momentum, int N, int C, int L, int training,
                    float eps, int act, float slope, float* y, float* chan, float* batch_mean,
                    float* batch_var_unbiased, float* ws, fpsg_stream_t stream);
int fpsg_bn_stats(const float* x, const float* pre_bias, const float* gamma, const float* beta,
                  float* running_mean, float* running_var, float momentum, int N, int C, int L, int training,
                  float eps, float* chan, float* batch_mean, float* batch_var_unbiased, float* ws,
                  const float* parts, int n_parts, fpsg_stream_t stream);
int fpsg_bn_act_bwd(const float* x, const float* pre_bias, const float* dy, const float* chan, int N, int C,
                    int L, int training, int act, float slope, float* dx, float* dgamma, float* dbeta,
                    float* dpre_bias, float* coef, float* ws, fpsg_stream_t stream);
int fpsg_bn_act_bwd_coef(const float* x, const float* pre_bias, const float* dy, const float* chan, int N, int C,
                         int L, int training, int act, float slope, float* dgamma, float* dbeta, float* coef,
                         float* ws, fpsg_stream_t stream);
int fpsg_bn_act_rows_fwd(const float* x, int ld, const int* seg_off, const int* seg_len, int nseg,
                         const float* pre_bias, const float* gamma, const float* beta, int C, float eps, int act,
                         float slope, float* y, float* chan, float* stats, fpsg_stream_t stream);
int fpsg_bn_act_rows_bwd(const float* x, int ld, const int* seg_off, const int* seg_len, int nseg,
                         const float* pre_bias, const float* dy, const float* chan, int C, int act, float slope,
                         float* dx, float* dgamma, float* dbeta, float* dpre_bias, fpsg_stream_t stream);
int fpsg_bn_act_bwd_parts(const float* x, const float* pre_bias, const float* dy, const float* chan, int N,
                          int C, int L, int training, int act, float slope, float* dx, float* dgamma,
                          float* dbeta, float* dpre_bias, float* coef, float* ws, const float* parts,
                          int n_parts, fpsg_stream_t stream);

size_t fpsg_bn_pool_workspace_floats(int N, int C, int H, int W);
int fpsg_bn_act_pool_fwd(const float* x, const float* pre_bias, const float* gamma, const float* beta,
                         float* running_mean, float* running_var, float momentum, int N, int C, int H, int W,
                         int training, float eps, int act, float slope, float* y_pooled, float* chan,
                         float* batch_mean, float* batch_var_unbiased, float* ws, const float* parts, int n_parts,
                         fpsg_stream_t stream);
int fpsg_bn_act_pool_bwd(const float* x, const float* pre_bias, const float* dy_pooled, const float* chan,
                         int N, int C, int H, int W, int training, int act, float slope, float* dx,
                         float* dgamma, float* dbeta, float* dpre_bias, float* coef, float* ws,
                         fpsg_stream_t stream);

size_t fpsg_bn_max_workspace_floats(int N, int C, int L);
size_t fpsg_bn_max_dz_offset(int N, int C, int L);
int fpsg_bn_act_max_fwd(const float* x, const float* pre_bias, const float* gamma, const float* beta,
                        float* running_mean, float* running_var, float momentum, int N, int C, int L, int training,
                        float eps, int act, float slope, float* out, int32_t* idx, float* chan, float* batch_mean,
                        float* batch_var_unbiased, float* ws, fpsg_stream_t stream);
int fpsg_bn_act_max_bwd(const float* x, const float* pre_bias, const float* gout, const int32_t* idx,
                        const float* chan, int N, int C, int L, int training, int act, float slope, float* dx,
                        float* dgamma, float* dbeta, float* dpre_bias, float* coef, float* ws, fpsg_stream_t stream);
int fpsg_bn_act_max_bwd_coef(const float* x, const float* pre_bias, const float* gout, const int32_t* idx,
                             const float* chan, int N, int C, int L, int training, int act, float slope,
                             float* dgamma, float* dbeta, float* coef, float* ws, fpsg_stream_t stream);

int fpsg_max_bwd_gather(const float* a, const float* dz, const int32_t* idx, int B, int K, int C, int L, float* S,
                        float* spart , fpsg_stream_t stream);
int fpsg_max_bwd_prep(const float* W, const float* coef, const float* pre_bias, const float* mean, const float* dz,
                      const float* spart, int B, int K, int C, int L, float* Wk, float* u, float* dpre_bias, float* s,
                      fpsg_stream_t stream);
int fpsg_max_bwd_dw(const float* S, const float* WG, const float* coef, const float* pre_bias, const float* s, int B,
                    int K, int C, float* dw, fpsg_stream_t stream);
size_t fpsg_max_bwd_scatter_workspace_floats(int B, int C, int L);
int fpsg_max_bwd_scatter(float* da, const float* W, const float* k1, const float* dz, const int32_t* idx, const float* v,
                         int B, int K, int C, int L, float* ws, fpsg_stream_t stream);


int fpsg_wino_input_transform(int m, const float* x, int N, int C, int H, int W, float* V, long ldp,
                              fpsg_stream_t stream);
int fpsg_wino_output_transform(int m, const float* M, int N, int K, int H, int W, float* y, long ldp,
                               fpsg_stream_t stream);
int fpsg_wino_stats_parts(int m, int N, int H, int W);
int fpsg_wino_output_transform_stats(int m, const float* M, int N, int K, int H, int W, float* y, const float* bias,
                                     float* parts, long ldp, fpsg_stream_t stream);
int fpsg_wino_output_transform_bwd_stats(int m, const float* M, int N, int K, int H, int W, float* y,
                                         const float* xpre, const float* pre_bias, const float* chan,
                                         float* parts, long ldp, fpsg_stream_t stream);
int fpsg_wino_grad_output_transform(int m, const float* dy, int N, int K, int H, int W, float* dM, long ldp,
                                    fpsg_stream_t stream);
int fpsg_wino_grad_transforms(int m, const float* dy, int N, int K, int H, int W, float* V, float* dM, long ldp,
                              fpsg_stream_t stream);
int fpsg_wino_filter_transform(int m, const float* w, int K, int C, int flip_transpose, float* U,
                               fpsg_stream_t stream);
int fpsg_wino_filter_transform_batch(const int64_t* jobs, int n_jobs, long total_blocks, fpsg_stream_t stream);
int fpsg_wino_filter_grad_transform(int m, const float* dU, int K, int C, float* dw, fpsg_stream_t stream);

size_t fpsg_gemm_split_workspace_floats(int batch, int M, int N, int K, int transB, int variant);
int fpsg_gemm_split(const float* A, const float* B, float* C, int batch, int M, int N, int K, int lda, int ldb, int ldc,
                    long sA, long sB, long sC, int transB, int variant, float* ws, size_t ws_floats,
                    fpsg_stream_t stream);

size_t fpsg_gemm_split_packed_a_bytes(int batch, int M, int K, int variant);
int fpsg_gemm_split_pack_a(const float* A, int batch, int M, int K, int lda, long sA, int variant, void* Ap,
                           fpsg_stream_t stream);
int fpsg_gemm_split_nn_packed(const void* Ap, const float* B, float* C, int batch, int M, int N, int K, int ldb, int ldc,
                              long sB, long sC, int variant, fpsg_stream_t stream);

int fpsg_gemm_split_nn_persistent(const void* Ap, const float* B, float* C, int batch, int M, int N, int K, int ldb, int ldc,
                                  long sB, long sC, int variant, fpsg_stream_t stream);

int fpsg_gemm_f32_nn(const float* A, const float* B, float* C, int batch, int M, int N, int K, int lda, int ldb, int ldc,
                     long sA, long sB, long sC, int variant, fpsg_stream_t stream);

int fpsg_wino_conv_fused(const float* x, const float* U, int N, int C, int K, int H, int W, float* y,
                         fpsg_stream_t stream);

int fpsg_wino_conv_fused_parts(int N, int K, int H, int W);
int fpsg_wino_conv_fused_stats(const float* x, const float* chan, const float* pre_bias, const float* U, int N, int C,
                               int K, int H, int W, float* y, const float* out_bias, float* parts, fpsg_stream_t stream);

size_t fpsg_wino_dw_fused_workspace_floats(int N, int K, int H, int W);
int fpsg_wino_dw_fused(const float* x, const float* chan, const float* pre_bias, const float* dy, int N, int C, int K,
                       int H, int W, float* dU, float* ws, fpsg_stream_t stream);

int fpsg_wino_input_transform_act(int m, const float* x, const float* chan, const float* pre_bias, int N, int C,
                                  int H, int W, float* V, long ldp, fpsg_stream_t stream);
int fpsg_wino_conv_fused_act(const float* x, const float* chan, const float* pre_bias, const float* U, int N, int C,
                             int K, int H, int W, float* y, fpsg_stream_t stream);

size_t fpsg_conv_first_dw_workspace_floats(int N, int H, int W);
int fpsg_conv_first_dw(const float* x, const float* dy, int N, int C, int K, int H, int W, float* dw, float* ws,
                       fpsg_stream_t stream);
int fpsg_conv_first_dw_fold(const float* x, const float* y, const float* ga, const float* chan, const float* coef,
                            const float* pre_bias, int N, int C, int K, int H, int W, float* dw, float* ws,
                            fpsg_stream_t stream);
int fpsg_conv_first_parts(int N, int H, int W);
int fpsg_conv_first_fwd(const float* x, const float* w, int N, int C, int K, int H, int W, float* y, const float* bias,
                        float* parts, fpsg_stream_t stream);

int fpsg_adam_step(float* param, const float* grad, float* exp_avg, float* exp_avg_sq, size_t n, float lr,
                   float beta1, float beta2, float eps, int step, float grad_scale, fpsg_stream_t stream);
int fpsg_adam_step_segments(float* param, const float* const* grad_ptrs, const long long* seg_off, int nseg,
                            float* exp_avg, float* exp_avg_sq, size_t n, float lr, float beta1, float beta2,
                            float eps, int step, float grad_scale, fpsg_stream_t stream);
int fpsg_flat_accumulate_segments(float* flat, const float* const* grad_ptrs, const long long* seg_off, int nseg,
                                  size_t n, int accumulate, fpsg_stream_t stream);
int fpsg_flat_accumulate_tables(float* flat, const float* const* grad_ptrs, const long long* seg_off, int nseg, int ntab,
                                size_t n, int accumulate, fpsg_stream_t stream);

#ifdef __cplusplus
}
#endif
#endif
```

Measured before the change: 46.06.

## Fold BatchNorm-ReLU backward into the Winograd gradient input transform across conv chains

Adds a stage-chain autograd function that runs consecutive conv-BN-ReLU layers as a single node, so that each BN backward no longer writes out a full dx tensor. Instead the BN/ReLU backward (dz masking plus the k1/k2/k3 coefficients) is computed inside the Winograd gradient input transform, which reads ga and y directly. The dpre_bias reduction is taken from per-tile partial sums written by the same kernel. This removes a full-tensor write and re-read per layer, at the cost of a second input stream, more registers in the transform kernel, and a more complex autograd path that does not support retain_graph.

```diff
diff --git a/fpsg_amd/_hip.py b/fpsg_amd/_hip.py
--- a/fpsg_amd/_hip.py
+++ b/fpsg_amd/_hip.py
@@ -94,6 +94,9 @@
                              _c_f32p, _c_f32p, _c_f32p, _c_f32p, _c_stream],
     "fpsg_bn_act_bwd_parts": [_c_f32p, _c_f32p, _c_f32p, _c_f32p, _c_int, _c_int, _c_int, _c_int, _c_int,
                         ctypes.c_float, _c_f32p, _c_f32p, _c_f32p, _c_f32p, _c_f32p, _c_f32p, _c_f32p, _c_int, _c_stream],
+    "fpsg_bn_act_bwd_parts_coef": [_c_f32p, _c_int, _c_int, _c_int, _c_int, _c_f32p, _c_f32p, _c_f32p, _c_f32p, _c_int,
+                                   _c_stream],
+    "fpsg_bn_dxsum_vec": [_c_f32p, _c_int, _c_int, _c_int, _c_f32p, _c_f32p, _c_stream],
     "fpsg_bn_pool_workspace_floats": [_c_int, _c_int, _c_int, _c_int],
     "fpsg_bn_act_pool_fwd": [_c_f32p, _c_f32p, _c_f32p, _c_f32p, _c_f32p, _c_f32p, ctypes.c_float, _c_int, _c_int, _c_int, _c_int,
                              _c_int, ctypes.c_float, _c_int, ctypes.c_float, _c_f32p, _c_f32p, _c_f32p, _c_f32p,
@@ -123,6 +126,8 @@
                                          ctypes.c_long, _c_stream],
     "fpsg_wino_grad_output_transform": [_c_int, _c_f32p, _c_int, _c_int, _c_int, _c_int, _c_f32p, ctypes.c_long, _c_stream],
     "fpsg_wino_grad_transforms": [_c_int, _c_f32p, _c_int, _c_int, _c_int, _c_int, _c_f32p, _c_f32p, ctypes.c_long, _c_stream],
+    "fpsg_wino_grad_transforms_bnbwd": [_c_int, _c_f32p, _c_f32p, _c_f32p, _c_f32p, _c_f32p, _c_int, _c_int, _c_int, _c_int,
+                                        _c_f32p, _c_f32p, _c_f32p, ctypes.c_long, _c_stream],
     "fpsg_wino_filter_transform": [_c_int, _c_f32p, _c_int, _c_int, _c_int, _c_f32p, _c_stream],
     "fpsg_wino_output_transform_bwd_stats": [_c_int, _c_f32p, _c_int, _c_int, _c_int, _c_int, _c_f32p, _c_f32p, _c_f32p,
                                              _c_f32p, _c_f32p, ctypes.c_long, _c_stream],
diff --git a/fpsg_amd/csrc/bnact.hip b/fpsg_amd/csrc/bnact.hip
--- a/fpsg_amd/csrc/bnact.hip
+++ b/fpsg_amd/csrc/bnact.hip
@@ -321,6 +321,25 @@
   if (threadIdx.x == 0) dpb[c] = (float)a;
 }
 
+__global__ __launch_bounds__(kBnThreads) void bn_vecsum_kernel(const float* __restrict__ vsum, int L,
+                                                               float* __restrict__ dxpart) {
+  __shared__ float red[8];
+  const int row = blockIdx.x, seg = blockIdx.y;
+  float acc = 0.0f, unused = 0.0f;
+  const int len = (L - seg * kBnSeg) < kBnSeg ? (L - seg * kBnSeg) : kBnSeg;
+  const float* __restrict__ vp = vsum + ((size_t)row * L + (size_t)seg * kBnSeg) / 4;
+  const int nvec = len / 4;
+  for (int e0 = threadIdx.x; e0 < nvec; e0 += kBnU * kBnThreads) {
+#pragma unroll
+    for (int j = 0; j < kBnU; ++j) {
+      const int e = e0 + j * kBnThreads;
+      if (e < nvec) acc += vp[e];
+    }
+  }
+  block_reduce2(acc, unused, red);
+  if (threadIdx.x == 0) dxpart[(size_t)row * gridDim.y + seg] = acc;
+}
+
 constexpr int kBnSmallMax = 16384;
 
 constexpr int kBnMaxSegs = 4;
@@ -1235,6 +1254,36 @@
     return launch_status("fpsg_bn_act_bwd_parts(dpre_bias)");
   }
   return 0;
+}
+
+extern "C" int fpsg_bn_act_bwd_parts_coef(const float* chan, int N, int C, int L, int training, float* dgamma,
+                                          float* dbeta, float* coef, const float* parts, int n_parts,
+                                          fpsg_stream_t stream) {
+  using namespace fpsg;
+  int rc = check_dims("fpsg_bn_act_bwd_parts_coef", N, C, L, kActRelu);
+  if (rc) return rc;
+  FPSG_REQUIRE_PTR(chan); FPSG_REQUIRE_PTR(parts); FPSG_REQUIRE_PTR(dgamma); FPSG_REQUIRE_PTR(dbeta);
+  FPSG_REQUIRE_PTR(coef);
+  FPSG_REQUIRE(n_parts > 0, FPSG_E_SHAPE, "fpsg_bn_act_bwd_parts_coef: n_parts must be positive (got %d)", n_parts);
+  hipLaunchKernelGGL(bn_bwd_finalize_kernel, dim3(C), dim3(64), 0, static_cast<hipStream_t>(stream), parts, chan, C,
+                     n_parts, (double)N * (double)L, training, dgamma, dbeta, coef);
+  return launch_status("fpsg_bn_act_bwd_parts_coef");
+}
+
+extern "C" int fpsg_bn_dxsum_vec(const float* vsum, int N, int C, int L, float* dpre_bias, float* ws,
+                                 fpsg_stream_t stream) {
+  using namespace fpsg;
+  int rc = check_dims("fpsg_bn_dxsum_vec", N, C, L, kActRelu);
+  if (rc) return rc;
+  FPSG_REQUIRE_PTR(vsum); FPSG_REQUIRE_PTR(dpre_bias); FPSG_REQUIRE_PTR(ws);
+  FPSG_REQUIRE(L % 4 == 0, FPSG_E_SHAPE, "fpsg_bn_dxsum_vec: L must be a multiple of 4 (got %d)", L);
+  hipStream_t s = static_cast<hipStream_t>(stream);
+  const int segs = (L + kBnSeg - 1) / kBnSeg;
+  float* dxpart = ws + (size_t)C * kBnSlices * 2;
+  hipLaunchKernelGGL(bn_vecsum_kernel, dim3((unsigned)((size_t)N * C), segs), dim3(kBnThreads), 0, s, vsum, L, dxpart);
+  if ((rc = launch_status("fpsg_bn_dxsum_vec(rows)"))) return rc;
+  hipLaunchKernelGGL(bn_dxsum_kernel, dim3(C), dim3(64), 0, s, dxpart, N, C, segs, dpre_bias);
+  return launch_status("fpsg_bn_dxsum_vec(sum)");
 }
 
 extern "C" size_t fpsg_bn_pool_workspace_floats(int N, int C, int H, int W) {
diff --git a/fpsg_amd/csrc/winograd.hip b/fpsg_amd/csrc/winograd.hip
--- a/fpsg_amd/csrc/winograd.hip
+++ b/fpsg_amd/csrc/winograd.hip
@@ -95,12 +95,15 @@
   return t;
 }
 
-template <int M, bool ACT, bool NT = false, bool RAG = false, bool GO = false>
+template <int M, bool ACT, bool NT = false, bool RAG = false, bool GO = false, bool BNB = false>
 __global__ __launch_bounds__(kWinoThreads) void wino_input_kernel(const float* __restrict__ x, int C, int H, int W,
                                                                    int Th, int Tw, long P, long Ps, float* __restrict__ V,
                                                                    const float* __restrict__ chan,
                                                                    const float* __restrict__ pre_bias,
-                                                                   float* __restrict__ dM = nullptr) {
+                                                                   float* __restrict__ dM = nullptr,
+                                                                   const float* __restrict__ yb = nullptr,
+                                                                   const float* __restrict__ coef = nullptr,
+                                                                   float* __restrict__ vsum = nullptr) {
   constexpr int A = Wino<M>::A;
   typedef float vin __attribute__((ext_vector_type(M)));
   const long p_raw = (long)blockIdx.x * kWinoThreads + threadIdx.x;
@@ -114,48 +117,75 @@
   const bool has_left = ti.tw > 0, has_right = ti.tw < Tw - 1;
   const bool left_lane = has_left && lane > 0;
   const bool right_lane = has_right && lane < kWave - 1;
-  float sc = 1.0f, sh = 0.0f, pb = 0.0f;
-  if (ACT) { sc = chan[c]; sh = chan[C + c]; pb = pre_bias ? pre_bias[c] : 0.0f; }
+  static_assert(!BNB || (GO && !ACT), "the BatchNorm-backward load is a form of the output-gradient transform");
+  float sc = 1.0f, sh = 0.0f, pb = 0.0f, k1 = 0.0f, k2 = 0.0f, k3 = 0.0f;
+  if (ACT || BNB) { sc = chan[c]; sh = chan[C + c]; pb = pre_bias ? pre_bias[c] : 0.0f; }
+  if (BNB) { k1 = coef[c]; k2 = coef[C + c]; k3 = coef[2 * C + c]; }
   auto act = [&](float v) { return ACT ? __builtin_fmaxf(fma_rn(v + pb, sc, sh), 0.0f) : v; };
-  vin mid[A];
+  auto val = [&](float v, float u) {
+    if constexpr (BNB) {
+      const float xv = u + pb;
+      const float dz = v * (fma_rn(xv, sc, sh) > 0.0f ? 1.0f : 0.0f);
+      return fma_rn(k1, dz, fma_rn(k2, xv, k3));
+    } else {
+      return act(v);
+    }
+  };
+  vin mid[A], ymid[A];
   bool rin[A];
   const float* rp[A];
+  const float* yrp[A];
   const bool hi_in = !RAG || c0 + 2 < W;
+  auto load_row = [&](const float* q, vin& out) {
+    if constexpr (RAG) {
+      typedef float v2 __attribute__((ext_vector_type(2)));
+      const v2 lo = *reinterpret_cast<const v2*>(q);
+      v2 hi = {0.0f, 0.0f};
+      if (hi_in) hi = *reinterpret_cast<const v2*>(q + 2);
+      out[0] = lo[0]; out[1] = lo[1]; out[M - 2] = hi[0]; out[M - 1] = hi[1];
+    } else {
+      out = *reinterpret_cast<const vin*>(q);
+    }
+  };
 #pragma unroll
   for (int i = 0; i < A; ++i) {
     const int r = r0 + i;
     rin[i] = r >= 0 && r < H;
-    rp[i] = xp + (size_t)(rin[i] ? r : (r < 0 ? 0 : H - 1)) * W + c0;
-    if constexpr (RAG) {
-      typedef float v2 __attribute__((ext_vector_type(2)));
-      const v2 lo = *reinterpret_cast<const v2*>(rp[i]);
-      v2 hi = {0.0f, 0.0f};
-      if (hi_in) hi = *reinterpret_cast<const v2*>(rp[i] + 2);
-      mid[i][0] = lo[0]; mid[i][1] = lo[1]; mid[i][M - 2] = hi[0]; mid[i][M - 1] = hi[1];
-    } else {
-      mid[i] = *reinterpret_cast<const vin*>(rp[i]);
-    }
-  }
-  float el[A], er[A];
-#pragma unroll
-  for (int i = 0; i < A; ++i) el[i] = er[i] = 0.0f;
+    const size_t off = (size_t)(rin[i] ? r : (r < 0 ? 0 : H - 1)) * W + c0;
+    rp[i] = xp + off;
+    load_row(rp[i], mid[i]);
+    if constexpr (BNB) {
+      yrp[i] = yb + ((size_t)ti.n * C + c) * H * W + off;
+      load_row(yrp[i], ymid[i]);
+    }
+  }
+  float el[A], er[A], yel[A], yer[A];
+#pragma unroll
+  for (int i = 0; i < A; ++i) el[i] = er[i] = yel[i] = yer[i] = 0.0f;
   if (has_left && !left_lane) {
 #pragma unroll
-    for (int i = 0; i < A; ++i) el[i] = rp[i][-1];
+    for (int i = 0; i < A; ++i) {
+      el[i] = rp[i][-1];
+      if constexpr (BNB) yel[i] = yrp[i][-1];
+    }
   }
   if (has_right && !right_lane) {
 #pragma unroll
-    for (int i = 0; i < A; ++i) er[i] = rp[i][M];
+    for (int i = 0; i < A; ++i) {
+      er[i] = rp[i][M];
+      if constexpr (BNB) yer[i] = yrp[i][M];
+    }
   }
   float d[A][A];
 #pragma unroll
   for (int i = 0; i < A; ++i) {
 #pragma unroll
-    for (int j = 0; j < M; ++j) mid[i][j] = (rin[i] && (!RAG || j < 2 || hi_in)) ? act(mid[i][j]) : 0.0f;
+    for (int j = 0; j < M; ++j)
+      mid[i][j] = (rin[i] && (!RAG || j < 2 || hi_in)) ? val(mid[i][j], BNB ? ymid[i][j] : 0.0f) : 0.0f;
     float lft = __shfl_up(mid[i][M - 1], 1, kWave);
     float rgt = __shfl_down(mid[i][0], 1, kWave);
-    if (!left_lane) lft = (has_left && rin[i]) ? act(el[i]) : 0.0f;
-    if (!right_lane) rgt = (has_right && rin[i]) ? act(er[i]) : 0.0f;
+    if (!left_lane) lft = (has_left && rin[i]) ? val(el[i], yel[i]) : 0.0f;
+    if (!right_lane) rgt = (has_right && rin[i]) ? val(er[i], yer[i]) : 0.0f;
     d[i][0] = lft;
 #pragma unroll
     for (int j = 0; j < M; ++j) d[i][1 + j] = mid[i][j];
@@ -189,6 +219,14 @@
     Wino<M>::in(row, v);
 #pragma unroll
     for (int j = 0; j < A; ++j) stream_store<NT>(vp + (size_t)(A * i + j) * plane, v[j]);
+  }
+  if constexpr (BNB && M == 4 && !RAG) {
+    if (vsum) {
+      float* sp = vsum + ((size_t)ti.n * C + c) * (size_t)(H * W / 4) + (size_t)(M * ti.th) * (W / 4) + ti.tw;
+#pragma unroll
+      for (int i = 0; i < M; ++i)
+        sp[(size_t)i * (W / 4)] = (mid[1 + i][0] + mid[1 + i][1]) + (mid[1 + i][2] + mid[1 + i][3]);
+    }
   }
   if constexpr (GO) {
     static_assert(!ACT, "an output gradient is not activated");
@@ -617,6 +655,38 @@
   return launch_status("fpsg_wino_grad_transforms");
 }
 
+extern "C" int fpsg_wino_grad_transforms_bnbwd(int m, const float* ga, const float* y, const float* pre_bias,
+                                               const float* chan, const float* coef, int N, int K, int H, int W,
+                                               float* V, float* dM, float* vsum, long ldp, fpsg_stream_t stream) {
+  using namespace fpsg;
+  int rc = check_image("fpsg_wino_grad_transforms_bnbwd", m, N, K, H, W);
+  if (rc) return rc;
+  FPSG_REQUIRE_PTR(ga); FPSG_REQUIRE_PTR(y); FPSG_REQUIRE_PTR(chan); FPSG_REQUIRE_PTR(coef);
+  FPSG_REQUIRE_PTR(V); FPSG_REQUIRE_PTR(dM);
+  FPSG_REQUIRE(((reinterpret_cast<uintptr_t>(ga) | reinterpret_cast<uintptr_t>(y)) & 15) == 0, FPSG_E_ALIGN,
+               "fpsg_wino_grad_transforms_bnbwd: ga and y must be 16-byte aligned");
+  FPSG_REQUIRE(!misaligned4(pre_bias) && !misaligned4(chan) && !misaligned4(coef), FPSG_E_ALIGN,
+               "fpsg_wino_grad_transforms_bnbwd: pre_bias / chan / coef not 4-byte aligned");
+  FPSG_REQUIRE(!misaligned4(vsum), FPSG_E_ALIGN, "fpsg_wino_grad_transforms_bnbwd: vsum not 4-byte aligned");
+  FPSG_REQUIRE(vsum == nullptr || (m == 4 && H % 4 == 0 && W % 4 == 0), FPSG_E_SHAPE,
+               "fpsg_wino_grad_transforms_bnbwd: vsum needs m = 4 and H, W multiples of 4 (got m=%d, %dx%d)", m, H, W);
+  const long P = (long)N * tiles_of(H, m) * tiles_of(W, m);
+  const long Ps = ldp ? ldp : P;
+  FPSG_REQUIRE(Ps >= P, FPSG_E_SHAPE, "fpsg_wino_grad_transforms_bnbwd: row stride %ld must be 0 or at least the %ld tiles",
+               ldp, P);
+  dim3 grid((unsigned)((Ps + kWinoThreads - 1) / kWinoThreads), K);
+  hipStream_t hs = static_cast<hipStream_t>(stream);
+  const int Th = tiles_of(H, m), Tw = tiles_of(W, m);
+#define FPSG_GTB(MM, NT, RAG) hipLaunchKernelGGL((wino_input_kernel<MM, false, NT, RAG, true, true>), grid, dim3(kWinoThreads), 0, \
+                                                 hs, ga, K, H, W, Th, Tw, P, Ps, V, chan, pre_bias, dM, y, coef, vsum)
+  if (m == 2) FPSG_GTB(2, false, false);
+  else if (ragged(m, H, W)) FPSG_GTB(4, false, true);
+  else if ((size_t)36 * K * Ps * sizeof(float) > kStreamBytes) FPSG_GTB(4, true, false);
+  else FPSG_GTB(4, false, false);
+#undef FPSG_GTB
+  return launch_status("fpsg_wino_grad_transforms_bnbwd");
+}
+
 extern "C" int fpsg_wino_filter_transform(int m, const float* w, int K, int C, int flip_transpose, float* U,
                                           fpsg_stream_t stream) {
   using namespace fpsg;
diff --git a/fpsg_amd/image_net.py b/fpsg_amd/image_net.py
--- a/fpsg_amd/image_net.py
+++ b/fpsg_amd/image_net.py
@@ -77,7 +77,14 @@
                                                  stats_bias=layer.bias, want_parts=want)
                     pending = None
                 else:
-                    y = _conv_without_bias(layer, x, want)
+                    chain = self._stage_chain(layers, i, x) if want else None
+                    if chain is not None:
+                        convs, bns = chain
+                        y = winograd.stage_chain(x, convs, bns)
+                        i += 3 * (len(convs) - 1)
+                        layer, bn = layers[i], layers[i + 1]
+                    else:
+                        y = _conv_without_bias(layer, x, want)
                 if want:
                     y, parts = y
                 nxt = layers[i + 3] if i + 3 < len(layers) else None
@@ -108,6 +115,20 @@
                 i += 1
         return self.img_feature_pool(x).flatten(1)
 
+    @staticmethod
+    def _stage_chain(layers, i, x):
+        convs, bns = [layers[i]], [layers[i + 1]]
+        j = i
+        while (j + 5 < len(layers) and isinstance(layers[j + 3], nn.Conv2d) and isinstance(layers[j + 4], nn.BatchNorm2d)
+               and isinstance(layers[j + 5], nn.ReLU) and fusable_conv(layers[j + 3], layers[j + 4], x)
+               and foldable_into(x, layers[j + 1], layers[j + 3]) and wants_conv_stats(layers[j + 3], layers[j + 4], x)):
+            j += 3
+            convs.append(layers[j])
+            bns.append(layers[j + 1])
+        if winograd.stage_chain_applies(x, convs, bns) and all(winograd.eligible(x, c) for c in convs):
+            return convs, bns
+        return None
+
     def _set_finetune(self, new_layer: int | None = None) -> None:
         if new_layer is not None:
             self.finetune_layer = new_layer
diff --git a/fpsg_amd/winograd.py b/fpsg_amd/winograd.py
--- a/fpsg_amd/winograd.py
+++ b/fpsg_amd/winograd.py
@@ -364,6 +364,35 @@
     V = torch.empty(((m + 2) ** 2, K, Ps), dtype=torch.float32, device=gy.device)
     dM = torch.empty_like(V)
     _call("fpsg_wino_grad_transforms", m, _hip.ptr(gy), N, K, H, W, _hip.ptr(V), _hip.ptr(dM), Ps, _hip.stream_of(gy))
+    return V, dM
+
+
+class _FoldedGrad:
+
+    __slots__ = ("ga", "y", "pre_bias", "chan", "coef", "dpb")
+
+    def __init__(self, ga, y, pre_bias, chan, coef, dpb=None):
+        self.ga, self.y, self.pre_bias, self.chan, self.coef, self.dpb = ga, y, pre_bias, chan, coef, dpb
+
+
+def _fold_shape(m, H, W) -> bool:
+    return m == 4 and H % 4 == 0 and W % 4 == 0
+
+
+def _grad_transforms_bnbwd(m, g):
+    N, K, H, W = g.y.shape
+    dev = g.ga.device
+    Ps = row_stride(N * _tiles(H, W, m))
+    V = torch.empty(((m + 2) ** 2, K, Ps), dtype=torch.float32, device=dev)
+    dM = torch.empty_like(V)
+    vsum = torch.empty((N * K * H * W // 4,), dtype=torch.float32, device=dev) if g.dpb is not None else None
+    _call("fpsg_wino_grad_transforms_bnbwd", m, _hip.ptr(g.ga), _hip.ptr(g.y),
+          _hip.ptr(g.pre_bias) if g.pre_bias is not None else None, _hip.ptr(g.chan), _hip.ptr(g.coef), N, K, H, W,
+          _hip.ptr(V), _hip.ptr(dM), _hip.ptr(vsum) if vsum is not None else None, Ps, _hip.stream_of(g.ga))
+    if vsum is not None:
+        lib = _hip.load()
+        ws = torch.empty((lib.fpsg_bn_workspace_floats(N, K, H * W),), dtype=torch.float32, device=dev)
+        _call("fpsg_bn_dxsum_vec", _hip.ptr(vsum), N, K, H * W, _hip.ptr(g.dpb), _hip.ptr(ws), _hip.stream_of(g.ga))
     return V, dM
 
 
@@ -410,31 +439,49 @@
     def backward(ctx, gy, _gparts=None):
         if gy is None:
             return None, None, None, None, None
-        kept, w = ctx.saved_tensors
-        N, C, H, W, m, kept_is_v = ctx.dims
-        K = w.shape[0]
+        return _conv3x3_backward(ctx, gy)
+
+
+def _conv3x3_takes_folded(ctx) -> bool:
+    _, w = ctx.saved_tensors
+    N, C, H, W, m, kept_is_v = ctx.dims
+    K = w.shape[0]
+    return (ctx.needs_input_grad[0] and ctx.needs_input_grad[1] and grad_transforms_enabled() and _fold_shape(m, H, W)
+            and not _can_fuse(m, K, C, N * H * W, H, W) and not (not kept_is_v and _can_fuse_dw(m, C, K, N, H, W)))
+
+
+def _conv3x3_backward(ctx, gy):
+    kept, w = ctx.saved_tensors
+    N, C, H, W, m, kept_is_v = ctx.dims
+    K = w.shape[0]
+    folded = isinstance(gy, _FoldedGrad)
+    if not folded:
         gy = gy.contiguous()
-        gx = gw = None
-        with torch.cuda.device(gy.device):
-            fuse_dx = _can_fuse(m, K, C, N * H * W, H, W)
-            fuse_dw = not kept_is_v and _can_fuse_dw(m, C, K, N, H, W)
-            Vg = dM = None
-            if (ctx.needs_input_grad[0] and ctx.needs_input_grad[1] and not fuse_dx and not fuse_dw
-                    and grad_transforms_enabled()):
-                Vg, dM = _grad_transforms(m, gy)
-            if ctx.needs_input_grad[0]:
-                if fuse_dx:
-                    gx = _fused(gy, _filter(m, w, True))
-                else:
-                    gx = _output(m, _bmm(_filter(m, w, True), Vg if Vg is not None else _input(m, gy)), N, H, W)
-                    Vg = None
-            if ctx.needs_input_grad[1]:
-                if fuse_dw:
-                    gw = _filter_grad(m, _fused_dw(kept, None, None, gy), w)
-                else:
-                    V = kept if kept_is_v else _input(m, kept)
-                    gw = _filter_grad(m, _bmm_nt(dM if dM is not None else _grad_output(m, gy), V), w)
-        return gx, gw, None, None, None
+    dev = gy.ga.device if folded else gy.device
+    gx = gw = None
+    with torch.cuda.device(dev):
+        fuse_dx = _can_fuse(m, K, C, N * H * W, H, W)
+        fuse_dw = not kept_is_v and _can_fuse_dw(m, C, K, N, H, W)
+        Vg = dM = None
+        if folded:
+            assert _conv3x3_takes_folded(ctx)
+            Vg, dM = _grad_transforms_bnbwd(m, gy)
+        elif (ctx.needs_input_grad[0] and ctx.needs_input_grad[1] and not fuse_dx and not fuse_dw
+                and grad_transforms_enabled()):
+            Vg, dM = _grad_transforms(m, gy)
+        if ctx.needs_input_grad[0]:
+            if fuse_dx:
+                gx = _fused(gy, _filter(m, w, True))
+            else:
+                gx = _output(m, _bmm(_filter(m, w, True), Vg if Vg is not None else _input(m, gy)), N, H, W)
+                Vg = None
+        if ctx.needs_input_grad[1]:
+            if fuse_dw:
+                gw = _filter_grad(m, _fused_dw(kept, None, None, gy), w)
+            else:
+                V = kept if kept_is_v else _input(m, kept)
+                gw = _filter_grad(m, _bmm_nt(dM if dM is not None else _grad_output(m, gy), V), w)
+    return gx, gw, None, None, None
 
 
 def _input_act(m, x, chan, pre_bias):
@@ -507,53 +554,81 @@
     def backward(ctx, gout, _gparts=None):
         if gout is None:
             return (None,) * 14
-        y, chan, pre_bias, w, V = ctx.saved_tensors
-        N, C, H, W, m, training, has_g, has_b = ctx.cfg
-        K = w.shape[0]
-        lib = _hip.load()
-        dev = y.device
+        return _bnrc_backward(ctx, gout, False)
+
+
+def _bnrc_takes_folded(ctx) -> bool:
+    y, _, _, w, V = ctx.saved_tensors
+    N, C, H, W, m = ctx.cfg[:5]
+    K = w.shape[0]
+    return (ctx.needs_input_grad[9] and grad_transforms_enabled() and _fold_shape(m, H, W)
+            and not _can_fuse(m, K, C, N * H * W, H, W)
+            and not (V is None and _can_fuse_dw(m, C, K, N, H, W)))
+
+
+def _bnrc_backward(ctx, gout, fold):
+    y, chan, pre_bias, w, V = ctx.saved_tensors
+    N, C, H, W, m, training, has_g, has_b = ctx.cfg
+    K = w.shape[0]
+    lib = _hip.load()
+    dev = y.device
+    folded_in = isinstance(gout, _FoldedGrad)
+    if not folded_in:
         gout = gout.contiguous()
-        gw = None
-        with torch.cuda.device(dev):
-            bwd_parts = None
-            fuse_dx = _can_fuse(m, K, C, N * H * W, H, W)
-            fuse_dw = V is None and _can_fuse_dw(m, C, K, N, H, W)
-            Vg = dM = None
-            if ctx.needs_input_grad[9] and not fuse_dx and not fuse_dw and grad_transforms_enabled():
-                Vg, dM = _grad_transforms(m, gout)
-            if fuse_dx:
-                ga = _fused(gout, _filter(m, w, True))
-            elif bwd_stats_enabled() and N * H * W > _BN_SMALL_MAX:
-                ga, bwd_parts = _output_bwd_stats(m, _bmm(_filter(m, w, True), Vg if Vg is not None else _input(m, gout)),
-                                                  N, H, W, y, pre_bias, chan)
+    gw = None
+    with torch.cuda.device(dev):
+        bwd_parts = None
+        fuse_dx = _can_fuse(m, K, C, N * H * W, H, W)
+        fuse_dw = V is None and _can_fuse_dw(m, C, K, N, H, W)
+        Vg = dM = None
+        if folded_in:
+            assert _bnrc_takes_folded(ctx)
+            Vg, dM = _grad_transforms_bnbwd(m, gout)
+        elif ctx.needs_input_grad[9] and not fuse_dx and not fuse_dw and grad_transforms_enabled():
+            Vg, dM = _grad_transforms(m, gout)
+        if fuse_dx:
+            ga = _fused(gout, _filter(m, w, True))
+        elif bwd_stats_enabled() and N * H * W > _BN_SMALL_MAX:
+            ga, bwd_parts = _output_bwd_stats(m, _bmm(_filter(m, w, True), Vg if Vg is not None else _input(m, gout)),
+                                              N, H, W, y, pre_bias, chan)
+        else:
+            ga = _output(m, _bmm(_filter(m, w, True), Vg if Vg is not None else _input(m, gout)), N, H, W)
+        Vg = None
+        if ctx.needs_input_grad[9]:
+            if fuse_dw:
+                gw = _filter_grad(m, _fused_dw(y, chan, pre_bias, gout), w)
             else:
-                ga = _output(m, _bmm(_filter(m, w, True), Vg if Vg is not None else _input(m, gout)), N, H, W)
-            Vg = None
-            if ctx.needs_input_grad[9]:
-                if fuse_dw:
-                    gw = _filter_grad(m, _fused_dw(y, chan, pre_bias, gout), w)
-                else:
-                    if V is None:
-                        V = _input_act(m, y, chan, pre_bias)
-                    gw = _filter_grad(m, _bmm_nt(dM if dM is not None else _grad_output(m, gout), V), w)
-            want_dpb = pre_bias is not None and ctx.needs_input_grad[1]
-            dy = torch.empty_like(y)
+                if V is None:
+                    V = _input_act(m, y, chan, pre_bias)
+                gw = _filter_grad(m, _bmm_nt(dM if dM is not None else _grad_output(m, gout), V), w)
+        want_dpb = pre_bias is not None and ctx.needs_input_grad[1]
+        if fold and bwd_parts is not None:
             dgamma = torch.empty((C,), dtype=torch.float32, device=dev)
             dbeta = torch.empty((C,), dtype=torch.float32, device=dev)
+            coef = torch.empty((3, C), dtype=torch.float32, device=dev)
+            _call("fpsg_bn_act_bwd_parts_coef", _hip.ptr(chan), N, C, H * W, 1 if training else 0, _hip.ptr(dgamma),
+                  _hip.ptr(dbeta), _hip.ptr(coef), _hip.ptr(bwd_parts), bwd_parts.shape[1], _hip.stream_of(y))
             dpb = torch.empty((C,), dtype=torch.float32, device=dev) if want_dpb else None
-            coef = torch.empty((3, C), dtype=torch.float32, device=dev)
-            ws = torch.empty((lib.fpsg_bn_workspace_floats(N, C, H * W),), dtype=torch.float32, device=dev)
-            if bwd_parts is not None:
-                _call("fpsg_bn_act_bwd_parts", _hip.ptr(y), _hip.ptr(pre_bias) if pre_bias is not None else None,
-                      _hip.ptr(ga), _hip.ptr(chan), N, C, H * W, 1 if training else 0, 1, 0.0, _hip.ptr(dy),
-                      _hip.ptr(dgamma), _hip.ptr(dbeta), _hip.ptr(dpb) if want_dpb else None, _hip.ptr(coef),
-                      _hip.ptr(ws), _hip.ptr(bwd_parts), bwd_parts.shape[1], _hip.stream_of(y))
-            else:
-                _call("fpsg_bn_act_bwd", _hip.ptr(y), _hip.ptr(pre_bias) if pre_bias is not None else None, _hip.ptr(ga),
-                      _hip.ptr(chan), N, C, H * W, 1 if training else 0, 1, 0.0, _hip.ptr(dy), _hip.ptr(dgamma),
-                      _hip.ptr(dbeta), _hip.ptr(dpb) if want_dpb else None, _hip.ptr(coef), _hip.ptr(ws), _hip.stream_of(y))
-        return (dy, dpb, dgamma if has_g else None, dbeta if has_b else None, None, None, None, None, None, gw, None,
-                None, None, None)
+            dy = _FoldedGrad(ga, y, pre_bias, chan, coef, dpb)
+            return (dy, dpb, dgamma if has_g else None, dbeta if has_b else None, None, None, None, None, None, gw,
+                    None, None, None, None)
+        dy = torch.empty_like(y)
+        dgamma = torch.empty((C,), dtype=torch.float32, device=dev)
+        dbeta = torch.empty((C,), dtype=torch.float32, device=dev)
+        dpb = torch.empty((C,), dtype=torch.float32, device=dev) if want_dpb else None
+        coef = torch.empty((3, C), dtype=torch.float32, device=dev)
+        ws = torch.empty((lib.fpsg_bn_workspace_floats(N, C, H * W),), dtype=torch.float32, device=dev)
+        if bwd_parts is not None:
+            _call("fpsg_bn_act_bwd_parts", _hip.ptr(y), _hip.ptr(pre_bias) if pre_bias is not None else None,
+                  _hip.ptr(ga), _hip.ptr(chan), N, C, H * W, 1 if training else 0, 1, 0.0, _hip.ptr(dy),
+                  _hip.ptr(dgamma), _hip.ptr(dbeta), _hip.ptr(dpb) if want_dpb else None, _hip.ptr(coef),
+                  _hip.ptr(ws), _hip.ptr(bwd_parts), bwd_parts.shape[1], _hip.stream_of(y))
+        else:
+            _call("fpsg_bn_act_bwd", _hip.ptr(y), _hip.ptr(pre_bias) if pre_bias is not None else None, _hip.ptr(ga),
+                  _hip.ptr(chan), N, C, H * W, 1 if training else 0, 1, 0.0, _hip.ptr(dy), _hip.ptr(dgamma),
+                  _hip.ptr(dbeta), _hip.ptr(dpb) if want_dpb else None, _hip.ptr(coef), _hip.ptr(ws), _hip.stream_of(y))
+    return (dy, dpb, dgamma if has_g else None, dbeta if has_b else None, None, None, None, None, None, gw, None,
+            None, None, None)
 
 
 def stem_fold_enabled() -> bool:
@@ -673,6 +748,91 @@
                                 bn.eps, weight, m, parts, stats_bias, bool(want_parts))
 
 
+def bn_bwd_fold_enabled() -> bool:
+    return os.environ.get("FPSG_BN_BWD_FOLD", "1") != "0"
+
+
+class _SubCtx:
+
+    def __init__(self, needs_input_grad):
+        self.needs_input_grad = needs_input_grad
+        self.saved_tensors = ()
+
+    def set_materialize_grads(self, value):
+        pass
+
+    def save_for_backward(self, *tensors):
+        self.saved_tensors = tensors
+
+    def mark_non_differentiable(self, *tensors):
+        pass
+
+
+_CHAIN_LAYER_ARGS = 8
+
+
+class _StageChain(torch.autograd.Function):
+
+    @staticmethod
+    def forward(ctx, ms, x, w0, *rest):
+        ctx.set_materialize_grads(False)
+        n = 1 + (len(rest) - 1) // _CHAIN_LAYER_ARGS
+        need = ctx.needs_input_grad
+        sub = _SubCtx((need[1], need[2], False, False, False))
+        y, parts = _Conv3x3.forward(sub, x, w0, ms[0], rest[0], True)
+        subs = [sub]
+        for L in range(1, n):
+            b = 3 + _CHAIN_LAYER_ARGS * (L - 1)
+            pb, gamma, beta, rmean, rvar, mom, eps, w = rest[_CHAIN_LAYER_ARGS * (L - 1):_CHAIN_LAYER_ARGS * L]
+            sub = _SubCtx((True, need[b], need[b + 1], need[b + 2], False, False, False, False, False, need[b + 7],
+                           False, False, False, False))
+            y, parts = _BNReluConv3x3.forward(sub, y, pb, gamma, beta, rmean, rvar, True, mom, eps, w, ms[L], parts,
+                                              rest[_CHAIN_LAYER_ARGS * L], True)
+            subs.append(sub)
+        ctx.subs = subs
+        ctx.n_args = 3 + len(rest)
+        ctx.mark_non_differentiable(parts)
+        return y, parts
+
+    @staticmethod
+    def backward(ctx, gout, _gparts=None):
+        grads = [None] * ctx.n_args
+        if gout is None:
+            return tuple(grads)
+        subs = ctx.subs
+        if subs is None:
+            raise RuntimeError("_StageChain: backward through the same graph twice (retain_graph) is not supported")
+        ctx.subs = None
+        g = gout
+        for L in range(len(subs) - 1, 0, -1):
+            prev = subs[L - 1]
+            fold = _bnrc_takes_folded(prev) if L > 1 else _conv3x3_takes_folded(prev)
+            r = _bnrc_backward(subs[L], g, fold)
+            b = 3 + _CHAIN_LAYER_ARGS * (L - 1)
+            g = r[0]
+            grads[b], grads[b + 1], grads[b + 2], grads[b + 7] = r[1], r[2], r[3], r[9]
+        gx, gw0 = _conv3x3_backward(subs[0], g)[:2]
+        grads[1], grads[2] = gx, gw0
+        return tuple(grads)
+
+
+def stage_chain_applies(x, convs, bns) -> bool:
+    return (bn_bwd_fold_enabled() and len(convs) >= 2 and stats_enabled() and x.is_cuda and x.dtype == torch.float32
+            and x.dim() == 4 and x.shape[0] * x.shape[2] * x.shape[3] > _BN_SMALL_MAX
+            and all(bn.training and bn.track_running_stats for bn in bns[:-1]))
+
+
+def stage_chain(x, convs, bns):
+    m = tile_size(x.shape[2], x.shape[3])
+    rest = []
+    for L in range(1, len(convs)):
+        bn = bns[L - 1]
+        count_batch(bn)
+        mom = 0.1 if bn.momentum is None else float(bn.momentum)
+        rest += [convs[L - 1].bias, bn.weight, bn.bias, bn.running_mean, bn.running_var, mom, bn.eps, convs[L].weight]
+    rest.append(convs[-1].bias)
+    return _StageChain.apply((m,) * len(convs), x.contiguous(), convs[0].weight, *rest)
+
 def conv3x3(x: torch.Tensor, weight: torch.Tensor, m: int | None = None, stats_bias=None, want_parts: bool = False):
     if x.dim() != 4 or weight.dim() != 4 or tuple(weight.shape[2:]) != (3, 3) or weight.shape[1] != x.shape[1]:
         raise ValueError(f"conv3x3: x {tuple(x.shape)} / weight {tuple(weight.shape)}")
diff --git a/include/fpsg_hip.h b/include/fpsg_hip.h
--- a/include/fpsg_hip.h
+++ b/include/fpsg_hip.h
@@ -171,6 +171,9 @@
                           int C, int L, int training, int act, float slope, float* dx, float* dgamma,
                           float* dbeta, float* dpre_bias, float* coef, float* ws, const float* parts,
                           int n_parts, fpsg_stream_t stream);
+int fpsg_bn_act_bwd_parts_coef(const float* chan, int N, int C, int L, int training, float* dgamma, float* dbeta,
+                               float* coef, const float* parts, int n_parts, fpsg_stream_t stream);
+int fpsg_bn_dxsum_vec(const float* vsum, int N, int C, int L, float* dpre_bias, float* ws, fpsg_stream_t stream);
 
 size_t fpsg_bn_pool_workspace_floats(int N, int C, int H, int W);
 int fpsg_bn_act_pool_fwd(const float* x, const float* pre_bias, const float* gamma, const float* beta,
@@ -222,6 +225,9 @@
                                     fpsg_stream_t stream);
 int fpsg_wino_grad_transforms(int m, const float* dy, int N, int K, int H, int W, float* V, float* dM, long ldp,
                               fpsg_stream_t stream);
+int fpsg_wino_grad_transforms_bnbwd(int m, const float* ga, const float* y, const float* pre_bias, const float* chan,
+                                    const float* coef, int N, int K, int H, int W, float* V, float* dM, float* vsum,
+                                    long ldp, fpsg_stream_t stream);
 int fpsg_wino_filter_transform(int m, const float* w, int K, int C, int flip_transpose, float* U,
                                fpsg_stream_t stream);
 int fpsg_wino_filter_transform_batch(const int64_t* jobs, int n_jobs, long total_blocks, fpsg_stream_t stream);
```

After: 46.18, median of 6. About the same (+0.2%).
